# PiggyCh/RL_arm_under_sparse_reward

Hardware: AMD Instinct MI355X
Metric: HER-relabelled transitions sampled+updated /sec, batch 256, 1/2/4/8 MI355X (higher is better)
Workload: dtype f32; 1 GPU; push task (obs 27, goal 3, action 4, T 100), buffer 500000 transitions (5000 episodes) per GPU, batch 256 per GPU, replay_k 4, HIP HER sampler + FP32-MFMA DDPG update, 40 updates + store/normalizer/polyak per cycle; global_batch=256, episodes_per_gpu=5000, parallelism=dp1, cycle_mode=hipGraph, sampler_rng=MT19937 numpy-legacy stream on device (bit-exact indices)

## Files before the change

include/rlarm_hip_debug.h:

```cpp
#ifndef RLARM_HIP_DEBUG_H
#define RLARM_HIP_DEBUG_H

#include "rlarm_hip.h"

#ifdef __cplusplus
extern "C" {
#endif

int hp_ctx_launch_floor(hp_ctx *ctx, int n, int graph, double *us_per_kernel);
int hp_ctx_event_pair_us(hp_ctx *ctx, int reps, double *us);
int hp_ctx_clock_mhz(hp_ctx *ctx, double *mhz);

int hp_buffer_sample_device_us(hp_buffer *buf, hp_rng *rng, int64_t batch, double future_p, double sq_threshold,
                               int32_t reps, double *draw_us, double *gather_us);

int hp_buffer_sample_dev_us(hp_buffer *buf, hp_rng *rng, hp_norm *o_norm, hp_norm *g_norm, int64_t batch, double future_p,
                            double sq_threshold, double clip_obs, int32_t reps, int32_t f32_rows, double *draw_us, double *gather_us);

int hp_buffer_sample_dev_fast_us(hp_buffer *buf, hp_norm *o_norm, hp_norm *g_norm, int64_t batch, double future_p, double sq_threshold,
                                 double clip_obs, int32_t reps, int32_t f32_rows, double *us);

int hp_mt_jump_poly(uint64_t n_words, uint64_t *limbs312);
int hp_rng_parallel_info(hp_rng *rng, int64_t *min_batch, int64_t *n_parallel, int64_t *n_fallback);
int hp_rng_debug_set_window(hp_rng *rng, int64_t words);
int hp_rng_debug_table_ms(hp_rng *rng, double *ms);

int hp_agent_set_adam(hp_agent *ag, int32_t net, const float *m_host, const float *v_host, int64_t n, int64_t step);

int hp_agent_debug_chain(hp_agent *ag, int32_t kind, int32_t n, double *us_per_launch);
int hp_agent_update_kernels(hp_agent *ag, hp_buffer *buf, hp_norm *o_norm, hp_norm *g_norm, hp_rng *rng, double future_p,
                            double sq_threshold, int32_t n_updates, int32_t caller_exchanges, char *out, int32_t out_len);
int hp_agent_debug_timeline(hp_agent *ag, uint64_t *out192);

#define HP_STATE_DIRTY_CHUNK 2048
int hp_state_debug_dirty_scan(hp_buffer *buf, const uint32_t *stamps_host, int64_t current_size, uint32_t since, int64_t max_dirty,
                              int64_t *slots_out, int64_t *n_dirty, int32_t *overflow);

int hp_rollout_debug_set_launch_cap(hp_rollout *ro, int64_t timesteps);

int hp_ctx_calibrate(hp_ctx *ctx, double *out4);

#ifdef __cplusplus
}
#endif
#endif
```

rl_arm_under_sparse_reward_amd/_lib.py:

```python
from __future__ import annotations

import ctypes as C
import os
import threading

import numpy as np

_PKG = os.path.dirname(os.path.abspath(__file__))
LIB_PATH = os.path.join(_PKG, "librlarm_hip.so")

c_void_pp = C.POINTER(C.c_void_p)
f64p = C.POINTER(C.c_double)
f32p = C.POINTER(C.c_float)
i64p = C.POINTER(C.c_int64)
u32p = C.POINTER(C.c_uint32)
u8p = C.POINTER(C.c_uint8)


class HpError(RuntimeError):
    pass


class SampleOut(C.Structure):
    _fields_ = [("obs", f64p), ("ag", f64p), ("g", f64p), ("actions", f64p), ("obs_next", f64p), ("ag_next", f64p),
                ("r", f32p), ("e", i64p), ("t", i64p), ("future_t", i64p), ("her", u8p), ("r64", f64p)]


class SampleDevOut(C.Structure):
    _fields_ = [("x", C.c_void_p), ("x_next", C.c_void_p), ("actions", C.c_void_p), ("r", C.c_void_p),
                ("e", C.c_void_p), ("t", C.c_void_p), ("future_t", C.c_void_p), ("her", C.c_void_p)]


class AgentCfg(C.Structure):
    _fields_ = [("obs_dim", C.c_int32), ("goal_dim", C.c_int32), ("act_dim", C.c_int32), ("hidden", C.c_int32),
                ("batch", C.c_int32), ("grad_world_size", C.c_int32),
                ("max_action", C.c_double), ("gamma", C.c_double), ("action_l2", C.c_double),
                ("lr_actor", C.c_double), ("lr_critic", C.c_double), ("polyak", C.c_double),
                ("clip_obs", C.c_double), ("clip_range", C.c_double),
                ("adam_beta1", C.c_double), ("adam_beta2", C.c_double), ("adam_eps", C.c_double)]


class StateSection(C.Structure):
    _fields_ = [("name", C.c_char * 32), ("dtype", C.c_int32), ("elem_bytes", C.c_int32), ("count", C.c_int64),
                ("offset", C.c_int64)]


class EnvDesc(C.Structure):
    _fields_ = [("kind", C.c_int32), ("reserved", C.c_int32), ("params", C.c_double * 8), ("state_dev", C.c_void_p * 4)]


class DemoScriptDesc(C.Structure):
    _fields_ = [("phase_end", C.c_int32 * 5), ("reserved", C.c_int32), ("lift", C.c_double * 4), ("waypoint", C.c_double * 3),
                ("behind", C.c_double), ("stop_radius", C.c_double)]


ENV_POINT_MASS = 1
ENV_PUSH_BLOCK = 2
ROLLOUT_MAX_LAUNCH_TIMESTEPS = 4096


class StateDims(C.Structure):
    _fields_ = [("obs_dim", C.c_int32), ("goal_dim", C.c_int32), ("act_dim", C.c_int32), ("hidden", C.c_int32),
                ("T", C.c_int32), ("reserved", C.c_int32), ("capacity", C.c_int64), ("current_size", C.c_int64)]


STATE_SECTIONS = 32
STATE_DELTA_SECTIONS = 34
STATE_DIRTY_CHUNK = 2048
ABI_VERSION = 4
PARALLEL_DRAW_MIN_BATCH = 65536

DEBUG_SYMBOLS = {"hp_ctx_launch_floor", "hp_ctx_event_pair_us", "hp_ctx_clock_mhz", "hp_ctx_calibrate", "hp_buffer_sample_device_us",
                 "hp_buffer_sample_dev_us", "hp_buffer_sample_dev_fast_us",
                 "hp_mt_jump_poly", "hp_rng_parallel_info", "hp_rng_debug_set_window", "hp_rng_debug_table_ms",
                 "hp_state_debug_dirty_scan", "hp_rollout_debug_set_launch_cap",
                 "hp_agent_set_adam", "hp_agent_debug_chain", "hp_agent_debug_timeline", "hp_agent_update_kernels"}

PROTOTYPES = {
    "hp_abi_version": (C.c_int, []),
    "hp_last_error": (C.c_char_p, []),
    "hp_ctx_create": (C.c_int, [C.c_int, c_void_pp]),
    "hp_ctx_set_stream": (C.c_int, [C.c_void_p, C.c_void_p]),
    "hp_ctx_get_stream": (C.c_int, [C.c_void_p, c_void_pp]),
    "hp_ctx_borrow_stream": (C.c_int, [C.c_void_p, C.c_void_p]),
    "hp_ctx_return_stream": (C.c_int, [C.c_void_p]),
    "hp_ctx_synchronize": (C.c_int, [C.c_void_p]),
    "hp_ctx_device_name": (C.c_int, [C.c_void_p, C.c_char_p, C.c_size_t]),
    "hp_ctx_pci_bus_id": (C.c_int, [C.c_void_p, C.c_char_p, C.c_size_t]),
    "hp_ctx_launch_floor": (C.c_int, [C.c_void_p, C.c_int, C.c_int, f64p]),
    "hp_ctx_event_pair_us": (C.c_int, [C.c_void_p, C.c_int, f64p]),
    "hp_ctx_clock_mhz": (C.c_int, [C.c_void_p, f64p]),
    "hp_ctx_calibrate": (C.c_int, [C.c_void_p, f64p]),
    "hp_ctx_destroy": (None, [C.c_void_p]),
    "hp_rng_create": (C.c_int, [C.c_void_p, c_void_pp]),
    "hp_rng_seed": (C.c_int, [C.c_void_p, C.c_uint32]),
    "hp_rng_set_state": (C.c_int, [C.c_void_p, u32p, C.c_int32]),
    "hp_rng_get_state": (C.c_int, [C.c_void_p, u32p, C.POINTER(C.c_int32)]),
    "hp_rng_randint": (C.c_int, [C.c_void_p, C.c_int64, C.c_int64, C.c_int64, i64p]),
    "hp_rng_uniform": (C.c_int, [C.c_void_p, C.c_int64, f64p]),
    "hp_rng_standard_normal": (C.c_int, [C.c_void_p, C.c_int64, f64p]),
    "hp_rng_binomial1": (C.c_int, [C.c_void_p, C.c_double, C.c_double, C.c_int64, i64p]),
    "hp_rng_get_gauss": (C.c_int, [C.c_void_p, C.POINTER(C.c_int32), f64p]),
    "hp_rng_set_gauss": (C.c_int, [C.c_void_p, C.c_int32, C.c_double]),
    "hp_rng_advance": (C.c_int, [C.c_void_p, C.c_uint64]),
    "hp_rng_set_parallel": (C.c_int, [C.c_void_p, C.c_int64]),
    "hp_rng_parallel_info": (C.c_int, [C.c_void_p, i64p, i64p, i64p]),
    "hp_rng_debug_set_window": (C.c_int, [C.c_void_p, C.c_int64]),
    "hp_rng_debug_table_ms": (C.c_int, [C.c_void_p, f64p]),
    "hp_mt_jump_poly": (C.c_int, [C.c_uint64, C.POINTER(C.c_uint64)]),
    "hp_rng_destroy": (None, [C.c_void_p]),
    "hp_buffer_create": (C.c_int, [C.c_void_p, C.c_int64, C.c_int32, C.c_int32, C.c_int32, C.c_int32, c_void_pp]),
    "hp_buffer_store": (C.c_int, [C.c_void_p, C.c_void_p, f64p, f64p, f64p, f64p, C.c_int64]),
    "hp_buffer_stage": (C.c_int, [C.c_void_p, f64p, f64p, f64p, f64p, C.c_int64]),
    "hp_host_register": (C.c_int, [C.c_void_p, C.c_void_p, C.c_size_t]),
    "hp_host_unregister": (C.c_int, [C.c_void_p, C.c_void_p]),
    "hp_buffer_store_pinned": (C.c_int, [C.c_void_p, C.c_void_p, C.c_void_p, C.c_int64, C.POINTER(C.c_uint64)]),
    "hp_buffer_store_dev": (C.c_int, [C.c_void_p, C.c_void_p, C.c_void_p, C.c_int64]),
    "hp_buffer_store_done": (C.c_int, [C.c_void_p, C.c_uint64, C.c_int32, C.POINTER(C.c_int32)]),
    "hp_buffer_info": (C.c_int, [C.c_void_p, i64p, i64p, i64p, C.POINTER(C.c_int32)]),
    "hp_buffer_last_slots": (C.c_int, [C.c_void_p, i64p, C.c_int64]),
    "hp_buffer_read": (C.c_int, [C.c_void_p, C.c_int32, C.c_int64, C.c_int64, f64p]),
    "hp_buffer_sample": (C.c_int, [C.c_void_p, C.c_void_p, C.c_int64, C.c_double, C.c_double, C.POINTER(SampleOut)]),
    "hp_buffer_sample_device_us": (C.c_int, [C.c_void_p, C.c_void_p, C.c_int64, C.c_double, C.c_double, C.c_int32, f64p,
                                             f64p]),
    "hp_buffer_sample_dev": (C.c_int, [C.c_void_p, C.c_void_p, C.c_void_p, C.c_void_p, C.c_int64, C.c_double, C.c_double,
                                       C.c_double, C.POINTER(SampleDevOut)]),
    "hp_buffer_sample_dev_us": (C.c_int, [C.c_void_p, C.c_void_p, C.c_void_p, C.c_void_p, C.c_int64, C.c_double, C.c_double,
                                          C.c_double, C.c_int32, C.c_int32, f64p, f64p]),
    "hp_buffer_enable_f32_rows": (C.c_int, [C.c_void_p]),
    "hp_buffer_sample_dev_f32": (C.c_int, [C.c_void_p, C.c_void_p, C.c_void_p, C.c_void_p, C.c_int64, C.c_double, C.c_double,
                                           C.c_double, C.POINTER(SampleDevOut)]),
    "hp_buffer_sample_dev_fast": (C.c_int, [C.c_void_p, C.c_void_p, C.c_void_p, C.c_int64, C.c_double, C.c_double, C.c_double,
                                            C.c_uint64, C.c_uint64, C.c_int32, C.POINTER(SampleDevOut)]),
    "hp_buffer_sample_dev_fast_us": (C.c_int, [C.c_void_p, C.c_void_p, C.c_void_p, C.c_int64, C.c_double, C.c_double, C.c_double,
                                               C.c_int32, C.c_int32, f64p]),
    "hp_buffer_destroy": (None, [C.c_void_p]),
    "hp_compute_reward_dev": (C.c_int, [C.c_void_p, C.c_void_p, C.c_void_p, C.c_int64, C.c_int32, C.c_double, C.c_int32,
                                        C.c_void_p, C.c_void_p]),
    "hp_is_success_dev": (C.c_int, [C.c_void_p, C.c_void_p, C.c_void_p, C.c_int64, C.c_int32, C.c_double, C.c_void_p]),
    "hp_compute_reward": (C.c_int, [C.c_void_p, f64p, f64p, C.c_int64, C.c_int32, C.c_double, C.c_int32, f32p, f64p]),
    "hp_is_success": (C.c_int, [C.c_void_p, f64p, f64p, C.c_int64, C.c_int32, C.c_double, f32p]),
    "hp_norm_create": (C.c_int, [C.c_void_p, C.c_int32, C.c_double, C.c_double, C.c_int32, c_void_pp]),
    "hp_norm_update": (C.c_int, [C.c_void_p, f64p, C.c_int64]),
    "hp_norm_recompute_begin": (C.c_int, [C.c_void_p, c_void_pp, i64p]),
    "hp_norm_recompute_end": (C.c_int, [C.c_void_p]),
    "hp_norm_recompute": (C.c_int, [C.c_void_p]),
    "hp_norm_get": (C.c_int, [C.c_void_p, f32p, f64p, f32p, f32p, f32p, f32p, f32p, f32p]),
    "hp_norm_set_stats": (C.c_int, [C.c_void_p, f32p, f64p]),
    "hp_norm_normalize": (C.c_int, [C.c_void_p, f64p, C.c_int64, C.c_double, f64p]),
    "hp_norm_update_from_staged": (C.c_int, [C.c_void_p, C.c_void_p, C.c_void_p, C.c_void_p, C.c_double, C.c_double]),
    "hp_norm_destroy": (None, [C.c_void_p]),
    "hp_agent_create": (C.c_int, [C.c_void_p, C.POINTER(AgentCfg), c_void_pp]),
    "hp_agent_param_count": (C.c_int64, [C.c_void_p, C.c_int32]),
    "hp_agent_set_params": (C.c_int, [C.c_void_p, C.c_int32, f32p, C.c_int64]),
    "hp_agent_get_params": (C.c_int, [C.c_void_p, C.c_int32, f32p, C.c_int64]),
    "hp_agent_get_grads": (C.c_int, [C.c_void_p, C.c_int32, f32p, C.c_int64]),
    "hp_agent_get_adam": (C.c_int, [C.c_void_p, C.c_int32, f32p, f32p, C.c_int64, i64p]),
    "hp_agent_set_adam": (C.c_int, [C.c_void_p, C.c_int32, f32p, f32p, C.c_int64, C.c_int64]),
    "hp_agent_update_minibatch": (C.c_int, [C.c_void_p, f32p, f32p, f32p, f32p, f32p]),
    "hp_agent_sample_and_update": (C.c_int, [C.c_void_p, C.c_void_p, C.c_void_p, C.c_void_p, C.c_void_p, C.c_double,
                                             C.c_double, C.c_int32]),
    "hp_agent_get_losses": (C.c_int, [C.c_void_p, f32p, C.c_int32]),
    "hp_agent_soft_update": (C.c_int, [C.c_void_p]),
    "hp_agent_actor_forward": (C.c_int, [C.c_void_p, C.c_int32, f32p, C.c_int64, f32p]),
    "hp_agent_critic_forward": (C.c_int, [C.c_void_p, C.c_int32, f32p, f32p, C.c_int64, f32p]),
    "hp_agent_act": (C.c_int, [C.c_void_p, C.c_void_p, C.c_void_p, C.c_int32, f64p, f64p, C.c_int64, C.c_double, f32p]),
    "hp_agent_act_dev": (C.c_int, [C.c_void_p, C.c_void_p, C.c_void_p, C.c_int32, C.c_void_p, C.c_void_p, C.c_int64, C.c_double,
                                   C.c_void_p]),
    "hp_rollout_create": (C.c_int, [C.c_void_p, C.c_void_p, C.c_int64, c_void_pp]),
    "hp_rollout_begin": (C.c_int, [C.c_void_p, C.c_int64, C.c_int64]),
    "hp_rollout_set_action_max": (C.c_int, [C.c_void_p, C.c_double]),
    "hp_rollout_step": (C.c_int, [C.c_void_p, C.c_void_p, C.c_void_p, C.c_void_p, C.c_void_p, C.c_int32, C.c_void_p, C.c_void_p,
                                  C.c_void_p, C.c_int32, C.c_double, C.c_double, C.c_double, C.c_double, C.c_void_p]),
    "hp_rollout_finish": (C.c_int, [C.c_void_p, C.c_void_p, C.c_void_p]),
    "hp_rollout_block": (C.c_int, [C.c_void_p, c_void_pp, i64p, i64p, i64p]),
    "hp_rollout_read": (C.c_int, [C.c_void_p, C.c_int32, f64p]),
    "hp_rollout_destroy": (None, [C.c_void_p]),
    "hp_streams_create": (C.c_int, [C.c_void_p, C.c_int64, c_void_pp]),
    "hp_streams_seed": (C.c_int, [C.c_void_p, u32p, C.c_int64, C.c_uint32]),
    "hp_streams_get_state": (C.c_int, [C.c_void_p, C.c_int64, u32p, C.POINTER(C.c_int32), C.POINTER(C.c_int32), f64p]),
    "hp_streams_set_state": (C.c_int, [C.c_void_p, C.c_int64, u32p, C.c_int32, C.c_int32, C.c_double]),
    "hp_streams_get_all": (C.c_int, [C.c_void_p, u32p, C.POINTER(C.c_int32), C.POINTER(C.c_int32), f64p]),
    "hp_streams_set_all": (C.c_int, [C.c_void_p, u32p, C.POINTER(C.c_int32), C.POINTER(C.c_int32), f64p]),
    "hp_streams_destroy": (None, [C.c_void_p]),
    "hp_rollout_step_streams": (C.c_int, [C.c_void_p, C.c_void_p, C.c_void_p, C.c_void_p, C.c_void_p, C.c_int32, C.c_void_p,
                                          C.c_void_p, C.c_void_p, C.c_int32, C.c_double, C.c_double, C.c_double, C.c_double,
                                          C.c_void_p]),
    "hp_rollout_episodes": (C.c_int, [C.c_void_p, C.c_void_p, C.c_void_p, C.c_void_p, C.c_void_p, C.POINTER(EnvDesc), C.c_int32,
                                      C.c_double, C.c_double, C.c_double, C.c_double, C.c_void_p]),
    "hp_env_reset": (C.c_int, [C.c_void_p, C.POINTER(EnvDesc), C.c_void_p, C.c_int64]),
    "hp_rollout_waves": (C.c_int, [C.c_void_p, C.c_void_p, C.c_void_p, C.c_void_p, C.c_void_p, C.c_void_p, C.POINTER(EnvDesc),
                                   C.c_int64, C.c_int32, C.c_double, C.c_double, C.c_double, C.c_double, C.c_void_p,
                                   C.POINTER(C.c_int32)]),
    "hp_rollout_debug_set_launch_cap": (C.c_int, [C.c_void_p, C.c_int64]),
    "hp_demo_episodes": (C.c_int, [C.c_void_p, C.POINTER(EnvDesc), C.c_void_p, C.POINTER(DemoScriptDesc), C.c_int64, C.c_int64,
                                   C.c_int64, C.c_int32, C.c_void_p, C.c_void_p, C.c_void_p, C.POINTER(C.c_int32)]),
    "hp_demo_compact": (C.c_int, [C.c_void_p, C.c_void_p, C.c_void_p, C.c_void_p, C.c_int64, C.c_void_p, C.c_void_p, C.c_int64,
                                  C.c_int64, C.c_void_p]),
    "hp_agent_policy_snapshot": (C.c_int, [C.c_void_p, C.c_void_p, C.c_void_p]),
    "hp_agent_act_snapshot": (C.c_int, [C.c_void_p, f64p, f64p, C.c_int64, C.c_double, f32p]),
    "hp_agent_forward_backward": (C.c_int, [C.c_void_p, C.c_void_p, C.c_void_p, C.c_void_p, C.c_void_p, C.c_double,
                                            C.c_double]),
    "hp_agent_grad_buffer": (C.c_int, [C.c_void_p, c_void_pp, i64p]),
    "hp_agent_param_buffer": (C.c_int, [C.c_void_p, c_void_pp, i64p]),
    "hp_agent_apply": (C.c_int, [C.c_void_p]),
    "hp_agent_sync_targets": (C.c_int, [C.c_void_p]),
    "hp_comm_unique_id": (C.c_int, [u8p]),
    "hp_comm_create": (C.c_int, [C.c_void_p, u8p, C.c_int32, C.c_int32, c_void_pp]),
    "hp_comm_info": (C.c_int, [C.c_void_p, C.POINTER(C.c_int32), C.POINTER(C.c_int32)]),
    "hp_comm_allreduce_sum_f32": (C.c_int, [C.c_void_p, C.c_void_p, C.c_int64]),
    "hp_comm_allreduce_mean_f32": (C.c_int, [C.c_void_p, C.c_void_p, C.c_int64]),
    "hp_comm_broadcast_f32": (C.c_int, [C.c_void_p, C.c_void_p, C.c_int64, C.c_int32]),
    "hp_comm_destroy": (None, [C.c_void_p]),
    "hp_agent_set_comm": (C.c_int, [C.c_void_p, C.c_void_p]),
    "hp_peer_create": (C.c_int, [C.c_void_p, C.c_int32, C.c_int32, C.c_int64, c_void_pp, u8p]),
    "hp_peer_connect": (C.c_int, [C.c_void_p, u8p]),
    "hp_peer_allreduce_f32": (C.c_int, [C.c_void_p, C.c_void_p, C.c_int64, C.c_int32]),
    "hp_peer_selfcheck": (C.c_int, [C.c_void_p, C.POINTER(C.c_uint32)]),
    "hp_peer_status": (C.c_int, [C.c_void_p, C.POINTER(C.c_uint32)]),
    "hp_peer_phases": (C.c_int, [C.c_void_p, C.POINTER(C.c_int32)]),
    "hp_peer_set_gate": (C.c_int, [C.c_void_p, C.c_int32]),
    "hp_peer_destroy": (None, [C.c_void_p]),
    "hp_agent_set_peer": (C.c_int, [C.c_void_p, C.c_void_p]),
    "hp_agent_cycle_mode": (C.c_int, [C.c_void_p, C.POINTER(C.c_int32)]),
    "hp_agent_set_grad_reduce": (C.c_int, [C.c_void_p, C.c_int32]),
    "hp_agent_train_cycle": (C.c_int, [C.c_void_p, C.c_void_p, C.c_void_p, C.c_void_p, C.c_void_p, f64p, f64p, f64p,
                                       f64p, C.c_int64, C.c_double, C.c_double, C.c_int32]),
    "hp_agent_train_cycle_pinned": (C.c_int, [C.c_void_p, C.c_void_p, C.c_void_p, C.c_void_p, C.c_void_p, C.c_void_p, C.c_int64,
                                              C.c_double, C.c_double, C.c_int32, C.POINTER(C.c_uint64)]),
    "hp_agent_train_cycle_dev": (C.c_int, [C.c_void_p, C.c_void_p, C.c_void_p, C.c_void_p, C.c_void_p, C.c_void_p, C.c_int64,
                                           C.c_double, C.c_double, C.c_int32]),
    "hp_agent_debug_chain": (C.c_int, [C.c_void_p, C.c_int32, C.c_int32, f64p]),
    "hp_agent_debug_timeline": (C.c_int, [C.c_void_p, C.POINTER(C.c_uint64)]),
    "hp_agent_update_kernels": (C.c_int, [C.c_void_p, C.c_void_p, C.c_void_p, C.c_void_p, C.c_void_p, C.c_double, C.c_double,
                                          C.c_int32, C.c_int32, C.c_char_p, C.c_int32]),
    "hp_agent_engine": (C.c_int, [C.c_void_p, C.POINTER(C.c_int32), C.POINTER(C.c_int32), C.POINTER(C.c_int32)]),
    "hp_agent_status": (C.c_int, [C.c_void_p, u32p]),
    "hp_agent_update_form": (C.c_int, [C.c_void_p, C.c_int32, C.POINTER(C.c_int32)]),
    "hp_agent_profile": (C.c_int, [C.c_void_p, C.c_int32]),
    "hp_agent_profile_read": (C.c_int, [C.c_void_p, f64p, C.c_int32]),
    "hp_agent_destroy": (None, [C.c_void_p]),
    "hp_state_layout": (C.c_int, [C.c_void_p, C.c_void_p, C.c_void_p, C.c_void_p, C.c_int64, C.POINTER(StateSection),
                                  C.POINTER(C.c_int32), C.POINTER(C.c_size_t)]),
    "hp_state_capture": (C.c_int, [C.c_void_p, C.c_void_p, C.c_void_p, C.c_void_p, C.c_void_p, C.POINTER(C.c_uint64),
                                   C.POINTER(C.c_size_t)]),
    "hp_state_fetch": (C.c_int, [C.c_void_p, C.c_uint64, C.c_int32, C.c_void_p, C.c_size_t, C.POINTER(C.c_uint64),
                                 C.POINTER(C.c_int32)]),
    "hp_state_restore": (C.c_int, [C.c_void_p, C.c_void_p, C.c_void_p, C.c_void_p, C.c_void_p, C.POINTER(StateDims), C.c_void_p,
                                   C.c_size_t, C.POINTER(C.c_uint64)]),
    "hp_state_layout_delta": (C.c_int, [C.c_void_p, C.c_void_p, C.c_void_p, C.c_void_p, C.c_int64, C.POINTER(StateSection),
                                        C.POINTER(C.c_int32), C.POINTER(C.c_size_t)]),
    "hp_state_capture_delta": (C.c_int, [C.c_void_p, C.c_void_p, C.c_void_p, C.c_void_p, C.c_void_p, C.c_uint32, C.c_int64,
                                         C.POINTER(C.c_uint64), C.POINTER(C.c_size_t)]),
    "hp_state_epochs": (C.c_int, [C.c_void_p, C.c_void_p, u32p, u32p, u32p]),
    "hp_state_debug_dirty_scan": (C.c_int, [C.c_void_p, u32p, C.c_int64, C.c_uint32, C.c_int64, i64p, i64p,
                                            C.POINTER(C.c_int32)]),
    "hp_state_checksum_dev": (C.c_int, [C.c_void_p, C.c_void_p, C.c_size_t, C.c_int32, C.POINTER(C.c_uint64)]),
}

_lib = None
_lock = threading.Lock()

pending_lock = threading.RLock()
_pending = []
_NO_FLUSH = {"hp_last_error", "hp_abi_version"}


def register_pending(obj):
    with pending_lock:
        if not any(o is obj for o in _pending):
            _pending.append(obj)


def unregister_pending(obj):
    with pending_lock:
        _pending[:] = [o for o in _pending if o is not obj]


def flush_pending():
    if not _pending:
        return
    with pending_lock:
        todo, _pending[:] = list(_pending), []
        for i, o in enumerate(todo):
            try:
                o._flush_updates()
            except BaseException:
                for rest in todo[i + 1:]:
                    register_pending(rest)
                raise


class _Library:

    def __init__(self, cdll):
        object.__setattr__(self, "_cdll", cdll)

    def __getattr__(self, name):
        fn = getattr(object.__getattribute__(self, "_cdll"), name)
        if name in _NO_FLUSH or not name.startswith("hp_"):
            return fn

        def call(*args):
            if _pending:
                flush_pending()
            return fn(*args)

        call.__name__ = name
        object.__setattr__(self, name, call)
        return call


def load(path: str | None = None):
    global _lib
    with _lock:
        if _lib is not None:
            return _lib
        p = path or os.environ.get("RLARM_LIB") or LIB_PATH
        if not os.path.exists(p):
            raise HpError(
                f"{p} is missing: build it with `python -c 'import __graft_entry__ as g; g.build()'` "
                "(hipcc --offload-arch=gfx950).  This package has no CPU fallback.")
        lib = C.CDLL(p)
        missing = []
        for name, (res, args) in PROTOTYPES.items():
            try:
                fn = getattr(lib, name)
            except AttributeError:
                missing.append(name)
                continue
            fn.restype = res
            fn.argtypes = args
        if missing:
            raise HpError("librlarm_hip.so does not export: " + ", ".join(missing) + " -- rebuild it")
        if lib.hp_abi_version() != ABI_VERSION:
            raise HpError(f"librlarm_hip.so has ABI version {lib.hp_abi_version()}, this package binds version {ABI_VERSION} "
                          "(include/rlarm_hip.h: HP_ABI_VERSION) -- rebuild it")
        _lib = _Library(lib)
        return _lib


def last_error(lib=None):
    return ((lib or load()).hp_last_error() or b"").decode("utf-8", "replace")


def check(status: int):
    if status == 0:
        return
    msg = (load().hp_last_error() or b"").decode("utf-8", "replace")
    if status in (-1, -2):
        raise ValueError(msg)
    raise HpError(f"[hp_status {status}] {msg}")


def ptr(a: np.ndarray, ctype):
    return a.ctypes.data_as(C.POINTER(ctype)) if a is not None else None


def as_f64(a):
    return np.ascontiguousarray(a, dtype=np.float64)


def as_f32(a):
    return np.ascontiguousarray(a, dtype=np.float32)


class Context:

    _default = None

    def __init__(self, device_id: int | None = None):
        lib = load()
        if device_id is None:
            device_id = int(os.environ.get("LOCAL_RANK", "0"))
        h = C.c_void_p()
        check(lib.hp_ctx_create(int(device_id), C.byref(h)))
        self.lib, self.h, self.device_id = lib, h, int(device_id)

    @classmethod
    def default(cls):
        if cls._default is None:
            cls._default = cls()
        return cls._default

    def set_stream(self, stream_ptr):
        check(self.lib.hp_ctx_set_stream(self.h, C.c_void_p(stream_ptr or 0)))
        self._bound_stream = stream_ptr or 0

    def use_torch_stream(self):
        import torch

        torch.cuda.set_device(self.device_id)
        self.set_stream(torch.cuda.current_stream(self.device_id).cuda_stream or 1)

    def torch_bridge(self):
        import contextlib

        import torch

        @contextlib.contextmanager
        def bridge():
            cur = C.c_void_p(torch.cuda.current_stream(self.device_id).cuda_stream or None)
            check(self.lib.hp_ctx_borrow_stream(self.h, cur))
            try:
                yield
            finally:
                self.lib.hp_ctx_return_stream(self.h)
        return bridge()

    def synchronize(self):
        check(self.lib.hp_ctx_synchronize(self.h))

    @property
    def name(self):
        buf = C.create_string_buffer(160)
        check(self.lib.hp_ctx_device_name(self.h, buf, 160))
        return buf.value.decode()


class DevicePointer:

    def __init__(self, address: int, n: int, typestr="<f4"):
        self.__cuda_array_interface__ = {"shape": (int(n),), "typestr": typestr, "data": (int(address), False),
                                         "version": 2}
```

rl_arm_under_sparse_reward_amd/csrc/agent.h:

```cpp
#pragma once
#include "internal.h"

#include <algorithm>
#include <cstdlib>

typedef float f32x4 __attribute__((ext_vector_type(4)));
typedef float f32x16 __attribute__((ext_vector_type(16)));

#define S8_AHEAD_WGS 4
#define S32_ROWS 32
#define DW_PART (64 * 64 + 64)

struct NetLayout {
    int K1;
    int w1, b1, w2, b2, w3, b3, w4, b4, total;
};

enum { EPI_NONE = 0, EPI_BIAS_RELU = 1, EPI_BIAS = 2, EPI_BIAS_TANH = 3, EPI_MASK = 4 };

struct GemmProb {
    const float *A, *B;
    float *C;
    const float *bias;
    const float *mask;
    float *bias_grad;
    float *C2;
    int a_si, a_sk;
    int b_sj, b_sk;
    int ldc, ldmask, ldc2;
    int M, N, K;
    int n_store;
    int epi;
    int tile0, tiles_n;
    int ks, part0;
    float max_action;
    int frag_layer;
};

#define MAX_PROBS 8
#define GL_PART (32 * 32 + 32)
#define GL_MAX_SPLIT_TILES 64
#define GL_MAX_KS 8
struct GemmGroup {
    int n;
    int xcd;
    int uni;
    int bias0;
    int loss_wg;
    float *part;
    unsigned long long *ticket;
    GemmProb p[MAX_PROBS];
};

struct Pass {
    float *h1, *h2, *h3;
};

struct AgentDevState {
    long long step;
    long long n_logged;
    float neg_step_actor, neg_step_critic, bc2_sqrt;
    unsigned open_timeouts;
};

struct AdamCfg {
    double lr_actor, lr_critic, beta1, beta2, eps;
};

__device__ __forceinline__ void adam_prepare(AgentDevState *st, const AdamCfg c) {
    const double step = (double)st->step;
    const double bc1 = 1.0 - pow(c.beta1, step);
    const double bc2 = 1.0 - pow(c.beta2, step);
    st->neg_step_actor = (float)(-(c.lr_actor / bc1));
    st->neg_step_critic = (float)(-(c.lr_critic / bc1));
    st->bc2_sqrt = (float)sqrt(bc2);
}

#define SPLIT_CTR_STRIDE 64
#define SPLIT_COUNTERS 8
#define SPLIT_CTR_NONE 15u
#define SPLIT_SET_WORDS (SPLIT_COUNTERS * 8 * SPLIT_CTR_STRIDE)
#define SPLIT_FAULT (2 * SPLIT_SET_WORDS)
#define SPLIT_SYNC_WORDS (SPLIT_FAULT + 4)

__device__ __forceinline__ void handoff_fault(unsigned *fault, unsigned *fault_host, unsigned which) {
    const unsigned word = 1u | (1u << (3u + which));
    __hip_atomic_fetch_or(fault, word, __ATOMIC_RELAXED, __HIP_MEMORY_SCOPE_AGENT);
    if (fault_host) __hip_atomic_fetch_or(fault_host, word, __ATOMIC_RELAXED, __HIP_MEMORY_SCOPE_SYSTEM);
}

__device__ __forceinline__ bool handoff_wait(const unsigned *ctr, unsigned need, unsigned long long ticks, unsigned *fault,
                                             unsigned *fault_host, unsigned which, int *flag) {
    if (threadIdx.x == 0) {
        int ok = 1;
        const unsigned long long t0 = wall_clock64();
        for (;;) {
            const unsigned seen = __hip_atomic_load(ctr, __ATOMIC_RELAXED, __HIP_MEMORY_SCOPE_AGENT);
            if (seen >= need) break;
            if (seen == 0u) __builtin_amdgcn_s_sleep(64);
            else __builtin_amdgcn_s_sleep(6);
            if (wall_clock64() - t0 > ticks) {
                handoff_fault(fault, fault_host, which);
                ok = 0;
                break;
            }
        }
        *flag = ok;
    }
    __syncthreads();
    const bool ok = *flag != 0;
    __syncthreads();
    return ok;
}
#define LOSS_LOG 4096

#include "slab_common.h"
#include "peer.h"

struct SeqKey {
    enum Kind { CYCLE, UPDATES } kind;
    hp_buffer *b;
    hp_norm *on, *gn;
    hp_rng *rng;
    int n;
    int64_t n_new;
    double future_p, sq_threshold;
    bool open;
    uint64_t gen;
    bool operator==(const SeqKey &o) const {
        return kind == o.kind && b == o.b && on == o.on && gn == o.gn && rng == o.rng && n == o.n && n_new == o.n_new &&
               future_p == o.future_p && sq_threshold == o.sq_threshold && open == o.open && gen == o.gen;
    }
};
struct GraphCache {
    struct Entry {
        SeqKey key;
        GraphExec exec;
    };
    std::vector<Entry> entries;
    hipGraphExec_t find(const SeqKey &k) const {
        for (const Entry &e : entries)
            if (e.key == k) return e.exec.h;
        return nullptr;
    }
    bool has(SeqKey::Kind kind) const {
        return std::any_of(entries.begin(), entries.end(), [&](const Entry &e) { return e.key.kind == kind; });
    }
    hipGraphExec_t put(const SeqKey &k, GraphExec &&x) {
        const auto same_kind = [&](const Entry &e) { return e.key.kind == k.kind; };
        if (std::count_if(entries.begin(), entries.end(), same_kind) >= (k.kind == SeqKey::CYCLE ? 1 : 8))
            entries.erase(std::find_if(entries.begin(), entries.end(), same_kind));
        entries.push_back({k, std::move(x)});
        return entries.back().exec.h;
    }
    void clear() { entries.clear(); }
};

enum { PROF_SAMPLE = 0, PROF_GEMM_FWD = 1, PROF_GEMM_BWD = 2, PROF_LOSS = 3, PROF_ADAM = 4, PROF_PLAN = 5, PROF_DW = 6, PROF_N = 7 };

struct hp_agent {
    hp_ctx *ctx = nullptr;
    hp_agent_cfg cfg;
    int H = 256, B = 0, Mp = 0;
    int xdim = 0, act_off = 0, ldx = 0;
    NetLayout la, lc;
    int n_arena = 0;
    float *params = nullptr, *targets = nullptr, *grads = nullptr, *adam_m = nullptr, *adam_v = nullptr;
    float *XA = nullptr, *XP = nullptr, *XT = nullptr, *R = nullptr, *TP = nullptr;
    float *XA2 = nullptr, *XP2 = nullptr, *XT2 = nullptr, *R2 = nullptr;
    Pass AT, CT, CA, AP, CP;
    float *QT = nullptr, *QA = nullptr, *QP = nullptr, *dQA = nullptr, *dQP = nullptr;
    float *QT2 = nullptr;
    float *dA3 = nullptr, *dA2 = nullptr, *dA1 = nullptr;
    float *dP3 = nullptr, *dP2 = nullptr, *dP1 = nullptr, *dXP = nullptr;
    float *dZ = nullptr, *dK3 = nullptr, *dK2 = nullptr, *dK1 = nullptr;
    float *loss_log = nullptr;
    AgentDevState *d_state = nullptr;
    float *fragF = nullptr, *fragD = nullptr, *fragFT = nullptr, *part = nullptr;
    unsigned long long *timeline = nullptr;
    bool slab = true;
    bool slab8 = true;
    bool slab32 = false;
    int s8_rows = 4;
    bool fuse_adam_ok = true;
    bool dw64 = false;
    int dw_S = 3;
    DevBuf dw_part, dw_ticket;
    int chain_wt = -1;
    bool keep_grads_dbg = false;
    bool upd_graph_ok = true;
    bool gather_ahead = true;
    DevBuf plan, norm_plan;
    int plan_batches = 0;
    DevBuf fwd_ws;
    struct PolicySnap {
        float *params = nullptr, *fragF = nullptr;
        NormDev *on = nullptr, *gn = nullptr;
        double clip_o = 0, clip_g = 0;
        int od = 0, gd = 0;
        hipEvent_t ready = nullptr;
    } snap[2];
    int snap_cur = -1, snap_pending = -1;
    struct StateArena *state = nullptr;
    hipStream_t act_stream = nullptr;
    hipEvent_t act_done = nullptr;
    bool act_recorded = false;
    DevBuf act_ws;
    PinnedBuf pin;
    std::vector<void *> owned;
    hp_comm *comm = nullptr;
    hp_peer *peer = nullptr;
    bool grad_mean = false;
    bool comm_warm = false;
    bool graph_refused = false;
    GraphCache graphs;
    unsigned *open_sync = nullptr;
    int loss_wg = 1;
    int dw_ksplit = 0;
    float *gl_part = nullptr;
    unsigned long long *gl_ticket = nullptr;
    int split_mode = -1;
    unsigned *k1_sync = nullptr;
    unsigned *fault_host = nullptr;
    unsigned *fault_host_dev = nullptr;
    bool cycle_open = true;
    bool prof = false;
    hipEvent_t ev0 = nullptr, ev1 = nullptr;
    double prof_ms[PROF_N] = {0};
    long long prof_cnt[PROF_N] = {0};
    long long host_steps = 0;
};


static inline AdamCfg adam_cfg(const hp_agent *a) {
    return AdamCfg{a->cfg.lr_actor, a->cfg.lr_critic, a->cfg.adam_beta1, a->cfg.adam_beta2, a->cfg.adam_eps};
}

static inline NetLayout make_layout(int K1, int H) {
    NetLayout l;
    l.K1 = K1;
    int o = 0;
    l.w1 = o; o += H * K1;
    l.b1 = o; o += H;
    l.w2 = o; o += H * H;
    l.b2 = o; o += H;
    l.w3 = o; o += H * H;
    l.b3 = o; o += H;
    l.w4 = o; o += 16 * H;
    l.b4 = o; o += 16;
    l.total = o;
    return l;
}

static inline int roundup(int v, int m) { return (v + m - 1) / m * m; }

struct Launch {
    GemmGroup g;
    int tiles = 0;
    Launch() {
        g.n = 0;
        g.xcd = 0;
        g.uni = 0;
        g.bias0 = 0;
        g.loss_wg = 0;
        g.part = nullptr;
        g.ticket = nullptr;
    }
    int split_tiles = 0;
    unsigned long long head(int half) const {
        unsigned long long w = 0ull;
        for (int i = 0; i < 4; ++i) {
            const int pi = 4 * half + i;
            w |= (unsigned long long)(pi < g.n ? (g.p[pi].tile0 & 0xffff) : 0xffff) << (16 * i);
        }
        return w;
    }
    int separate_bias() {
        int nb = 0;
        for (int i = 0; i < g.n; ++i)
            if (g.p[i].bias_grad) nb += (g.p[i].M + 31) / 32;
        g.bias0 = tiles;
        return nb;
    }
    void split_last(int ks) {
        GemmProb &p = g.p[g.n - 1];
        const int nt = tiles - p.tile0;
        p.ks = ks;
        p.part0 = split_tiles;
        split_tiles += nt;
        tiles += (ks - 1) * nt;
    }
    void place_on_xcds() {
        if (g.n < 4) return;
        for (int i = 0; i < 4; ++i)
            if (g.p[i].tiles_n != 8 || g.p[i].M != 256 || g.p[i].tile0 != 64 * i) return;
        g.xcd = 1;
    }
    GemmProb &add(int M, int N, int K) {
        GemmProb &p = g.p[g.n++];
        memset(&p, 0, sizeof(p));
        p.M = M; p.N = N; p.K = K;
        p.n_store = N;
        p.ks = 1;
        p.tiles_n = (N + 31) / 32;
        p.tile0 = tiles;
        tiles += ((M + 31) / 32) * p.tiles_n;
        return p;
    }
};

struct ProfScope {
    hp_agent *a;
    int which;
    ProfScope(hp_agent *ag, int w) : a(ag), which(w) {
        if (a->prof) (void)hipEventRecord(a->ev0, a->ctx->stream);
    }
    ~ProfScope() {
        if (a->prof) {
            (void)hipEventRecord(a->ev1, a->ctx->stream);
            (void)hipEventSynchronize(a->ev1);
            float ms = 0.f;
            (void)hipEventElapsedTime(&ms, a->ev0, a->ev1);
            a->prof_ms[which] += ms;
            a->prof_cnt[which] += 1;
        }
    }
};

static inline void add_fwd(Launch &L, const float *X, int ldx, int K, const float *W, const float *bias, float *Y, int ldy,
                    int M, int N, int epi) {
    GemmProb &p = L.add(M, N, K);
    p.A = X; p.a_si = ldx; p.a_sk = 1;
    p.B = W; p.b_sj = K; p.b_sk = 1;
    p.C = Y; p.ldc = ldy;
    p.bias = bias;
    p.epi = epi;
}

static inline void add_dx(Launch &L, const float *dY, int ldy, int Nout, const float *W, int Kin, float *dX, int lddx, int M,
                   const float *gate, int ldgate) {
    GemmProb &p = L.add(M, Kin, Nout);
    p.A = dY; p.a_si = ldy; p.a_sk = 1;
    p.B = W; p.b_sj = 1; p.b_sk = Kin;
    p.C = dX; p.ldc = lddx;
    p.mask = gate; p.ldmask = ldgate;
    p.epi = gate ? EPI_MASK : EPI_NONE;
}

static inline void add_dw(Launch &L, const float *dY, int ldy, int Nout, const float *X, int ldx, int Kin, float *dW,
                   float *db, int Mrows, int layer = 0) {
    GemmProb &p = L.add(Nout, Kin, Mrows);
    p.frag_layer = layer;
    p.A = dY; p.a_si = 1; p.a_sk = ldy;
    p.B = X; p.b_sj = 1; p.b_sk = ldx;
    p.C = dW; p.ldc = Kin;
    p.bias_grad = db;
    p.epi = EPI_NONE;
}

enum { SPLIT_TILES_ADAM = 0,
       SPLIT_TILES_PEER = 1,
       SPLIT_TILES_GRADS = 2 };
#define SPLIT_MIN_UPDATES 12

struct SeqPlan {
    enum { RIDE_NONE,
           RIDE_CHAIN,
           RIDE_DW,
           RIDE_FRONT
    } ride = RIDE_NONE;
    int lead = 1;
    bool ahead = false;
    bool s32_serial = false;
    bool split = false;
    int tiles_mode = SPLIT_TILES_GRADS;
    enum { OPT_NONE,
           OPT_TILES,
           OPT_PEER_TILES,
           OPT_KERNEL,
           OPT_PEER_KERNEL,
           OPT_ALLREDUCE
    } opt = OPT_NONE;
    bool fold = false;
};

struct GatherCtx {
    hp_buffer *b;
    hp_norm *on, *gn;
    const PlanRec *plan;
    double sq;
    const SeqPlan *seq = nullptr;
    int u = 0;
    hp_rng *rng = nullptr;
    PlanRec *next_plan = nullptr;
    double future_p = 0.0;
    int xset = 0;
    bool pregathered = false;
    const PlanRec *ahead_plan = nullptr;
    float *grads_out = nullptr;
    bool polyak_after = false;
    int qset = 0;
    const PlanRec *t_plan = nullptr;
};

static inline int chain_wgs(const hp_agent *a) { return 2 * (a->Mp / a->s8_rows); }

int launch_group(hp_agent *a, const Launch &L, int which);
int enqueue_gather(hp_agent *a, hp_buffer *b, hp_norm *on, hp_norm *gn, const PlanRec *plan, double sq, int xset = 0,
                   hipStream_t stream = nullptr);
int enqueue_relayout(hp_agent *a, bool targets);
Launch build_dw_group(const hp_agent *a, const float *sXA, const float *sXP, float *grads = nullptr);
int enqueue_forward_backward(hp_agent *a, const GatherCtx *gc = nullptr, bool fuse_adam = false, bool *fused = nullptr);
int enqueue_forward_backward_slab(hp_agent *a, const GatherCtx *gc, bool fuse_adam, int only = 0);
bool split_fits(const hp_agent *a);
bool split_fits_rows(const hp_agent *a, int rows);
int enqueue_split_prologue(hp_agent *a, const GatherCtx *gc);
int agent_check_fault(const hp_agent *a, const char *who);
static inline unsigned *split_set(const hp_agent *a, int u) { return a->k1_sync + (u & 1) * SPLIT_SET_WORDS; }
int enqueue_adam(hp_agent *a, const GatherCtx *gc = nullptr, unsigned *reset_sync = nullptr);
int enqueue_polyak(hp_agent *a);
bool cycle_open_fits(const hp_agent *a, int64_t n_new);
int cycle_open_launch(hp_agent *a, hp_buffer *b, hp_norm *on, hp_norm *gn, hp_rng *rng, PlanRec *norm_plan, int n_first,
                      double future_p, bool recompute);
int enqueue_peer_adam(hp_agent *a, const GatherCtx *gc, unsigned *reset_sync);
void state_arena_destroy(hp_agent *a);
int enqueue_forward_backward_layers(hp_agent *a);
int layers_enqueue_adam(hp_agent *a);
int layers_enqueue_polyak(hp_agent *a);
```

rl_arm_under_sparse_reward_amd/csrc/agent.hip:

```cpp
#include "agent.h"

#include <functional>

static int run_seq(hp_agent *a, const SeqKey &k);

int agent_check_fault(const hp_agent *a, const char *who) {
    const unsigned w = a->fault_host ? *(volatile const unsigned *)a->fault_host : 0u;
    if (w == 0u) return HP_OK;
    hp_set_error("%s: an in-launch hand-off gave up earlier (%s%s%s; word 0x%x): the launches since skipped work and the "
                 "learner's state is not valid -- recreate the agent", who, (w & 0x10u) ? "critic chains -> weight-gradient tiles; " : "",
                 (w & 0x20u) ? "actor chains -> critic optimizer step; " : "", (w & 0x40u) ? "cycle-opening launch; " : "", w);
    return HP_ERR_STATE;
}

static int ensure_plan(hp_agent *a, int n_batches, int norm_rows = 0) {
    if (n_batches > a->plan_batches) {
        a->graphs.clear();
        HP_TRY(a->plan.ensure((size_t)n_batches * a->B * sizeof(PlanRec)));
        a->plan_batches = n_batches;
    }
    if ((size_t)norm_rows * sizeof(PlanRec) > a->norm_plan.bytes) {
        a->graphs.clear();
        HP_TRY(a->norm_plan.ensure((size_t)norm_rows * sizeof(PlanRec)));
    }
    return HP_OK;
}

static int check_handles(hp_agent *a, hp_buffer *b, hp_norm *on, hp_norm *gn, hp_rng *rng, const char *who) {
    HP_REQUIRE(a && b && on && gn && rng, HP_ERR_INVALID, "%s: null handle", who);
    HP_REQUIRE(b->obs_dim == a->cfg.obs_dim && b->goal_dim == a->cfg.goal_dim && b->act_dim == a->cfg.act_dim,
               HP_ERR_INVALID, "%s: buffer dimensions do not match the agent", who);
    HP_REQUIRE(on->size == a->cfg.obs_dim && gn->size == a->cfg.goal_dim, HP_ERR_INVALID,
               "%s: normalizer sizes do not match the agent", who);
    return HP_OK;
}

struct CycleOpts {
    PlanRec *norm_plan;
    bool open;
    bool recompute;
    std::function<int()> between;
    bool polyak_folded = false;
};
static bool peer_tiles_ok(const hp_agent *a) {
    return a->peer && a->peer->tiles && a->peer->phases == 1 && !a->peer->gate && a->slab && !a->dw64 && a->fuse_adam_ok &&
           build_dw_group(a, a->XA, a->XP).tiles <= HP_PEER_TILES;
}

static SeqPlan seq_plan(const hp_agent *a, int n_updates, bool with_adam) {
    SeqPlan p;
    const bool ride = a->slab && with_adam;
    const bool full = a->slab8 && chain_wgs(a) + 1 + S8_AHEAD_WGS > a->ctx->cu_count;
    const bool s32_ride = ride && a->slab32 && !a->prof;
    const bool dw_ride = s32_ride || (ride && a->slab8 && full);
    p.s32_serial = a->slab32 && !s32_ride;
    p.ahead = ride && ((a->slab8 && (a->gather_ahead || dw_ride)) || s32_ride);
    p.lead = p.ahead ? 2 : 1;
    p.ride = !ride ? SeqPlan::RIDE_NONE : dw_ride ? SeqPlan::RIDE_DW
           : (p.s32_serial && 2 * (a->Mp / S32_ROWS) >= a->ctx->cu_count) ? SeqPlan::RIDE_FRONT : SeqPlan::RIDE_CHAIN;
    const bool peer_tiles = with_adam && peer_tiles_ok(a);
    const bool fuse = with_adam && !a->comm && (!a->peer || peer_tiles) && a->slab && a->fuse_adam_ok;
    p.opt = !with_adam ? SeqPlan::OPT_NONE : peer_tiles ? SeqPlan::OPT_PEER_TILES : a->peer ? SeqPlan::OPT_PEER_KERNEL
          : fuse ? SeqPlan::OPT_TILES : a->comm ? SeqPlan::OPT_ALLREDUCE : SeqPlan::OPT_KERNEL;
    p.split = p.ahead && p.ride == SeqPlan::RIDE_CHAIN && a->slab8 && split_fits(a) &&
              (a->split_mode >= 0 ? a->split_mode == 1 : n_updates >= SPLIT_MIN_UPDATES);
    p.tiles_mode = p.opt == SeqPlan::OPT_PEER_TILES ? SPLIT_TILES_PEER : p.opt == SeqPlan::OPT_TILES ? SPLIT_TILES_ADAM : SPLIT_TILES_GRADS;
    return p;
}

static int enqueue_updates(hp_agent *a, hp_buffer *b, hp_norm *on, hp_norm *gn, hp_rng *rng, double future_p, double sq,
                           int n_updates, bool with_adam, CycleOpts *cyc = nullptr) {
    SeqPlan P = seq_plan(a, n_updates, with_adam);
    P.fold = cyc && with_adam && a->slab;
    HP_REQUIRE(P.opt != SeqPlan::OPT_PEER_TILES || !a->comm, HP_ERR_STATE,
               "tile-wise exchange: the engine did not take the fused optimizer path (a communicator is attached too)");
    PlanRec *plans = a->plan.as<PlanRec>();
    HP_KLOG("#open");
    {
        ProfScope ps(a, PROF_PLAN);
        const int first = P.ride != SeqPlan::RIDE_NONE ? std::min(n_updates, P.lead) : n_updates;
        if (cyc && cyc->open)
            HP_TRY(cycle_open_launch(a, b, on, gn, rng, cyc->norm_plan, first, future_p, cyc->recompute));
        else if (cyc)
            HP_TRY(rng_launch_plan2(rng, b->staged_n, b->T, b->T, cyc->norm_plan, b->d_meta, a->B, first, future_p, plans));
        else
            HP_TRY(rng_launch_plan(rng, b->d_meta, 0, b->T, a->B, first, future_p, plans));
    }
    if (cyc && cyc->between) HP_TRY(cyc->between());
    if (cyc) cyc->polyak_folded = P.fold;
    if (P.split) {
        HP_KLOG("#prologue");
        GatherCtx g0{b, on, gn, plans, sq, &P};
        HP_TRY(enqueue_split_prologue(a, &g0));
    }
    for (int u = 0; u < n_updates; ++u) {
        HP_KLOG("#update");
        GatherCtx gc{b, on, gn, plans + (size_t)u * a->B, sq, &P, u};
        gc.qset = u & 1;
        gc.t_plan = (P.split && u + 1 < n_updates) ? plans + (size_t)(u + 1) * a->B : nullptr;
        if (P.ride != SeqPlan::RIDE_NONE && u + P.lead < n_updates) {
            PlanRec *next = plans + (size_t)(u + P.lead) * a->B;
            if (P.ride == SeqPlan::RIDE_FRONT) HP_TRY(rng_launch_plan(rng, b->d_meta, 0, b->T, a->B, 1, future_p, next));
            else {
                gc.rng = rng;
                gc.next_plan = next;
                gc.future_p = future_p;
            }
        }
        if (a->slab32 && (P.s32_serial || u == 0))
            HP_TRY(enqueue_gather(a, b, on, gn, gc.plan, sq, P.ahead ? (u & 1) : 0));
        if (P.ahead) {
            gc.xset = u & 1;
            gc.pregathered = u > 0;
            if (u + 1 < n_updates) gc.ahead_plan = plans + (size_t)(u + 1) * a->B;
        }
        gc.polyak_after = P.fold && u == n_updates - 1;
        if (P.opt == SeqPlan::OPT_PEER_KERNEL) gc.grads_out = peer_grad_buffer(a->peer, u + 1);
        HP_TRY(enqueue_forward_backward(a, &gc, P.opt == SeqPlan::OPT_TILES || P.opt == SeqPlan::OPT_PEER_TILES));
        unsigned *reset = P.split && P.tiles_mode == SPLIT_TILES_GRADS ? split_set(a, u) : nullptr;
        if (P.opt == SeqPlan::OPT_PEER_KERNEL) {
            HP_TRY(enqueue_peer_adam(a, &gc, reset));
        } else if (P.opt == SeqPlan::OPT_ALLREDUCE) {
            HP_TRY(a->grad_mean ? comm_allreduce_mean_f32(a->comm, a->grads, (size_t)a->n_arena)
                                : comm_allreduce_sum_f32(a->comm, a->grads, (size_t)a->n_arena));
            HP_TRY(enqueue_adam(a, &gc, reset));
        } else if (P.opt == SeqPlan::OPT_KERNEL) {
            HP_TRY(enqueue_adam(a, &gc, reset));
        }
    }
    HP_KLOG("#close");
    if (with_adam && a->peer) HP_TRY(peer_enqueue_seq_end(a->peer, n_updates));
    return HP_OK;
}

static void pack_net(const hp_agent *a, bool critic, const float *flat, float *arena_seg) {
    const NetLayout &l = critic ? a->lc : a->la;
    const int H = a->H, xdim = a->xdim, act = a->cfg.act_dim;
    const int in1 = critic ? xdim + act : xdim;
    const int out4 = critic ? 1 : act;
    memset(arena_seg, 0, sizeof(float) * l.total);
    const float *src = flat;
    for (int r = 0; r < H; ++r)
        for (int c = 0; c < in1; ++c) arena_seg[l.w1 + r * l.K1 + (c < xdim ? c : a->act_off + (c - xdim))] = *src++;
    memcpy(arena_seg + l.b1, src, H * 4); src += H;
    memcpy(arena_seg + l.w2, src, H * H * 4); src += H * H;
    memcpy(arena_seg + l.b2, src, H * 4); src += H;
    memcpy(arena_seg + l.w3, src, H * H * 4); src += H * H;
    memcpy(arena_seg + l.b3, src, H * 4); src += H;
    memcpy(arena_seg + l.w4, src, out4 * H * 4); src += out4 * H;
    memcpy(arena_seg + l.b4, src, out4 * 4);
}

static void unpack_net(const hp_agent *a, bool critic, const float *arena_seg, float *flat) {
    const NetLayout &l = critic ? a->lc : a->la;
    const int H = a->H, xdim = a->xdim, act = a->cfg.act_dim;
    const int in1 = critic ? xdim + act : xdim;
    const int out4 = critic ? 1 : act;
    float *dst = flat;
    for (int r = 0; r < H; ++r)
        for (int c = 0; c < in1; ++c) *dst++ = arena_seg[l.w1 + r * l.K1 + (c < xdim ? c : a->act_off + (c - xdim))];
    memcpy(dst, arena_seg + l.b1, H * 4); dst += H;
    memcpy(dst, arena_seg + l.w2, H * H * 4); dst += H * H;
    memcpy(dst, arena_seg + l.b2, H * 4); dst += H;
    memcpy(dst, arena_seg + l.w3, H * H * 4); dst += H * H;
    memcpy(dst, arena_seg + l.b3, H * 4); dst += H;
    memcpy(dst, arena_seg + l.w4, out4 * H * 4); dst += out4 * H;
    memcpy(dst, arena_seg + l.b4, out4 * 4);
}

static int64_t flat_count(const hp_agent *a, bool critic) {
    const int H = a->H, act = a->cfg.act_dim;
    const int in1 = critic ? a->xdim + act : a->xdim;
    const int out4 = critic ? 1 : act;
    return (int64_t)H * in1 + H + 2ll * (H * H + H) + (int64_t)out4 * H + out4;
}

static int arena_read(hp_agent *a, const float *d_arena, bool critic, float *flat_host, int64_t n) {
    HP_REQUIRE(n == flat_count(a, critic), HP_ERR_INVALID, "flat vector has %lld elements, expected %lld", (long long)n,
               (long long)flat_count(a, critic));
    const NetLayout &l = critic ? a->lc : a->la;
    std::vector<float> seg(l.total);
    HP_CHECK_HIP(hipMemcpyAsync(seg.data(), d_arena + (critic ? a->la.total : 0), sizeof(float) * l.total,
                                hipMemcpyDeviceToHost, a->ctx->stream));
    HP_CHECK_HIP(hipStreamSynchronize(a->ctx->stream));
    unpack_net(a, critic, seg.data(), flat_host);
    return HP_OK;
}

template <class T> static int dev_alloc(hp_agent *a, T **p, size_t count) {
    void *q = nullptr;
    HP_CHECK_HIP(hipMalloc(&q, count * sizeof(T)));
    HP_CHECK_HIP(hipMemsetAsync(q, 0, count * sizeof(T), a->ctx->stream));
    a->owned.push_back(q);
    *p = static_cast<T *>(q);
    return HP_OK;
}

extern "C" {

int hp_agent_create(hp_ctx *ctx, const hp_agent_cfg *cfg, hp_agent **out) {
    HP_REQUIRE(ctx && cfg && out, HP_ERR_INVALID, "hp_agent_create: null argument");
    HP_REQUIRE(cfg->hidden > 0 && cfg->hidden % 32 == 0, HP_ERR_INVALID, "hp_agent_create: hidden must be a multiple of 32");
    HP_REQUIRE(cfg->batch > 0, HP_ERR_INVALID, "hp_agent_create: batch must be positive");
    HP_REQUIRE(cfg->obs_dim > 0 && cfg->goal_dim > 0 && cfg->act_dim > 0 && cfg->act_dim <= 16, HP_ERR_INVALID,
               "hp_agent_create: need obs_dim, goal_dim > 0 and 0 < act_dim <= 16");
    HP_REQUIRE(cfg->max_action > 0, HP_ERR_INVALID, "hp_agent_create: max_action must be positive");
    hp_agent *a = new hp_agent();
    a->ctx = ctx;
    a->cfg = *cfg;
    a->H = cfg->hidden;
    a->B = cfg->batch;
    a->Mp = roundup(cfg->batch, 32);
    a->xdim = cfg->obs_dim + cfg->goal_dim;
    a->act_off = roundup(a->xdim, 16);
    a->ldx = roundup(a->act_off + cfg->act_dim, 16);
    a->la = make_layout(a->act_off, a->H);
    a->lc = make_layout(a->ldx, a->H);
    a->n_arena = a->la.total + a->lc.total;
    const size_t Mp = a->Mp, H = a->H, ldx = a->ldx;
    int st = HP_OK;
    auto A = [&](float **p, size_t n) { if (st == HP_OK) st = dev_alloc(a, p, n); };
    A(&a->params, a->n_arena); A(&a->targets, a->n_arena); A(&a->grads, a->n_arena);
    A(&a->adam_m, a->n_arena); A(&a->adam_v, a->n_arena);
    A(&a->XA, Mp * ldx); A(&a->XP, Mp * ldx); A(&a->XT, Mp * ldx); A(&a->R, Mp); A(&a->TP, 2 * Mp * 16);
    A(&a->XA2, Mp * ldx); A(&a->XP2, Mp * ldx); A(&a->XT2, Mp * ldx); A(&a->R2, Mp);
    for (Pass *ps : {&a->AT, &a->CT, &a->CA, &a->AP, &a->CP}) { A(&ps->h1, Mp * H); A(&ps->h2, Mp * H); A(&ps->h3, Mp * H); }
    A(&a->QT, Mp * 16); A(&a->QT2, Mp * 16); A(&a->QA, Mp * 16); A(&a->QP, Mp * 16); A(&a->dQA, Mp * 16); A(&a->dQP, Mp * 16);
    A(&a->dA3, Mp * H); A(&a->dA2, Mp * H); A(&a->dA1, Mp * H);
    A(&a->dP3, Mp * H); A(&a->dP2, Mp * H); A(&a->dP1, Mp * H); A(&a->dXP, Mp * ldx);
    A(&a->dZ, Mp * 16); A(&a->dK3, Mp * H); A(&a->dK2, Mp * H); A(&a->dK1, Mp * H);
    A(&a->loss_log, LOSS_LOG * 2);
    A(&a->fragF, a->n_arena); A(&a->fragD, a->n_arena); A(&a->fragFT, a->n_arena); A(&a->part, 3 * (Mp / 4));
    {
        const char *e_all = getenv("RLARM_ENGINE");
        char e_name[16] = "";
        for (const char *t = e_all; t && *t;) {
            const size_t n = strcspn(t, ",");
            if (n == 8 && strncmp(t, "chain_wt", n) == 0) a->chain_wt = 1;
            else if (n == 11 && strncmp(t, "chain_plain", n) == 0) a->chain_wt = 0;
            else if (n < sizeof(e_name)) { memcpy(e_name, t, n); e_name[n] = 0; }
            t += n + (t[n] == ',' ? 1 : 0);
        }
        const char *e = e_name[0] ? e_name : nullptr;
        const bool slab_shape = a->H == 256 && a->ldx <= 48 && cfg->act_dim <= 4;
        a->slab = !(e && strcmp(e, "layers") == 0) && slab_shape;
        const int cus_e = a->ctx->cu_count > 0 ? a->ctx->cu_count : 256;
        const bool thin_fits = 2 * (a->Mp / 16) <= cus_e;
        a->slab8 = a->slab && (e && (strcmp(e, "slab8") == 0 || strcmp(e, "slab32") == 0) ? strcmp(e, "slab8") == 0 : thin_fits);
        a->slab32 = a->slab && !a->slab8;
        const int cus = a->ctx->cu_count > 0 ? a->ctx->cu_count : 256;
        auto tri = [](const char *name) { const char *e = getenv(name); return e ? (e[0] != '0' ? 1 : 0) : -1; };
        a->s8_rows = 2 * (a->Mp / 4) <= cus ? 4 : (2 * (a->Mp / 8) <= cus ? 8 : 16);
        if (const char *sr = getenv("RLARM_SLAB_ROWS")) {
            if (strcmp(sr, "4") == 0) a->s8_rows = 4;
            if (strcmp(sr, "8") == 0) a->s8_rows = 8;
            if (strcmp(sr, "16") == 0) a->s8_rows = 16;
        }
        const char *fa = getenv("RLARM_FUSE_ADAM");
        a->fuse_adam_ok = !(fa && fa[0] == '0');
        a->upd_graph_ok = tri("RLARM_UPDATE_GRAPH") != 0;
        a->keep_grads_dbg = tri("RLARM_KEEP_GRADS") == 1;
        a->cycle_open = tri("RLARM_CYCLE_OPEN") != 0;
        a->split_mode = tri("RLARM_SPLIT");
        a->dw64 = a->slab && (tri("RLARM_DW64") >= 0 ? tri("RLARM_DW64") == 1 : a->Mp >= 1536);
        if (const char *ds = getenv("RLARM_DW64"))
            if (ds[0] == 's' && atoi(ds + 1) > 0 && atoi(ds + 1) <= 16) a->dw_S = atoi(ds + 1);
        a->gather_ahead = chain_wgs(a) + 1 + S8_AHEAD_WGS <= cus;
    }
    if (st == HP_OK) st = dev_alloc(a, &a->d_state, 1);
    if (st == HP_OK) st = dev_alloc(a, &a->open_sync, 4);
    if (st == HP_OK) st = dev_alloc(a, &a->k1_sync, SPLIT_SYNC_WORDS);
    if (st == HP_OK) {
        void *hp = nullptr, *dp = nullptr;
        if (hipHostMalloc(&hp, 64, hipHostMallocMapped) != hipSuccess || hipHostGetDevicePointer(&dp, hp, 0) != hipSuccess) {
            hp_set_error("hp_agent_create: pinned fault word: %s", hipGetErrorString(hipGetLastError()));
            st = HP_ERR_HIP;
        } else {
            memset(hp, 0, 64);
            a->fault_host = static_cast<unsigned *>(hp);
            a->fault_host_dev = static_cast<unsigned *>(dp);
        }
    }
    if (st == HP_OK && a->slab) {
        const char *e = getenv("RLARM_DW_KSPLIT");
        a->dw_ksplit = e ? atoi(e) : (a->Mp >= 768 ? 4 : 1);
        if (a->dw_ksplit < 1 || a->dw_ksplit > GL_MAX_KS) a->dw_ksplit = 1;
        const int H = a->H;
        const int narrow = 2 * ((H + 31) / 32) + ((H + 31) / 32) * (((a->lc.K1 + 31) / 32) + ((a->la.K1 + 31) / 32));
        if (narrow <= GL_MAX_SPLIT_TILES) {
            st = dev_alloc(a, &a->gl_part, (size_t)GL_MAX_SPLIT_TILES * GL_MAX_KS * GL_PART);
            if (st == HP_OK) st = dev_alloc(a, &a->gl_ticket, GL_MAX_SPLIT_TILES);
        }
    }
    if (st == HP_OK) st = dev_alloc(a, &a->timeline, 192);
    if (st == HP_OK && a->dw64) {
        Launch L = build_dw_group(a, a->XA, a->XP);
        size_t tiles = 0;
        for (int i = 0; i < L.g.n; ++i) tiles += (size_t)((L.g.p[i].M + 63) / 64) * ((L.g.p[i].N + 63) / 64);
        if (a->dw_part.ensure(tiles * a->dw_S * DW_PART * sizeof(float)) != HP_OK || a->dw_ticket.ensure(tiles * sizeof(unsigned long long)) != HP_OK ||
            hipMemsetAsync(a->dw_ticket.p, 0, tiles * sizeof(unsigned long long), a->ctx->stream) != hipSuccess)
            st = HP_ERR_HIP;
    }
    if (st == HP_OK && hipEventCreate(&a->ev0) != hipSuccess) st = HP_ERR_HIP;
    if (st == HP_OK && hipEventCreate(&a->ev1) != hipSuccess) st = HP_ERR_HIP;
    if (st == HP_OK) st = ensure_plan(a, 1);
    if (st != HP_OK) {
        hp_agent_destroy(a);
        return st;
    }
    *out = a;
    return HP_OK;
}

int64_t hp_agent_param_count(hp_agent *a, int32_t net) {
    if (!a) return -1;
    return flat_count(a, net == HP_NET_CRITIC || net == HP_NET_CRITIC_TARGET);
}

int hp_agent_set_params(hp_agent *a, int32_t net, const float *flat_host, int64_t n) {
    HP_REQUIRE(a && flat_host, HP_ERR_INVALID, "hp_agent_set_params: null argument");
    HP_SERIALISE(a);
    HP_REQUIRE(net >= 0 && net <= 3, HP_ERR_INVALID, "hp_agent_set_params: net=%d not in 0..3", net);
    const bool critic = (net == HP_NET_CRITIC || net == HP_NET_CRITIC_TARGET);
    const bool target = net >= 2;
    HP_REQUIRE(n == flat_count(a, critic), HP_ERR_INVALID, "hp_agent_set_params: got %lld values, expected %lld",
               (long long)n, (long long)flat_count(a, critic));
    const NetLayout &l = critic ? a->lc : a->la;
    std::vector<float> seg(l.total);
    pack_net(a, critic, flat_host, seg.data());
    float *dst = (target ? a->targets : a->params) + (critic ? a->la.total : 0);
    HP_CHECK_HIP(hipMemcpyAsync(dst, seg.data(), sizeof(float) * l.total, hipMemcpyHostToDevice, a->ctx->stream));
    HP_TRY(enqueue_relayout(a, target));
    HP_CHECK_HIP(hipStreamSynchronize(a->ctx->stream));
    return HP_OK;
}

int hp_agent_get_params(hp_agent *a, int32_t net, float *flat_host, int64_t n) {
    HP_REQUIRE(a && flat_host, HP_ERR_INVALID, "hp_agent_get_params: null argument");
    HP_SERIALISE(a);
    HP_REQUIRE(net >= 0 && net <= 3, HP_ERR_INVALID, "hp_agent_get_params: net=%d not in 0..3", net);
    return arena_read(a, net >= 2 ? a->targets : a->params, net == HP_NET_CRITIC || net == HP_NET_CRITIC_TARGET,
                      flat_host, n);
}

int hp_agent_get_grads(hp_agent *a, int32_t net, float *flat_host, int64_t n) {
    HP_REQUIRE(a && flat_host, HP_ERR_INVALID, "hp_agent_get_grads: null argument");
    HP_SERIALISE(a);
    HP_REQUIRE(net == HP_NET_ACTOR || net == HP_NET_CRITIC, HP_ERR_INVALID, "hp_agent_get_grads: net must be actor or critic");
    return arena_read(a, a->grads, net == HP_NET_CRITIC, flat_host, n);
}

int hp_agent_get_adam(hp_agent *a, int32_t net, float *m_host, float *v_host, int64_t n, int64_t *step) {
    HP_REQUIRE(a, HP_ERR_INVALID, "hp_agent_get_adam: null handle");
    HP_SERIALISE(a);
    HP_REQUIRE(net == HP_NET_ACTOR || net == HP_NET_CRITIC, HP_ERR_INVALID, "hp_agent_get_adam: net must be actor or critic");
    if (m_host) HP_TRY(arena_read(a, a->adam_m, net == HP_NET_CRITIC, m_host, n));
    if (v_host) HP_TRY(arena_read(a, a->adam_v, net == HP_NET_CRITIC, v_host, n));
    if (step) {
        AgentDevState h;
        HP_CHECK_HIP(hipMemcpyAsync(&h, a->d_state, sizeof(h), hipMemcpyDeviceToHost, a->ctx->stream));
        HP_CHECK_HIP(hipStreamSynchronize(a->ctx->stream));
        *step = h.step;
    }
    return HP_OK;
}

int hp_agent_set_adam(hp_agent *a, int32_t net, const float *m_host, const float *v_host, int64_t n, int64_t step) {
    HP_REQUIRE(a, HP_ERR_INVALID, "hp_agent_set_adam: null handle");
    HP_SERIALISE(a);
    HP_REQUIRE(net == HP_NET_ACTOR || net == HP_NET_CRITIC, HP_ERR_INVALID, "hp_agent_set_adam: net must be actor or critic");
    HP_REQUIRE(step >= 0, HP_ERR_INVALID, "hp_agent_set_adam: step must be >= 0");
    const bool critic = net == HP_NET_CRITIC;
    HP_REQUIRE(n == flat_count(a, critic), HP_ERR_INVALID, "hp_agent_set_adam: got %lld values, expected %lld", (long long)n,
               (long long)flat_count(a, critic));
    const NetLayout &l = critic ? a->lc : a->la;
    std::vector<float> seg(l.total);
    for (int which = 0; which < 2; ++which) {
        const float *src = which ? v_host : m_host;
        if (!src) continue;
        pack_net(a, critic, src, seg.data());
        float *dst = (which ? a->adam_v : a->adam_m) + (critic ? a->la.total : 0);
        HP_CHECK_HIP(hipMemcpyAsync(dst, seg.data(), sizeof(float) * l.total, hipMemcpyHostToDevice, a->ctx->stream));
        HP_CHECK_HIP(hipStreamSynchronize(a->ctx->stream));
    }
    const long long st = step;
    HP_CHECK_HIP(hipMemcpyAsync(&a->d_state->step, &st, sizeof(st), hipMemcpyHostToDevice, a->ctx->stream));
    HP_CHECK_HIP(hipStreamSynchronize(a->ctx->stream));
    return HP_OK;
}

int hp_agent_sync_targets(hp_agent *a) {
    HP_REQUIRE(a, HP_ERR_INVALID, "hp_agent_sync_targets: null handle");
    HP_SERIALISE(a);
    HP_CHECK_HIP(hipMemcpyAsync(a->targets, a->params, sizeof(float) * a->n_arena, hipMemcpyDeviceToDevice, a->ctx->stream));
    HP_TRY(enqueue_relayout(a, false));
    return enqueue_relayout(a, true);
}

int hp_agent_update_minibatch(hp_agent *a, const float *x, const float *x_next, const float *actions, const float *r,
                              float *losses_host) {
    HP_REQUIRE(a && x && x_next && actions && r, HP_ERR_INVALID, "hp_agent_update_minibatch: null argument");
    HP_SERIALISE(a);
    const int B = a->B, Mp = a->Mp, ldx = a->ldx, xd = a->xdim, ad = a->cfg.act_dim;
    std::vector<float> hxa((size_t)Mp * ldx, 0.f), hxp((size_t)Mp * ldx, 0.f), hxt((size_t)Mp * ldx, 0.f), hr(Mp, 0.f);
    const float maxa = (float)a->cfg.max_action;
    for (int i = 0; i < B; ++i) {
        for (int c = 0; c < xd; ++c) {
            hxa[(size_t)i * ldx + c] = x[(size_t)i * xd + c];
            hxp[(size_t)i * ldx + c] = x[(size_t)i * xd + c];
            hxt[(size_t)i * ldx + c] = x_next[(size_t)i * xd + c];
        }
        for (int c = 0; c < ad; ++c) hxa[(size_t)i * ldx + a->act_off + c] = actions[(size_t)i * ad + c] / maxa;
        hr[i] = r[i];
    }
    hipStream_t s = a->ctx->stream;
    HP_CHECK_HIP(hipMemcpyAsync(a->XA, hxa.data(), hxa.size() * 4, hipMemcpyHostToDevice, s));
    HP_CHECK_HIP(hipMemcpyAsync(a->XP, hxp.data(), hxp.size() * 4, hipMemcpyHostToDevice, s));
    HP_CHECK_HIP(hipMemcpyAsync(a->XT, hxt.data(), hxt.size() * 4, hipMemcpyHostToDevice, s));
    HP_CHECK_HIP(hipMemcpyAsync(a->R, hr.data(), hr.size() * 4, hipMemcpyHostToDevice, s));
    HP_CHECK_HIP(hipStreamSynchronize(s));
    bool fused = false;
    HP_TRY(enqueue_forward_backward(a, nullptr, true, &fused));
    if (!fused) HP_TRY(enqueue_adam(a));
    a->host_steps += 1;
    if (losses_host) HP_TRY(hp_agent_get_losses(a, losses_host, 1));
    else HP_CHECK_HIP(hipStreamSynchronize(s));
    return HP_OK;
}

int hp_agent_sample_and_update(hp_agent *a, hp_buffer *b, hp_norm *on, hp_norm *gn, hp_rng *rng, double future_p,
                               double sq_threshold, int32_t n_updates) {
    HP_TRY(check_handles(a, b, on, gn, rng, "hp_agent_sample_and_update"));
    HP_SERIALISE(a);
    HP_REQUIRE(n_updates > 0, HP_ERR_INVALID, "hp_agent_sample_and_update: n_updates must be positive");
    HP_TRY(peer_check_alive(a->peer, "hp_agent_sample_and_update"));
    HP_TRY(agent_check_fault(a, "hp_agent_sample_and_update"));
    HP_REQUIRE(b->current_size > 0, HP_ERR_EMPTY, "high <= 0");
    return run_seq(a, {SeqKey::UPDATES, b, on, gn, rng, n_updates, 0, future_p, sq_threshold, false, b->gen});
}

int hp_agent_forward_backward(hp_agent *a, hp_buffer *b, hp_norm *on, hp_norm *gn, hp_rng *rng, double future_p,
                              double sq_threshold) {
    HP_TRY(check_handles(a, b, on, gn, rng, "hp_agent_forward_backward"));
    HP_SERIALISE(a);
    HP_REQUIRE(b->current_size > 0, HP_ERR_EMPTY, "high <= 0");
    HP_TRY(ensure_plan(a, 1));
    return enqueue_updates(a, b, on, gn, rng, future_p, sq_threshold, 1, false);
}

int hp_agent_grad_buffer(hp_agent *a, void **dev_grads, int64_t *n_floats) {
    HP_REQUIRE(a && dev_grads && n_floats, HP_ERR_INVALID, "hp_agent_grad_buffer: null argument");
    HP_SERIALISE(a);
    *dev_grads = a->grads;
    *n_floats = a->n_arena;
    return HP_OK;
}

int hp_agent_param_buffer(hp_agent *a, void **dev_params, int64_t *n_floats) {
    HP_REQUIRE(a && dev_params && n_floats, HP_ERR_INVALID, "hp_agent_param_buffer: null argument");
    HP_SERIALISE(a);
    *dev_params = a->params;
    *n_floats = a->n_arena;
    return HP_OK;
}

int hp_agent_apply(hp_agent *a) {
    HP_REQUIRE(a, HP_ERR_INVALID, "hp_agent_apply: null handle");
    HP_SERIALISE(a);
    HP_TRY(enqueue_adam(a));
    a->host_steps += 1;
    return HP_OK;
}

int hp_agent_get_losses(hp_agent *a, float *out_host, int32_t n_last) {
    HP_REQUIRE(a && out_host, HP_ERR_INVALID, "hp_agent_get_losses: null argument");
    HP_SERIALISE(a);
    HP_REQUIRE(n_last > 0 && n_last <= LOSS_LOG, HP_ERR_INVALID, "hp_agent_get_losses: n_last must be in [1, %d]", LOSS_LOG);
    hipStream_t s = a->ctx->stream;
    AgentDevState h;
    std::vector<float> log(LOSS_LOG * 2);
    HP_CHECK_HIP(hipMemcpyAsync(&h, a->d_state, sizeof(h), hipMemcpyDeviceToHost, s));
    HP_CHECK_HIP(hipMemcpyAsync(log.data(), a->loss_log, log.size() * 4, hipMemcpyDeviceToHost, s));
    HP_CHECK_HIP(hipStreamSynchronize(s));
    HP_TRY(agent_check_fault(a, "hp_agent_get_losses"));
    HP_REQUIRE(h.open_timeouts == 0u, HP_ERR_STATE, "hp_agent_get_losses: %u hand-off polls of the cycle-opening launch gave up "
               "(k_cycle_open): the cycles since are not valid", h.open_timeouts);
    HP_REQUIRE(h.n_logged >= n_last, HP_ERR_STATE, "hp_agent_get_losses: only %lld updates logged", h.n_logged);
    for (int i = 0; i < n_last; ++i) {
        const long long k = h.n_logged - n_last + i;
        out_host[2 * i] = log[(k % LOSS_LOG) * 2];
        out_host[2 * i + 1] = log[(k % LOSS_LOG) * 2 + 1];
    }
    return HP_OK;
}

int hp_agent_status(hp_agent *a, uint32_t *fault) {
    HP_REQUIRE(a && fault, HP_ERR_INVALID, "hp_agent_status: null argument");
    *fault = a->fault_host ? *(volatile const unsigned *)a->fault_host : 0u;
    return HP_OK;
}

int hp_agent_soft_update(hp_agent *a) {
    HP_REQUIRE(a, HP_ERR_INVALID, "hp_agent_soft_update: null handle");
    HP_SERIALISE(a);
    return enqueue_polyak(a);
}

}

static int enqueue_cycle_tail(hp_agent *a, hp_buffer *b, hp_norm *on, hp_norm *gn, hp_rng *rng, double future_p,
                              double sq, int n_batches, PlanRec *norm_plan, bool open) {
    CycleOpts cyc;
    cyc.norm_plan = norm_plan;
    cyc.open = open;
    cyc.recompute = !a->comm && !a->peer;
    cyc.between = [=]() -> int {
        if (!open) HP_TRY(norm_launch_update_from_plan(on, gn, b, norm_plan, b->T, a->cfg.clip_obs, !a->comm && !a->peer));
        if (!a->comm && !a->peer) {
        } else if (a->peer) {
            HP_TRY(norm_launch_begin(on));
            HP_TRY(norm_launch_begin(gn));
            HP_TRY(peer_allreduce_small(a->peer, on->d->sync, (size_t)(2 * on->size + 1), true));
            HP_TRY(peer_allreduce_small(a->peer, gn->d->sync, (size_t)(2 * gn->size + 1), true));
            HP_TRY(norm_launch_end(on));
            HP_TRY(norm_launch_end(gn));
        } else {
            HP_TRY(norm_launch_begin(on));
            HP_TRY(norm_launch_begin(gn));
            HP_TRY(comm_allreduce_mean_f32(a->comm, on->d->sync, (size_t)(2 * on->size + 1)));
            HP_TRY(comm_allreduce_mean_f32(a->comm, gn->d->sync, (size_t)(2 * gn->size + 1)));
            HP_TRY(norm_launch_end(on));
            HP_TRY(norm_launch_end(gn));
        }
        return HP_OK;
    };
    HP_TRY(enqueue_updates(a, b, on, gn, rng, future_p, sq, n_batches, true, &cyc));
    if (!cyc.polyak_folded) HP_TRY(enqueue_polyak(a));
    return HP_OK;
}

static int comm_warm_up(hp_agent *a, hp_norm *on, hp_norm *gn) {
    if (!a->comm || a->comm_warm) return HP_OK;
    a->comm_warm = true;
    HP_TRY(comm_allreduce_sum_f32(a->comm, a->grads, (size_t)a->n_arena));
    HP_TRY(comm_allreduce_sum_f32(a->comm, on->d->sync, (size_t)(2 * on->size + 1)));
    return comm_allreduce_sum_f32(a->comm, gn->d->sync, (size_t)(2 * gn->size + 1));
}

static int enqueue_seq(hp_agent *a, const SeqKey &k) {
    if (k.kind == SeqKey::UPDATES) return enqueue_updates(a, k.b, k.on, k.gn, k.rng, k.future_p, k.sq_threshold, k.n, true);
    return enqueue_cycle_tail(a, k.b, k.on, k.gn, k.rng, k.future_p, k.sq_threshold, k.n, a->norm_plan.as<PlanRec>(), k.open);
}

static int run_seq(hp_agent *a, const SeqKey &k) {
    hipStream_t s = a->ctx->stream;
    const bool eager = a->prof || s == hipStreamLegacy || a->graph_refused || (k.kind == SeqKey::UPDATES && !a->upd_graph_ok);
    hipGraphExec_t exec = eager ? nullptr : a->graphs.find(k);
    if (!exec) {
        HP_TRY(ensure_plan(a, k.n, k.kind == SeqKey::CYCLE ? k.b->T : 0));
        if (!eager) {
            HP_TRY(comm_warm_up(a, k.on, k.gn));
            HP_CHECK_HIP(hipStreamSynchronize(s));
            Captured c = capture_graph(s, [&] { return enqueue_seq(a, k); });
            if (c.exec.h) exec = a->graphs.put(k, std::move(c.exec));
            else if (!a->comm) return c.status();
            else a->graph_refused = true;
        }
    }
    if (exec) HP_CHECK_HIP(hipGraphLaunch(exec, s));
    else HP_TRY(enqueue_seq(a, k));
    a->host_steps += k.n;
    return HP_OK;
}

extern "C" {

int hp_agent_set_grad_reduce(hp_agent *a, int32_t mean) {
    HP_REQUIRE(a, HP_ERR_INVALID, "hp_agent_set_grad_reduce: null handle");
    HP_SERIALISE(a);
    if (a->grad_mean != (mean != 0)) a->graphs.clear();
    a->grad_mean = mean != 0;
    return HP_OK;
}

int hp_agent_cycle_mode(hp_agent *a, int32_t *mode) {
    HP_REQUIRE(a && mode, HP_ERR_INVALID, "hp_agent_cycle_mode: null argument");
    HP_SERIALISE(a);
    *mode = a->graph_refused ? 2 : (a->graphs.has(SeqKey::CYCLE) ? 1 : 0);
    return HP_OK;
}

int hp_agent_set_peer(hp_agent *a, hp_peer *peer) {
    HP_REQUIRE(a, HP_ERR_INVALID, "hp_agent_set_peer: null handle");
    HP_SERIALISE(a);
    HP_REQUIRE(!peer || peer->ctx == a->ctx, HP_ERR_INVALID, "hp_agent_set_peer: exchange belongs to another context");
    HP_REQUIRE(!peer || (peer->connected && peer->n_grad == (size_t)a->n_arena), HP_ERR_INVALID,
               "hp_agent_set_peer: exchange not connected, or its gradient length differs from the agent's (%d floats)", a->n_arena);
    HP_REQUIRE(!peer || a->slab, HP_ERR_INVALID, "hp_agent_set_peer: needs a slab engine (the optimizer kernel with fragment copies)");
    a->graphs.clear();
    a->peer = peer;
    return HP_OK;
}

int hp_agent_set_comm(hp_agent *a, hp_comm *comm) {
    HP_REQUIRE(a, HP_ERR_INVALID, "hp_agent_set_comm: null handle");
    HP_SERIALISE(a);
    HP_REQUIRE(!comm || comm->ctx == a->ctx, HP_ERR_INVALID, "hp_agent_set_comm: communicator belongs to another context");
    a->graphs.clear();
    a->graph_refused = false;
    a->comm_warm = false;
    a->comm = comm;
    return HP_OK;
}

static int train_cycle_checks(hp_agent *a, hp_buffer *b, int64_t n_new, int32_t n_batches, const char *who) {
    HP_REQUIRE(n_new > 0 && n_batches > 0, HP_ERR_INVALID, "%s: n_new and n_batches must be positive", who);
    HP_REQUIRE(!(b->current_size == 0 && n_new > b->size), HP_ERR_INVALID, "high <= 0");
    HP_REQUIRE(!a->prof, HP_ERR_STATE, "%s: profiling mode uses the eager path (hp_agent_profile(0) first)", who);
    HP_TRY(agent_check_fault(a, who));
    return peer_check_alive(a->peer, who);
}

int hp_agent_train_cycle(hp_agent *a, hp_buffer *b, hp_norm *on, hp_norm *gn, hp_rng *rng, const double *obs,
                         const double *ag_host, const double *g, const double *actions, int64_t n_new,
                         double future_p, double sq_threshold, int32_t n_batches) {
    HP_TRY(check_handles(a, b, on, gn, rng, "hp_agent_train_cycle"));
    HP_SERIALISE(a);
    HP_REQUIRE(obs && ag_host && g && actions, HP_ERR_INVALID, "hp_agent_train_cycle: null episode array");
    HP_TRY(train_cycle_checks(a, b, n_new, n_batches, "hp_agent_train_cycle"));
    const bool open = a->cycle_open && cycle_open_fits(a, n_new);
    if (open) HP_TRY(buffer_stage_for_cycle(b, obs, ag_host, g, actions, n_new));
    else HP_TRY(buffer_stage_and_store(b, rng, obs, ag_host, g, actions, n_new));
    return run_seq(a, {SeqKey::CYCLE, b, on, gn, rng, n_batches, n_new, future_p, sq_threshold, open, b->gen});
}

int hp_agent_train_cycle_pinned(hp_agent *a, hp_buffer *b, hp_norm *on, hp_norm *gn, hp_rng *rng, const double *block,
                                int64_t n_new, double future_p, double sq_threshold, int32_t n_batches, uint64_t *ticket) {
    HP_TRY(check_handles(a, b, on, gn, rng, "hp_agent_train_cycle_pinned"));
    HP_SERIALISE(a);
    HP_REQUIRE(block, HP_ERR_INVALID, "hp_agent_train_cycle_pinned: null block");
    HP_TRY(train_cycle_checks(a, b, n_new, n_batches, "hp_agent_train_cycle_pinned"));
    const bool open = a->cycle_open && cycle_open_fits(a, n_new);
    HP_TRY(buffer_stage_pinned(b, rng, block, n_new, ticket, !open));
    return run_seq(a, {SeqKey::CYCLE, b, on, gn, rng, n_batches, n_new, future_p, sq_threshold, open, b->gen});
}

int hp_agent_train_cycle_dev(hp_agent *a, hp_buffer *b, hp_norm *on, hp_norm *gn, hp_rng *rng, const double *block_dev,
                             int64_t n_new, double future_p, double sq_threshold, int32_t n_batches) {
    HP_TRY(check_handles(a, b, on, gn, rng, "hp_agent_train_cycle_dev"));
    HP_SERIALISE(a);
    HP_REQUIRE(block_dev, HP_ERR_INVALID, "hp_agent_train_cycle_dev: null block");
    HP_TRY(train_cycle_checks(a, b, n_new, n_batches, "hp_agent_train_cycle_dev"));
    const bool open = a->cycle_open && cycle_open_fits(a, n_new);
    HP_TRY(buffer_stage_dev(b, rng, block_dev, n_new, !open));
    return run_seq(a, {SeqKey::CYCLE, b, on, gn, rng, n_batches, n_new, future_p, sq_threshold, open, b->gen});
}

int hp_agent_update_form(hp_agent *a, int32_t n_updates, int32_t *form) {
    HP_REQUIRE(a && form, HP_ERR_INVALID, "hp_agent_update_form: null argument");
    *form = seq_plan(a, n_updates, true).split ? 1 : 0;
    return HP_OK;
}

int hp_agent_update_kernels(hp_agent *a, hp_buffer *b, hp_norm *on, hp_norm *gn, hp_rng *rng, double future_p, double sq_threshold,
                            int32_t n_updates, int32_t caller_exchanges, char *out, int32_t out_len) {
    HP_TRY(check_handles(a, b, on, gn, rng, "hp_agent_update_kernels"));
    HP_SERIALISE(a);
    HP_REQUIRE(out && out_len > 0 && n_updates > 0, HP_ERR_INVALID, "hp_agent_update_kernels: bad argument");
    HP_REQUIRE(!a->prof, HP_ERR_STATE, "hp_agent_update_kernels: not in profiling mode (its launches are bracketed by events)");
    hipStream_t bound = a->ctx->stream, s = (bound == hipStreamLegacy || bound == hipStreamPerThread) ? a->ctx->own_stream : bound;
    HP_TRY(ensure_plan(a, n_updates));
    HP_CHECK_HIP(hipStreamSynchronize(bound));
    struct Rebind {
        hp_ctx *c; hipStream_t keep;
        ~Rebind() { c->stream = keep; }
    } rebind{a->ctx, bound};
    a->ctx->stream = s;
    std::vector<std::string> log;
    hp_klog = &log;
    const Captured c = capture_graph(s, [&] {
        if (!caller_exchanges) return enqueue_updates(a, b, on, gn, rng, future_p, sq_threshold, n_updates, true);
        HP_TRY(enqueue_updates(a, b, on, gn, rng, future_p, sq_threshold, 1, false));
        HP_KLOG("host:all_reduce");
        return enqueue_adam(a);
    }, false);
    hp_klog = nullptr;
    HP_TRY(c.status());
    std::string j;
    for (size_t i = 0; i < log.size(); ++i) j += (i ? "," : "") + log[i];
    HP_REQUIRE((int)j.size() + 1 <= out_len, HP_ERR_INVALID, "hp_agent_update_kernels: %zu bytes needed", j.size() + 1);
    memcpy(out, j.c_str(), j.size() + 1);
    return HP_OK;
}

int hp_agent_engine(hp_agent *a, int32_t *engine, int32_t *slab_rows, int32_t *dw_split) {
    HP_REQUIRE(a, HP_ERR_INVALID, "hp_agent_engine: null handle");
    if (engine) *engine = !a->slab ? 0 : (a->slab8 ? 8 : 32);
    if (slab_rows) *slab_rows = !a->slab ? 0 : (a->slab8 ? a->s8_rows : S32_ROWS);
    if (dw_split) *dw_split = a->dw64 ? a->dw_S : 0;
    return HP_OK;
}

int hp_agent_profile(hp_agent *a, int32_t enable) {
    HP_REQUIRE(a, HP_ERR_INVALID, "hp_agent_profile: null handle");
    HP_SERIALISE(a);
    a->prof = enable != 0;
    for (int i = 0; i < PROF_N; ++i) {
        a->prof_ms[i] = 0;
        a->prof_cnt[i] = 0;
    }
    return HP_OK;
}

int hp_agent_profile_read(hp_agent *a, double *ms_out, int32_t n) {
    HP_REQUIRE(a && ms_out, HP_ERR_INVALID, "hp_agent_profile_read: null argument");
    HP_SERIALISE(a);
    for (int i = 0; i < PROF_N && 2 * i + 1 < n; ++i) {
        ms_out[2 * i] = a->prof_ms[i];
        ms_out[2 * i + 1] = (double)a->prof_cnt[i];
    }
    return HP_OK;
}

void hp_agent_destroy(hp_agent *a) {
    if (!a) return;
    a->graphs.clear();
    (void)hipStreamSynchronize(a->ctx->stream);
    state_arena_destroy(a);
    for (void *p : a->owned) (void)hipFree(p);
    if (a->act_stream) {
        (void)hipStreamSynchronize(a->act_stream);
        for (auto &ps : a->snap) {
            if (ps.params) (void)hipFree(ps.params);
            if (ps.fragF) (void)hipFree(ps.fragF);
            if (ps.on) (void)hipFree(ps.on);
            if (ps.gn) (void)hipFree(ps.gn);
            if (ps.ready) (void)hipEventDestroy(ps.ready);
        }
        (void)hipEventDestroy(a->act_done);
        (void)hipStreamDestroy(a->act_stream);
    }
    a->act_ws.release();
    a->plan.release();
    a->dw_part.release();
    a->dw_ticket.release();
    a->norm_plan.release();
    a->fwd_ws.release();
    a->pin.release();
    if (a->ev0) (void)hipEventDestroy(a->ev0);
    if (a->ev1) (void)hipEventDestroy(a->ev1);
    if (a->fault_host) (void)hipHostFree(a->fault_host);
    delete a;
}

}
```

rl_arm_under_sparse_reward_amd/csrc/buffer.hip:

```cpp
#include "store_device.h"

#include <cmath>

__global__ __launch_bounds__(256) void k_gather_dict(const double *__restrict__ obs, const double *__restrict__ ag,
                                                     const double *__restrict__ g, const double *__restrict__ act,
                                                     const PlanRec *__restrict__ plan, long long batch, int T,
                                                     int obs_dim, int goal_dim, int act_dim, double sq_threshold,
                                                     double *o_obs, double *o_ag, double *o_g, double *o_act,
                                                     double *o_obs_next, double *o_ag_next, float *o_r,
                                                     double *o_r64) {
    const int lane = threadIdx.x & 63;
    const long long i = (long long)blockIdx.x * (blockDim.x >> 6) + (threadIdx.x >> 6);
    if (i >= batch) return;
    const PlanRec rec = plan[i];
    const long long e = rec.e;
    const int t = rec.t;
    const double *obs_row = obs + (e * (T + 1) + t) * obs_dim;
    const double *ag_row = ag + (e * (T + 1) + t) * goal_dim;
    const double *g_src = rec.her ? ag + (e * (T + 1) + rec.fut) * goal_dim
                                  : g + (e * T + t) * goal_dim;
    const double *act_row = act + (e * T + t) * act_dim;
    for (int c = lane; c < obs_dim; c += 64) {
        o_obs[i * obs_dim + c] = obs_row[c];
        o_obs_next[i * obs_dim + c] = obs_row[obs_dim + c];
    }
    for (int c = lane; c < goal_dim; c += 64) {
        o_ag[i * goal_dim + c] = ag_row[c];
        o_ag_next[i * goal_dim + c] = ag_row[goal_dim + c];
        o_g[i * goal_dim + c] = g_src[c];
    }
    for (int c = lane; c < act_dim; c += 64) o_act[i * act_dim + c] = act_row[c];
    if (lane == 0) {
        double s = 0.0;
        for (int c = 0; c < goal_dim; ++c) {
            double d = __dsub_rn(ag_row[goal_dim + c], g_src[c]);
            double sq = __dmul_rn(d, d);
            s = (c == 0) ? sq : __dadd_rn(s, sq);
        }
        o_r[i] = hp_reward(s, sq_threshold);
        if (o_r64) o_r64[i] = hp_reward64(s, sq_threshold);
    }
}

struct FusedSampleArgs {
    const double *obs, *ag, *g, *act;
    const PlanRec *plan;
    const NormDev *onz, *gnz;
    long long batch;
    int T, od, gd, ad;
    double sq_threshold, clip_obs, clip_o, clip_g;
    float *x, *xn, *a, *r;
    long long *o_e, *o_t, *o_fut;
    unsigned char *o_her;
    unsigned long long fast_seed, fast_call;
    int fast_n_eps;
    double fast_future_p;
};

__device__ __forceinline__ void fs_philox4x32_10(unsigned c0, unsigned c1, unsigned c2, unsigned c3, unsigned k0, unsigned k1,
                                                 unsigned (&out)[4]) {
#pragma unroll
    for (int r = 0; r < 10; ++r) {
        const unsigned long long p0 = 0xD2511F53ull * c0, p1 = 0xCD9E8D57ull * c2;
        const unsigned n0 = (unsigned)(p1 >> 32) ^ c1 ^ k0, n2 = (unsigned)(p0 >> 32) ^ c3 ^ k1;
        c1 = (unsigned)p1;
        c3 = (unsigned)p0;
        c0 = n0;
        c2 = n2;
        k0 += 0x9E3779B9u;
        k1 += 0xBB67AE85u;
    }
    out[0] = c0; out[1] = c1; out[2] = c2; out[3] = c3;
}
__device__ __forceinline__ PlanRec fs_fast_rec(const FusedSampleArgs &A, long long m) {
    unsigned r[4];
    fs_philox4x32_10((unsigned)m, (unsigned)((unsigned long long)m >> 32), (unsigned)A.fast_call, (unsigned)(A.fast_call >> 32),
                     (unsigned)A.fast_seed, (unsigned)(A.fast_seed >> 32), r);
    PlanRec rec;
    rec.e = (int)(((unsigned long long)r[0] * (unsigned)A.fast_n_eps) >> 32);
    rec.t = (int)(((unsigned long long)r[1] * (unsigned)A.T) >> 32);
    rec.her = ((double)r[2] * 0x1p-32 < A.fast_future_p) ? 1 : 0;
    rec.fut = rec.t + 1 + (int)(((unsigned long long)r[3] * (unsigned)(A.T - rec.t)) >> 32);
    return rec;
}
template <int FLIGHT>
__device__ __forceinline__ void fs_fast_recs(const FusedSampleArgs &A, long long base, int lane, int h, PlanRec (&rec)[FLIGHT]) {
    const long long mj = base + (lane & (2 * FLIGHT - 1));
    const PlanRec mine = fs_fast_rec(A, mj < A.batch ? mj : A.batch - 1);
#pragma unroll
    for (int k = 0; k < FLIGHT; ++k) {
        const int src = 2 * k + h;
        rec[k].e = __shfl(mine.e, src);
        rec[k].t = __shfl(mine.t, src);
        rec[k].fut = __shfl(mine.fut, src);
        rec[k].her = __shfl(mine.her, src);
    }
}

template <int FLIGHT>
__global__ __launch_bounds__(256) void k_gather_fused(const FusedSampleArgs A) {
    const int lane = threadIdx.x & 63;
    const long long wave = (long long)blockIdx.x * (blockDim.x >> 6) + (threadIdx.x >> 6);
    const long long n_waves = (long long)gridDim.x * (blockDim.x >> 6);
    const int od = A.od, gd = A.gd, ad = A.ad, ldx = od + gd, Q = 2 * od + 2 * gd + ad;
    auto kind_of = [&](int q) { return q < od ? 0 : q < 2 * od ? 1 : q < 2 * od + gd ? 2 : q < 2 * od + 2 * gd ? 3 : q < Q ? 4 : 5; };
    auto col_of = [&](int q, int kind) { return kind == 0 ? q : kind == 1 ? q - od : kind == 2 ? q - 2 * od : kind == 3 ? q - 2 * od - gd : q - 2 * od - 2 * gd; };
    const int rc = lane < gd ? lane : gd - 1;
    for (long long base = wave * FLIGHT; base < A.batch; base += n_waves * FLIGHT) {
        PlanRec rec[FLIGHT];
#pragma unroll
        for (int k = 0; k < FLIGHT; ++k) rec[k] = A.plan[base + k < A.batch ? base + k : A.batch - 1];
        const double *obs0[FLIGHT], *g_src[FLIGHT];
        double ra[FLIGHT], rg[FLIGHT];
#pragma unroll
        for (int k = 0; k < FLIGHT; ++k) {
            const long long e = rec[k].e;
            const int t = rec[k].t;
            obs0[k] = A.obs + (e * (A.T + 1) + t) * od;
            g_src[k] = rec[k].her ? A.ag + (e * (A.T + 1) + rec[k].fut) * gd : A.g + (e * A.T + t) * gd;
            ra[k] = A.ag[(e * (A.T + 1) + t + 1) * gd + rc];
            rg[k] = g_src[k][rc];
        }
        for (int q0 = 0; q0 < Q; q0 += 64) {
            const int q = q0 + lane, kind = kind_of(q), j = col_of(q, kind);
            float mu = 0.f;
            double sd = 1.0, clip = 0.0;
            if (kind <= 1) { mu = A.onz->mean[j]; sd = A.onz->std[j]; clip = A.clip_o; }
            if (kind == 3) { mu = A.gnz->mean[j]; sd = A.gnz->std[j]; clip = A.clip_g; }
            double v[FLIGHT];
#pragma unroll
            for (int k = 0; k < FLIGHT; ++k) {
                const long long e = rec[k].e;
                const int t = rec[k].t;
                const double *p = kind <= 1 ? obs0[k] + q : kind == 2 ? A.ag + (e * (A.T + 1) + t + 1) * gd + j
                                : kind == 3 ? g_src[k] + j : kind == 4 ? A.act + (e * A.T + t) * ad + j : obs0[k];
                v[k] = *p;
            }
#pragma unroll
            for (int k = 0; k < FLIGHT; ++k) {
                const long long m = base + k;
                if (m >= A.batch) continue;
                if (kind <= 1 || kind == 3) {
                    double c = fmin(fmax(v[k], -A.clip_obs), A.clip_obs);
                    c = __ddiv_rn(__dsub_rn(c, (double)mu), sd);
                    const float x = (float)fmin(fmax(c, -clip), clip);
                    if (kind == 0) { if (A.x) A.x[m * ldx + j] = x; }
                    else if (kind == 1) { if (A.xn) A.xn[m * ldx + j] = x; }
                    else {
                        if (A.x) A.x[m * ldx + od + j] = x;
                        if (A.xn) A.xn[m * ldx + od + j] = x;
                    }
                } else if (kind == 4) {
                    if (A.a) A.a[m * ad + j] = (float)v[k];
                }
            }
        }
#pragma unroll
        for (int k = 0; k < FLIGHT; ++k) {
            const long long m = base + k;
            const double d = __dsub_rn(ra[k], rg[k]);
            const double sq = __dmul_rn(d, d);
            double s = 0.0;
            for (int c = 0; c < gd; ++c) {
                const double sc = __shfl(sq, c);
                s = (c == 0) ? sc : __dadd_rn(s, sc);
            }
            if (m < A.batch && lane == 0) {
                if (A.r) A.r[m] = hp_reward(s, A.sq_threshold);
                if (A.o_e) A.o_e[m] = rec[k].e;
                if (A.o_t) A.o_t[m] = rec[k].t;
                if (A.o_fut) A.o_fut[m] = rec[k].fut;
                if (A.o_her) A.o_her[m] = (unsigned char)rec[k].her;
            }
        }
    }
}

#ifndef FS2_FLIGHT
#define FS2_FLIGHT 4
#endif
typedef double fs_d2 __attribute__((ext_vector_type(2), aligned(8)));
template <int FLIGHT, bool FAST = false>
__global__ __launch_bounds__(256) void k_gather_fused2(const FusedSampleArgs A) {
    const int lane = threadIdx.x & 63, l = lane & 31, h = lane >> 5;
    const long long wave = (long long)blockIdx.x * (blockDim.x >> 6) + (threadIdx.x >> 6);
    const long long n_waves = (long long)gridDim.x * (blockDim.x >> 6);
    const int od = A.od, gd = A.gd, ad = A.ad, ldx = od + gd;
    const int ug = (gd + 1) >> 1, ua = (ad + 1) >> 1;
    const int unit = l < od ? 0 : l < od + ug ? 1 : l < od + ug + ua ? 2 : 3;
    const int j = unit == 0 ? l : unit == 1 ? l - od : l - od - ug;
    const int len = unit == 0 ? 2 * od : unit == 1 ? gd : ad;
    const bool tail = unit != 3 && 2 * j + 1 >= len;
    const int e0 = unit == 3 ? 0 : (tail ? len - 2 : 2 * j);
    float *p0[2], *p1[2];
    int stride0[2], off[2];
    float mu[2] = {0.f, 0.f};
    double sd[2] = {1.0, 1.0}, clip[2] = {INFINITY, INFINITY}, cobs[2] = {INFINITY, INFINITY};
#pragma unroll
    for (int s = 0; s < 2; ++s) {
        const int el = e0 + s;
        const bool ok = unit != 3 && !(tail && s == 0);
        p0[s] = p1[s] = nullptr;
        stride0[s] = ldx;
        off[s] = 0;
        if (ok && unit == 0) {
            const int col = el < od ? el : el - od;
            p0[s] = el < od ? A.x : A.xn;
            off[s] = col;
            mu[s] = A.onz->mean[col]; sd[s] = A.onz->std[col]; clip[s] = A.clip_o; cobs[s] = A.clip_obs;
        } else if (ok && unit == 1) {
            p0[s] = A.x;
            p1[s] = A.xn;
            off[s] = od + el;
            mu[s] = A.gnz->mean[el]; sd[s] = A.gnz->std[el]; clip[s] = A.clip_g; cobs[s] = A.clip_obs;
        } else if (ok) {
            p0[s] = A.a;
            stride0[s] = ad;
            off[s] = el;
        }
    }
    const int rc = l < gd ? l : gd - 1;
    const bool rc_tail = (gd & 1) && rc == gd - 1;
    const int g_lane = (h << 5) + od + (rc_tail ? ug - 1 : (rc >> 1)), g_slot = rc_tail ? 1 : (rc & 1);
    for (long long base = wave * (2 * FLIGHT); base < A.batch; base += n_waves * (2 * FLIGHT)) {
        PlanRec rec[FLIGHT];
        if constexpr (FAST) {
            fs_fast_recs<FLIGHT>(A, base, lane, h, rec);
        } else {
#pragma unroll
            for (int k = 0; k < FLIGHT; ++k) {
                const long long m = base + 2 * k + h;
                rec[k] = A.plan[m < A.batch ? m : A.batch - 1];
            }
        }
        fs_d2 v[FLIGHT];
        double ra[FLIGHT];
#pragma unroll
        for (int k = 0; k < FLIGHT; ++k) {
            const long long e = rec[k].e;
            const int t = rec[k].t;
            const double *obs0 = A.obs + (e * (A.T + 1) + t) * od;
            const double *g_src = rec[k].her ? A.ag + (e * (A.T + 1) + rec[k].fut) * gd : A.g + (e * A.T + t) * gd;
            const double *p = unit == 0 ? obs0 + e0 : unit == 1 ? g_src + e0 : unit == 2 ? A.act + (e * A.T + t) * ad + e0 : obs0;
            v[k] = *reinterpret_cast<const fs_d2 *>(p);
            ra[k] = A.ag[(e * (A.T + 1) + t + 1) * gd + rc];
        }
#pragma unroll
        for (int k = 0; k < FLIGHT; ++k) {
            const long long m = base + 2 * k + h;
            const bool live = m < A.batch;
#pragma unroll
            for (int s = 0; s < 2; ++s) {
                const double val = s ? v[k].y : v[k].x;
                double c = fmin(fmax(val, -cobs[s]), cobs[s]);
                c = __ddiv_rn(__dsub_rn(c, (double)mu[s]), sd[s]);
                const float x = (float)fmin(fmax(c, -clip[s]), clip[s]);
                if (live && p0[s]) p0[s][m * stride0[s] + off[s]] = x;
                if (live && p1[s]) p1[s][m * ldx + off[s]] = x;
            }
            const double gx = __shfl(v[k].x, g_lane), gy = __shfl(v[k].y, g_lane);
            const double d = __dsub_rn(ra[k], g_slot ? gy : gx);
            const double sq = __dmul_rn(d, d);
            double sum = 0.0;
            for (int c = 0; c < gd; ++c) {
                const double sc = __shfl(sq, (h << 5) + c);
                sum = (c == 0) ? sc : __dadd_rn(sum, sc);
            }
            if (live && l == 0) {
                if (A.r) A.r[m] = hp_reward(sum, A.sq_threshold);
                if (A.o_e) A.o_e[m] = rec[k].e;
                if (A.o_t) A.o_t[m] = rec[k].t;
                if (A.o_fut) A.o_fut[m] = rec[k].fut;
                if (A.o_her) A.o_her[m] = (unsigned char)rec[k].her;
            }
        }
    }
}

__global__ __launch_bounds__(256) void k_pack_rows(const long long *__restrict__ slots, long long n, long long first,
                                                   const double *__restrict__ obs, const double *__restrict__ ag,
                                                   const double *__restrict__ g, const double *__restrict__ act, float *p_row,
                                                   double *p_goal, int T, int od, int gd, int ad, int row_w, int goal_w) {
    const long long i = blockIdx.x / ((T + 8) / 8);
    const int t0 = (int)(blockIdx.x % ((T + 8) / 8)) * 8;
    const long long e = slots ? slots[i] : first + i;
    for (int idx = threadIdx.x; idx < 8 * row_w; idx += blockDim.x) {
        const int t = t0 + idx / row_w, c = idx % row_w;
        if (t > T) continue;
        float v = 0.f;
        if (c < od) v = (float)obs[(e * (T + 1) + t) * od + c];
        else if (c < od + ad && t < T) v = (float)act[(e * T + t) * ad + (c - od)];
        p_row[(e * (T + 1) + t) * row_w + c] = v;
    }
    for (int idx = threadIdx.x; idx < 8 * goal_w; idx += blockDim.x) {
        const int t = t0 + idx / goal_w, c = idx % goal_w;
        if (t > T) continue;
        double v = 0.0;
        if (c < gd) v = ag[(e * (T + 1) + t) * gd + c];
        else if (c < 2 * gd && t < T) v = g[(e * T + t) * gd + (c - gd)];
        p_goal[(e * (T + 1) + t) * goal_w + c] = v;
    }
}

struct PackedSampleArgs {
    const float *p_row;
    const double *p_goal;
    int row_w, goal_w;
    FusedSampleArgs f;
};
template <int FLIGHT, bool FAST = false>
__global__ __launch_bounds__(256) void k_gather_packed(const PackedSampleArgs P) {
    const FusedSampleArgs &A = P.f;
    const int lane = threadIdx.x & 63, l = lane & 31, h = lane >> 5;
    const long long wave = (long long)blockIdx.x * (blockDim.x >> 6) + (threadIdx.x >> 6);
    const long long n_waves = (long long)gridDim.x * (blockDim.x >> 6);
    const int od = A.od, gd = A.gd, ad = A.ad, ldx = od + gd, rw = P.row_w, gw = P.goal_w;
    const int load = l < 15 ? 0 : (l == 15 || l == 31) ? 1 : (l == 16 || l == 17) ? 2 : 3;
    const int gj = l == 31 ? 1 : 0;
    float *p0[2], *p1[2];
    int stride0[2], off[2];
    bool goal[2] = {false, false};
    float mu[2] = {0.f, 0.f};
    double sd[2] = {1.0, 1.0}, clip[2] = {INFINITY, INFINITY}, cobs[2] = {INFINITY, INFINITY};
#pragma unroll
    for (int s = 0; s < 2; ++s) {
        p0[s] = p1[s] = nullptr;
        stride0[s] = ldx;
        off[s] = 0;
        if (load == 1) {
            const int c = 2 * gj + s;
            if (c < gd) {
                goal[s] = true;
                p0[s] = A.x; p1[s] = A.xn;
                off[s] = od + c; mu[s] = A.gnz->mean[c]; sd[s] = A.gnz->std[c]; clip[s] = A.clip_g; cobs[s] = A.clip_obs;
            }
        } else if (l != 15 && l != 31) {
            const int col = 4 * (l & 15) + 2 * (l >> 4) + s;
            const int oc = col < rw ? col : col - rw;
            if (oc < od) {
                p0[s] = col < rw ? A.x : A.xn;
                off[s] = oc; mu[s] = A.onz->mean[oc]; sd[s] = A.onz->std[oc]; clip[s] = A.clip_o; cobs[s] = A.clip_obs;
            } else if (col < rw && oc < od + ad) {
                p0[s] = A.a;
                stride0[s] = ad;
                off[s] = oc - od;
            }
        }
    }
    const int rc = l < gd ? l : gd - 1;
    const int a_lane = (h << 5) + 16 + (rc >> 1), g_lane = (h << 5) + (rc < 2 ? 15 : 31), r_slot = rc & 1;
    const int from = (h << 5) + (l & 15);
    typedef float f4_t __attribute__((ext_vector_type(4)));
    typedef double d2_t __attribute__((ext_vector_type(2)));
    typedef float f4_a8 __attribute__((ext_vector_type(4), aligned(8)));
    union Ld { f4_t f; d2_t d; };
    for (long long base = wave * (2 * FLIGHT); base < A.batch; base += n_waves * (2 * FLIGHT)) {
        PlanRec rec[FLIGHT];
        if constexpr (FAST) {
            fs_fast_recs<FLIGHT>(A, base, lane, h, rec);
        } else {
#pragma unroll
            for (int k = 0; k < FLIGHT; ++k) {
                const long long m = base + 2 * k + h;
                rec[k] = A.plan[m < A.batch ? m : A.batch - 1];
            }
        }
        Ld v[FLIGHT];
#pragma unroll
        for (int k = 0; k < FLIGHT; ++k) {
            const long long e = rec[k].e;
            const int t = rec[k].t;
            const float *row = P.p_row + (e * (A.T + 1) + t) * rw;
            const double *goal_t = P.p_goal + (e * (A.T + 1) + t) * gw;
            const double *gsrc = rec[k].her ? P.p_goal + (e * (A.T + 1) + rec[k].fut) * gw : goal_t + gd;
            const void *p = load == 0 ? (const void *)(row + 4 * l) : load == 1 ? (const void *)(gsrc + 2 * gj)
                          : load == 2 ? (const void *)(goal_t + gw + 2 * (l - 16)) : (const void *)row;
            v[k].f = *reinterpret_cast<const f4_a8 *>(p);
        }
#pragma unroll
        for (int k = 0; k < FLIGHT; ++k) {
            const long long m = base + 2 * k + h;
            const bool live = m < A.batch;
            const float z = __shfl(v[k].f[2], from), w = __shfl(v[k].f[3], from);
            const float lo = l < 16 ? v[k].f[0] : z, hi = l < 16 ? v[k].f[1] : w;
#pragma unroll
            for (int s = 0; s < 2; ++s) {
                const float raw = s ? hi : lo;
                double x = goal[s] ? v[k].d[s] : (double)raw;
                x = fmin(fmax(x, -cobs[s]), cobs[s]);
                x = __ddiv_rn(__dsub_rn(x, (double)mu[s]), sd[s]);
                const float o = (float)fmin(fmax(x, -clip[s]), clip[s]);
                if (live && p0[s]) p0[s][m * stride0[s] + off[s]] = o;
                if (live && p1[s]) p1[s][m * ldx + off[s]] = o;
            }
            const double ax = __shfl(v[k].d[0], a_lane), ay = __shfl(v[k].d[1], a_lane);
            const double gx = __shfl(v[k].d[0], g_lane), gy = __shfl(v[k].d[1], g_lane);
            const double d = __dsub_rn(r_slot ? ay : ax, r_slot ? gy : gx);
            const double sq = __dmul_rn(d, d);
            double sum = 0.0;
            for (int c = 0; c < gd; ++c) {
                const double sc = __shfl(sq, (h << 5) + c);
                sum = (c == 0) ? sc : __dadd_rn(sum, sc);
            }
            if (live && l == 0) {
                if (A.r) A.r[m] = hp_reward(sum, A.sq_threshold);
                if (A.o_e) A.o_e[m] = rec[k].e;
                if (A.o_t) A.o_t[m] = rec[k].t;
                if (A.o_fut) A.o_fut[m] = rec[k].fut;
                if (A.o_her) A.o_her[m] = (unsigned char)rec[k].her;
            }
        }
    }
}

__global__ __launch_bounds__(256) void k_goal_reward(const double *__restrict__ ag, const double *__restrict__ g,
                                                     long long n, int goal_dim, double thr_sq, int mode, float *out32,
                                                     double *out64) {
    const long long i = (long long)blockIdx.x * blockDim.x + threadIdx.x;
    if (i >= n) return;
    double s = 0.0;
    for (int c = 0; c < goal_dim; ++c) {
        const double d = __dsub_rn(ag[i * goal_dim + c], g[i * goal_dim + c]);
        const double sq = __dmul_rn(d, d);
        s = (c == 0) ? sq : __dadd_rn(s, sq);
    }
    if (mode == 0) out32[i] = (s >= thr_sq) ? -1.0f : -0.0f;
    else if (mode == 1) out64[i] = -__dsqrt_rn(s);
    else out32[i] = (s < thr_sq) ? 1.0f : 0.0f;
}

#define STORE_PARTS 8
__global__ __launch_bounds__(256) void k_store_scatter(const long long *__restrict__ slots, long long n_new,
                                                       const double *s_obs, const double *s_ag, const double *s_g,
                                                       const double *s_act, double *obs, double *ag, double *g,
                                                       double *act, long long ep_obs, long long ep_ag,
                                                       long long ep_g, long long ep_act, uint32_t *slot_epoch,
                                                       const uint32_t *epoch) {
    store_scatter_share([&](long long j) { return slots[j]; }, blockIdx.x / STORE_PARTS, blockIdx.x % STORE_PARTS, STORE_PARTS,
                        n_new, s_obs, s_ag, s_g, s_act, obs, ag, g, act, ep_obs, ep_ag, ep_g, ep_act, slot_epoch, epoch);
}

int buffer_launch_gather_dict(hp_buffer *b, const PlanRec *d_plan, int64_t batch, double sq_threshold, double *d_out,
                              float *d_r, double *d_r64) {
    const int od = b->obs_dim, gd = b->goal_dim, ad = b->act_dim;
    double *o_obs = d_out;
    double *o_ag = o_obs + batch * od;
    double *o_g = o_ag + batch * gd;
    double *o_act = o_g + batch * gd;
    double *o_obs_next = o_act + batch * ad;
    double *o_ag_next = o_obs_next + batch * od;
    const int waves_per_block = 4;
    dim3 grid((unsigned)((batch + waves_per_block - 1) / waves_per_block));
    hipLaunchKernelGGL(k_gather_dict, grid, dim3(256), 0, b->ctx->stream, b->d_obs, b->d_ag, b->d_g, b->d_act, d_plan,
                       (long long)batch, (int)b->T, od, gd, ad, sq_threshold, o_obs, o_ag, o_g, o_act, o_obs_next,
                       o_ag_next, d_r, d_r64);
    HP_CHECK_HIP(hipGetLastError());
    return HP_OK;
}

static int launch_pack(hp_buffer *b, const long long *slots, int64_t first, int64_t n) {
    if (!b->p_row || n <= 0) return HP_OK;
    const unsigned per_ep = (unsigned)((b->T + 8) / 8);
    HP_KLOG("k_pack_rows");
    hipLaunchKernelGGL(k_pack_rows, dim3((unsigned)n * per_ep), dim3(256), 0, b->ctx->stream, slots, (long long)n, (long long)first,
                       b->d_obs, b->d_ag, b->d_g, b->d_act, b->p_row, b->p_goal, (int)b->T, (int)b->obs_dim, (int)b->goal_dim,
                       (int)b->act_dim, (int)b->row_w, (int)b->goal_w);
    HP_CHECK_HIP(hipGetLastError());
    return HP_OK;
}
int buffer_launch_pack(hp_buffer *b, int64_t n_new) { return launch_pack(b, b->st_slots.as<long long>(), 0, n_new); }
int buffer_launch_pack_range(hp_buffer *b, int64_t first, int64_t n) { return launch_pack(b, nullptr, first, n); }

static int stage_ensure(hp_buffer *b, DevBuf &d, size_t need) {
    if (need > d.bytes) ++b->gen;
    return d.ensure(need);
}

static int buffer_stage(hp_buffer *b, const double *obs, const double *ag, const double *g, const double *actions,
                        int64_t n_new) {
    hipStream_t s = b->ctx->stream;
    const size_t n0 = n_new * b->ep_obs() * 8, n1 = n_new * b->ep_ag() * 8, n2 = n_new * b->ep_g() * 8,
                 n3 = n_new * b->ep_act() * 8;
    HP_TRY(stage_ensure(b, b->st_obs, n0 + n1 + n2 + n3));
    char *dst = b->st_obs.as<char>();
    b->st_ag = reinterpret_cast<double *>(dst + n0);
    b->st_g = reinterpret_cast<double *>(dst + n0 + n1);
    b->st_act = reinterpret_cast<double *>(dst + n0 + n1 + n2);
    HP_TRY(b->pin.ensure(n0 + n1 + n2 + n3));
    char *h = static_cast<char *>(b->pin.p);
    memcpy(h, obs, n0);
    memcpy(h + n0, ag, n1);
    memcpy(h + n0 + n1, g, n2);
    memcpy(h + n0 + n1 + n2, actions, n3);
    HP_CHECK_HIP(hipMemcpyAsync(dst, h, n0 + n1 + n2 + n3, hipMemcpyHostToDevice, s));
    HP_TRY(b->pin.mark(s));
    b->staged_n = n_new;
    return HP_OK;
}

int buffer_stage_and_store(hp_buffer *b, hp_rng *rng, const double *obs, const double *ag, const double *g,
                           const double *actions, int64_t n_new) {
    hipStream_t s = b->ctx->stream;
    HP_TRY(stage_ensure(b, b->st_slots, n_new * 8));
    HP_TRY(buffer_stage(b, obs, ag, g, actions, n_new));
    HP_TRY(rng_launch_slots(rng, b, n_new, b->st_slots.as<int64_t>()));
    hipLaunchKernelGGL(k_store_scatter, dim3((unsigned)(n_new * STORE_PARTS)), dim3(256), 0, s, b->st_slots.as<long long>(),
                       (long long)n_new, b->st_obs.as<double>(), b->st_ag, b->st_g,
                       b->st_act, b->d_obs, b->d_ag, b->d_g, b->d_act, (long long)b->ep_obs(),
                       (long long)b->ep_ag(), (long long)b->ep_g(), (long long)b->ep_act(), b->d_slot_epoch, b->d_epoch);
    HP_CHECK_HIP(hipGetLastError());
    HP_TRY(buffer_launch_pack(b, n_new));
    b->current_size = (b->current_size + n_new < b->size) ? b->current_size + n_new : b->size;
    b->n_transitions_stored += (int64_t)b->T * n_new;
    return HP_OK;
}

int buffer_stage_pinned(hp_buffer *b, hp_rng *rng, const double *block, int64_t n_new, uint64_t *ticket, bool store_now) {
    hipStream_t s = b->ctx->stream;
    const size_t n0 = n_new * b->ep_obs() * 8, n1 = n_new * b->ep_ag() * 8, n2 = n_new * b->ep_g() * 8,
                 n3 = n_new * b->ep_act() * 8;
    HP_TRY(stage_ensure(b, b->st_slots, n_new * 8));
    HP_TRY(stage_ensure(b, b->st_obs, n0 + n1 + n2 + n3));
    char *dst = b->st_obs.as<char>();
    b->st_ag = reinterpret_cast<double *>(dst + n0);
    b->st_g = reinterpret_cast<double *>(dst + n0 + n1);
    b->st_act = reinterpret_cast<double *>(dst + n0 + n1 + n2);
    HP_CHECK_HIP(hipMemcpyAsync(dst, block, n0 + n1 + n2 + n3, hipMemcpyHostToDevice, s));
    const uint64_t t = ++b->pin_tickets;
    hipEvent_t &ev = b->pin_events[t % hp_buffer::PIN_RING];
    if (!ev) HP_CHECK_HIP(hipEventCreateWithFlags(&ev, hipEventDisableTiming));
    else HP_CHECK_HIP(hipEventSynchronize(ev));
    HP_CHECK_HIP(hipEventRecord(ev, s));
    if (ticket) *ticket = t;
    b->staged_n = n_new;
    if (store_now) {
        HP_TRY(rng_launch_slots(rng, b, n_new, b->st_slots.as<int64_t>()));
        hipLaunchKernelGGL(k_store_scatter, dim3((unsigned)(n_new * STORE_PARTS)), dim3(256), 0, s, b->st_slots.as<long long>(),
                           (long long)n_new, b->st_obs.as<double>(), b->st_ag, b->st_g, b->st_act, b->d_obs, b->d_ag, b->d_g,
                           b->d_act, (long long)b->ep_obs(), (long long)b->ep_ag(), (long long)b->ep_g(), (long long)b->ep_act(), b->d_slot_epoch, b->d_epoch);
        HP_CHECK_HIP(hipGetLastError());
        HP_TRY(buffer_launch_pack(b, n_new));
    }
    b->current_size = (b->current_size + n_new < b->size) ? b->current_size + n_new : b->size;
    b->n_transitions_stored += (int64_t)b->T * n_new;
    return HP_OK;
}

int buffer_stage_dev(hp_buffer *b, hp_rng *rng, const double *block_dev, int64_t n_new, bool store_now) {
    hipStream_t s = b->ctx->stream;
    const size_t n0 = n_new * b->ep_obs() * 8, n1 = n_new * b->ep_ag() * 8, n2 = n_new * b->ep_g() * 8,
                 n3 = n_new * b->ep_act() * 8;
    HP_TRY(stage_ensure(b, b->st_slots, n_new * 8));
    HP_TRY(stage_ensure(b, b->st_obs, n0 + n1 + n2 + n3));
    char *dst = b->st_obs.as<char>();
    b->st_ag = reinterpret_cast<double *>(dst + n0);
    b->st_g = reinterpret_cast<double *>(dst + n0 + n1);
    b->st_act = reinterpret_cast<double *>(dst + n0 + n1 + n2);
    HP_CHECK_HIP(hipMemcpyAsync(dst, block_dev, n0 + n1 + n2 + n3, hipMemcpyDeviceToDevice, s));
    b->staged_n = n_new;
    if (store_now) {
        HP_TRY(rng_launch_slots(rng, b, n_new, b->st_slots.as<int64_t>()));
        hipLaunchKernelGGL(k_store_scatter, dim3((unsigned)(n_new * STORE_PARTS)), dim3(256), 0, s, b->st_slots.as<long long>(),
                           (long long)n_new, b->st_obs.as<double>(), b->st_ag, b->st_g, b->st_act, b->d_obs, b->d_ag, b->d_g,
                           b->d_act, (long long)b->ep_obs(), (long long)b->ep_ag(), (long long)b->ep_g(), (long long)b->ep_act(), b->d_slot_epoch, b->d_epoch);
        HP_CHECK_HIP(hipGetLastError());
        HP_TRY(buffer_launch_pack(b, n_new));
    }
    b->current_size = (b->current_size + n_new < b->size) ? b->current_size + n_new : b->size;
    b->n_transitions_stored += (int64_t)b->T * n_new;
    return HP_OK;
}

int buffer_stage_for_cycle(hp_buffer *b, const double *obs, const double *ag, const double *g, const double *actions,
                           int64_t n_new) {
    HP_TRY(stage_ensure(b, b->st_slots, n_new * 8));
    HP_TRY(buffer_stage(b, obs, ag, g, actions, n_new));
    b->current_size = (b->current_size + n_new < b->size) ? b->current_size + n_new : b->size;
    b->n_transitions_stored += (int64_t)b->T * n_new;
    return HP_OK;
}

extern "C" {

int hp_buffer_create(hp_ctx *ctx, int64_t size_episodes, int32_t T, int32_t obs_dim, int32_t goal_dim,
                     int32_t act_dim, hp_buffer **out) {
    HP_REQUIRE(ctx && out, HP_ERR_INVALID, "hp_buffer_create: null argument");
    HP_REQUIRE(size_episodes > 0 && size_episodes < (1ll << 31), HP_ERR_INVALID,
               "hp_buffer_create: size_episodes=%lld must be in [1, 2^31)", (long long)size_episodes);
    HP_REQUIRE(T > 0 && obs_dim > 0 && goal_dim > 0 && act_dim > 0, HP_ERR_INVALID,
               "hp_buffer_create: dimensions must be positive");
    hp_buffer *b = new hp_buffer();
    b->ctx = ctx;
    b->size = size_episodes;
    b->T = T;
    b->obs_dim = obs_dim;
    b->goal_dim = goal_dim;
    b->act_dim = act_dim;
    hipError_t e = hipSuccess;
    if (e == hipSuccess) e = hipMalloc((void **)&b->d_obs, size_episodes * b->ep_obs() * 8);
    if (e == hipSuccess) e = hipMalloc((void **)&b->d_ag, size_episodes * b->ep_ag() * 8);
    if (e == hipSuccess) e = hipMalloc((void **)&b->d_g, size_episodes * b->ep_g() * 8);
    if (e == hipSuccess) e = hipMalloc((void **)&b->d_act, size_episodes * b->ep_act() * 8);
    if (e == hipSuccess) e = hipMalloc((void **)&b->d_meta, sizeof(BufMeta));
    if (e == hipSuccess) e = hipMemsetAsync(b->d_meta, 0, sizeof(BufMeta), ctx->stream);
    if (e == hipSuccess) e = hipMalloc((void **)&b->d_slot_epoch, size_episodes * sizeof(uint32_t));
    if (e == hipSuccess) e = hipMemsetAsync(b->d_slot_epoch, 0, size_episodes * sizeof(uint32_t), ctx->stream);
    if (e == hipSuccess) e = hipMalloc((void **)&b->d_epoch, sizeof(uint32_t));
    if (e == hipSuccess) e = hipMemsetD32Async((hipDeviceptr_t)b->d_epoch, (int)b->epoch, 1, ctx->stream);
    if (e != hipSuccess) {
        hp_set_error("hp_buffer_create: device allocation failed: %s", hipGetErrorString(e));
        hp_buffer_destroy(b);
        return HP_ERR_HIP;
    }
    *out = b;
    return HP_OK;
}

int hp_buffer_store(hp_buffer *b, hp_rng *rng, const double *obs, const double *ag, const double *g,
                    const double *actions, int64_t n_new) {
    HP_REQUIRE(b && rng && obs && ag && g && actions, HP_ERR_INVALID, "hp_buffer_store: null argument");
    HP_SERIALISE(b);
    HP_REQUIRE(n_new > 0, HP_ERR_INVALID, "hp_buffer_store: n_new must be positive");
    HP_REQUIRE(!(b->current_size == 0 && n_new > b->size), HP_ERR_INVALID, "high <= 0");
    return buffer_stage_and_store(b, rng, obs, ag, g, actions, n_new);
}

int hp_host_register(hp_ctx *ctx, void *host, size_t bytes) {
    HP_REQUIRE(ctx && host && bytes > 0, HP_ERR_INVALID, "hp_host_register: bad argument");
    CtxGuard guard(ctx);
    HP_CHECK_HIP(hipHostRegister(host, bytes, hipHostRegisterDefault));
    return HP_OK;
}

int hp_host_unregister(hp_ctx *ctx, void *host) {
    HP_REQUIRE(ctx && host, HP_ERR_INVALID, "hp_host_unregister: bad argument");
    CtxGuard guard(ctx);
    HP_CHECK_HIP(hipHostUnregister(host));
    return HP_OK;
}

int hp_buffer_store_pinned(hp_buffer *b, hp_rng *rng, const double *block, int64_t n_new, uint64_t *ticket) {
    HP_REQUIRE(b && rng && block, HP_ERR_INVALID, "hp_buffer_store_pinned: null argument");
    HP_SERIALISE(b);
    HP_REQUIRE(n_new > 0, HP_ERR_INVALID, "hp_buffer_store_pinned: n_new must be positive");
    HP_REQUIRE(!(b->current_size == 0 && n_new > b->size), HP_ERR_INVALID, "high <= 0");
    return buffer_stage_pinned(b, rng, block, n_new, ticket, true);
}

int hp_buffer_store_dev(hp_buffer *b, hp_rng *rng, const double *block_dev, int64_t n_new) {
    HP_REQUIRE(b && rng && block_dev, HP_ERR_INVALID, "hp_buffer_store_dev: null argument");
    HP_SERIALISE(b);
    HP_REQUIRE(n_new > 0, HP_ERR_INVALID, "hp_buffer_store_dev: n_new must be positive");
    HP_REQUIRE(!(b->current_size == 0 && n_new > b->size), HP_ERR_INVALID, "high <= 0");
    return buffer_stage_dev(b, rng, block_dev, n_new, true);
}

int hp_buffer_store_done(hp_buffer *b, uint64_t ticket, int32_t wait, int32_t *done) {
    HP_REQUIRE(b && done, HP_ERR_INVALID, "hp_buffer_store_done: null argument");
    hipEvent_t ev = nullptr;
    {
        HP_SERIALISE(b);
        HP_REQUIRE(ticket >= 1 && ticket <= b->pin_tickets, HP_ERR_INVALID, "hp_buffer_store_done: unknown ticket");
        if (ticket + hp_buffer::PIN_RING <= b->pin_tickets) {
            *done = 1;
            return HP_OK;
        }
        ev = b->pin_events[ticket % hp_buffer::PIN_RING];
    }
    hipError_t e = hipSuccess;
    if (wait) HP_CHECK_HIP(hipEventSynchronize(ev));
    else e = hipEventQuery(ev);
    if (e != hipSuccess && e != hipErrorNotReady) HP_CHECK_HIP(e);
    (void)hipGetLastError();
    *done = (e == hipSuccess) ? 1 : 0;
    if (!*done) {
        HP_SERIALISE(b);
        if (ticket + hp_buffer::PIN_RING <= b->pin_tickets) *done = 1;
    }
    return HP_OK;
}

int hp_buffer_stage(hp_buffer *b, const double *obs, const double *ag, const double *g, const double *actions,
                    int64_t n_new) {
    HP_REQUIRE(b && obs && ag && g && actions, HP_ERR_INVALID, "hp_buffer_stage: null argument");
    HP_SERIALISE(b);
    HP_REQUIRE(n_new > 0, HP_ERR_INVALID, "high <= 0");
    return buffer_stage(b, obs, ag, g, actions, n_new);
}

int hp_buffer_info(hp_buffer *b, int64_t *size, int64_t *current_size, int64_t *n_transitions_stored, int32_t *T) {
    HP_REQUIRE(b, HP_ERR_INVALID, "hp_buffer_info: null handle");
    HP_SERIALISE(b);
    if (size) *size = b->size;
    if (current_size) *current_size = b->current_size;
    if (n_transitions_stored) *n_transitions_stored = b->n_transitions_stored;
    if (T) *T = b->T;
    return HP_OK;
}

int hp_buffer_last_slots(hp_buffer *b, int64_t *host_out, int64_t n) {
    HP_REQUIRE(b && host_out, HP_ERR_INVALID, "hp_buffer_last_slots: null argument");
    HP_SERIALISE(b);
    HP_REQUIRE(n >= 0 && n <= b->staged_n, HP_ERR_INVALID, "hp_buffer_last_slots: n=%lld exceeds last store (%lld)",
               (long long)n, (long long)b->staged_n);
    HP_CHECK_HIP(hipMemcpyAsync(host_out, b->st_slots.p, n * 8, hipMemcpyDeviceToHost, b->ctx->stream));
    HP_CHECK_HIP(hipStreamSynchronize(b->ctx->stream));
    return HP_OK;
}

int hp_buffer_read(hp_buffer *b, int32_t which, int64_t first, int64_t n, double *host_out) {
    HP_REQUIRE(b && host_out, HP_ERR_INVALID, "hp_buffer_read: null argument");
    HP_SERIALISE(b);
    HP_REQUIRE(first >= 0 && n >= 0 && first + n <= b->size, HP_ERR_INVALID, "hp_buffer_read: range out of bounds");
    const double *src;
    size_t ep;
    switch (which) {
        case 0: src = b->d_obs; ep = b->ep_obs(); break;
        case 1: src = b->d_ag; ep = b->ep_ag(); break;
        case 2: src = b->d_g; ep = b->ep_g(); break;
        case 3: src = b->d_act; ep = b->ep_act(); break;
        default: hp_set_error("hp_buffer_read: which=%d not in 0..3", which); return HP_ERR_INVALID;
    }
    if (n == 0) return HP_OK;
    HP_CHECK_HIP(hipMemcpyAsync(host_out, src + first * ep, n * ep * 8, hipMemcpyDeviceToHost, b->ctx->stream));
    HP_CHECK_HIP(hipStreamSynchronize(b->ctx->stream));
    return HP_OK;
}

int hp_buffer_sample_device_us(hp_buffer *b, hp_rng *rng, int64_t batch, double future_p, double sq_threshold,
                               int32_t reps, double *draw_us, double *gather_us) {
    HP_REQUIRE(b && rng && draw_us && gather_us && batch > 0 && reps > 0, HP_ERR_INVALID, "hp_buffer_sample_device_us: bad argument");
    HP_SERIALISE(b);
    HP_REQUIRE(b->current_size > 0, HP_ERR_EMPTY, "high <= 0");
    hipStream_t s = b->ctx->stream;
    const size_t row = (size_t)(2 * b->obs_dim + 3 * b->goal_dim + b->act_dim);
    HP_TRY(b->plan.ensure(batch * sizeof(PlanRec)));
    HP_TRY(b->out.ensure(batch * row * 8 + batch * 4));
    PlanRec *d_plan = b->plan.as<PlanRec>();
    double *d_out = b->out.as<double>();
    float *d_r = reinterpret_cast<float *>(d_out + batch * row);
    struct Events {
        hipEvent_t e[3] = {nullptr, nullptr, nullptr};
        ~Events() { for (hipEvent_t x : e) if (x) (void)hipEventDestroy(x); }
    } ev;
    for (int i = 0; i < 3; ++i) HP_CHECK_HIP(hipEventCreate(&ev.e[i]));
    HP_TRY(rng_launch_plan(rng, b->d_meta, 0, b->T, batch, 1, future_p, d_plan));
    HP_TRY(buffer_launch_gather_dict(b, d_plan, batch, sq_threshold, d_out, d_r, nullptr));
    HP_CHECK_HIP(hipEventRecord(ev.e[0], s));
    for (int i = 0; i < reps; ++i) HP_TRY(rng_launch_plan(rng, b->d_meta, 0, b->T, batch, 1, future_p, d_plan));
    HP_CHECK_HIP(hipEventRecord(ev.e[1], s));
    for (int i = 0; i < reps; ++i) HP_TRY(buffer_launch_gather_dict(b, d_plan, batch, sq_threshold, d_out, d_r, nullptr));
    HP_CHECK_HIP(hipEventRecord(ev.e[2], s));
    HP_CHECK_HIP(hipEventSynchronize(ev.e[2]));
    float ms01 = 0.f, ms12 = 0.f;
    HP_CHECK_HIP(hipEventElapsedTime(&ms01, ev.e[0], ev.e[1]));
    HP_CHECK_HIP(hipEventElapsedTime(&ms12, ev.e[1], ev.e[2]));
    *draw_us = 1e3 * ms01 / reps;
    *gather_us = 1e3 * ms12 / reps;
    return HP_OK;
}

int hp_buffer_sample(hp_buffer *b, hp_rng *rng, int64_t batch, double future_p, double sq_threshold,
                     const hp_sample_out *o) {
    HP_REQUIRE(b && rng && o, HP_ERR_INVALID, "hp_buffer_sample: null argument");
    HP_SERIALISE(b);
    HP_REQUIRE(batch > 0, HP_ERR_INVALID, "hp_buffer_sample: batch must be positive");
    HP_REQUIRE(b->current_size > 0, HP_ERR_EMPTY, "high <= 0");
    hipStream_t s = b->ctx->stream;
    const int od = b->obs_dim, gd = b->goal_dim, ad = b->act_dim;
    const size_t row = (size_t)(2 * od + 3 * gd + ad);
    HP_TRY(b->plan.ensure(batch * sizeof(PlanRec)));
    HP_TRY(b->out.ensure(batch * row * 8 + batch * 8 + batch * 4));
    PlanRec *d_plan = b->plan.as<PlanRec>();
    double *d_out = b->out.as<double>();
    double *d_r64 = d_out + batch * row;
    float *d_r = reinterpret_cast<float *>(d_r64 + batch);
    HP_TRY(rng_launch_plan_sample(rng, b->d_meta, b->T, batch, future_p, d_plan));
    HP_TRY(buffer_launch_gather_dict(b, d_plan, batch, sq_threshold, d_out, d_r, o->r64 ? d_r64 : nullptr));
    double *p = d_out;
    auto pull = [&](double *dst, size_t n) -> hipError_t {
        hipError_t e = dst ? hipMemcpyAsync(dst, p, n * 8, hipMemcpyDeviceToHost, s) : hipSuccess;
        p += n;
        return e;
    };
    HP_CHECK_HIP(pull(o->obs, batch * od));
    HP_CHECK_HIP(pull(o->ag, batch * gd));
    HP_CHECK_HIP(pull(o->g, batch * gd));
    HP_CHECK_HIP(pull(o->actions, batch * ad));
    HP_CHECK_HIP(pull(o->obs_next, batch * od));
    HP_CHECK_HIP(pull(o->ag_next, batch * gd));
    if (o->r) HP_CHECK_HIP(hipMemcpyAsync(o->r, d_r, batch * 4, hipMemcpyDeviceToHost, s));
    if (o->r64) HP_CHECK_HIP(hipMemcpyAsync(o->r64, d_r64, batch * 8, hipMemcpyDeviceToHost, s));
    std::vector<PlanRec> hplan;
    if (o->e || o->t || o->future_t || o->her) {
        hplan.resize(batch);
        HP_CHECK_HIP(hipMemcpyAsync(hplan.data(), d_plan, batch * sizeof(PlanRec), hipMemcpyDeviceToHost, s));
    }
    HP_CHECK_HIP(hipStreamSynchronize(s));
    for (size_t i = 0; i < hplan.size(); ++i) {
        if (o->e) o->e[i] = hplan[i].e;
        if (o->t) o->t[i] = hplan[i].t;
        if (o->future_t) o->future_t[i] = hplan[i].fut;
        if (o->her) o->her[i] = (uint8_t)hplan[i].her;
    }
    return HP_OK;
}

struct FastDraw {
    uint64_t seed, call;
    double future_p;
};
static int buffer_launch_gather_fused(hp_buffer *b, const PlanRec *d_plan, hp_norm *on, hp_norm *gn, int64_t batch,
                                      double sq_threshold, double clip_obs, const hp_sample_dev_out *o, const FastDraw *fast = nullptr) {
    FusedSampleArgs A;
    A.fast_seed = fast ? fast->seed : 0ull; A.fast_call = fast ? fast->call : 0ull;
    A.fast_n_eps = (int)b->current_size; A.fast_future_p = fast ? fast->future_p : 0.0;
    A.obs = b->d_obs; A.ag = b->d_ag; A.g = b->d_g; A.act = b->d_act;
    A.plan = d_plan;
    A.onz = on->d; A.gnz = gn->d;
    A.batch = batch;
    A.T = b->T; A.od = b->obs_dim; A.gd = b->goal_dim; A.ad = b->act_dim;
    A.sq_threshold = sq_threshold;
    A.clip_obs = clip_obs;
    A.clip_o = on->clip; A.clip_g = gn->clip;
    A.x = o->x; A.xn = o->x_next; A.a = o->actions; A.r = o->r;
    A.o_e = reinterpret_cast<long long *>(o->e); A.o_t = reinterpret_cast<long long *>(o->t);
    A.o_fut = reinterpret_cast<long long *>(o->future_t);
    A.o_her = o->her;
    const int64_t cap = (int64_t)b->ctx->cu_count * 32;
    const int ug = (b->goal_dim + 1) / 2, ua = (b->act_dim + 1) / 2;
    if (b->obs_dim + ug + ua <= 32 && b->goal_dim >= 2 && b->act_dim >= 2) {
        HP_KLOG("k_gather_fused2");
        if (batch >= 16384) {
            const int64_t waves = (batch + 2 * FS2_FLIGHT - 1) / (2 * FS2_FLIGHT), wgs = (waves + 3) / 4;
            const dim3 grid((unsigned)(wgs < cap ? wgs : cap));
            if (fast) hipLaunchKernelGGL((k_gather_fused2<FS2_FLIGHT, true>), grid, dim3(256), 0, b->ctx->stream, A);
            else hipLaunchKernelGGL((k_gather_fused2<FS2_FLIGHT, false>), grid, dim3(256), 0, b->ctx->stream, A);
        } else {
            const int64_t waves = (batch + 1) / 2, wgs = (waves + 3) / 4;
            const dim3 grid((unsigned)(wgs < cap ? wgs : cap));
            if (fast) hipLaunchKernelGGL((k_gather_fused2<1, true>), grid, dim3(256), 0, b->ctx->stream, A);
            else hipLaunchKernelGGL((k_gather_fused2<1, false>), grid, dim3(256), 0, b->ctx->stream, A);
        }
        HP_CHECK_HIP(hipGetLastError());
        return HP_OK;
    }
    HP_REQUIRE(!fast, HP_ERR_INVALID, "hp_buffer_sample_dev_fast: needs obs_dim + ceil(goal_dim / 2) + ceil(act_dim / 2) <= 32 and goal_dim, act_dim >= 2");
    const int flight = batch >= 16384 ? 4 : 1;
    const int64_t waves = (batch + flight - 1) / flight, wgs = (waves + 3) / 4;
    HP_KLOG("k_gather_fused");
    if (flight == 4) hipLaunchKernelGGL(k_gather_fused<4>, dim3((unsigned)(wgs < cap ? wgs : cap)), dim3(256), 0, b->ctx->stream, A);
    else hipLaunchKernelGGL(k_gather_fused<1>, dim3((unsigned)(wgs < cap ? wgs : cap)), dim3(256), 0, b->ctx->stream, A);
    HP_CHECK_HIP(hipGetLastError());
    return HP_OK;
}

static int buffer_launch_gather_packed(hp_buffer *b, const PlanRec *d_plan, hp_norm *on, hp_norm *gn, int64_t batch,
                                       double sq_threshold, double clip_obs, const hp_sample_dev_out *o, const FastDraw *fast = nullptr) {
    PackedSampleArgs P;
    P.p_row = b->p_row; P.p_goal = b->p_goal; P.row_w = b->row_w; P.goal_w = b->goal_w;
    FusedSampleArgs &A = P.f;
    A.fast_seed = fast ? fast->seed : 0ull; A.fast_call = fast ? fast->call : 0ull;
    A.fast_n_eps = (int)b->current_size; A.fast_future_p = fast ? fast->future_p : 0.0;
    A.obs = b->d_obs; A.ag = b->d_ag; A.g = b->d_g; A.act = b->d_act;
    A.plan = d_plan;
    A.onz = on->d; A.gnz = gn->d;
    A.batch = batch;
    A.T = b->T; A.od = b->obs_dim; A.gd = b->goal_dim; A.ad = b->act_dim;
    A.sq_threshold = sq_threshold;
    A.clip_obs = clip_obs;
    A.clip_o = on->clip; A.clip_g = gn->clip;
    A.x = o->x; A.xn = o->x_next; A.a = o->actions; A.r = o->r;
    A.o_e = reinterpret_cast<long long *>(o->e); A.o_t = reinterpret_cast<long long *>(o->t);
    A.o_fut = reinterpret_cast<long long *>(o->future_t);
    A.o_her = o->her;
    const int64_t cap = (int64_t)b->ctx->cu_count * 32;
    HP_KLOG("k_gather_packed");
    if (batch >= 16384) {
        const int64_t waves = (batch + 2 * FS2_FLIGHT - 1) / (2 * FS2_FLIGHT), wgs = (waves + 3) / 4;
        const dim3 grid((unsigned)(wgs < cap ? wgs : cap));
        if (fast) hipLaunchKernelGGL((k_gather_packed<FS2_FLIGHT, true>), grid, dim3(256), 0, b->ctx->stream, P);
        else hipLaunchKernelGGL((k_gather_packed<FS2_FLIGHT, false>), grid, dim3(256), 0, b->ctx->stream, P);
    } else {
        const int64_t waves = (batch + 1) / 2, wgs = (waves + 3) / 4;
        const dim3 grid((unsigned)(wgs < cap ? wgs : cap));
        if (fast) hipLaunchKernelGGL((k_gather_packed<1, true>), grid, dim3(256), 0, b->ctx->stream, P);
        else hipLaunchKernelGGL((k_gather_packed<1, false>), grid, dim3(256), 0, b->ctx->stream, P);
    }
    HP_CHECK_HIP(hipGetLastError());
    return HP_OK;
}

static int sample_dev_check(hp_buffer *b, hp_rng *rng, hp_norm *on, hp_norm *gn, int64_t batch, double clip_obs,
                            const hp_sample_dev_out *o, const char *who) {
    HP_REQUIRE(b && rng && on && gn && o, HP_ERR_INVALID, "%s: null argument", who);
    HP_REQUIRE(on->ctx == b->ctx && gn->ctx == b->ctx && rng->ctx == b->ctx, HP_ERR_INVALID, "%s: handles of different contexts", who);
    HP_REQUIRE(on->size == b->obs_dim && gn->size == b->goal_dim, HP_ERR_INVALID,
               "%s: normalizer sizes (%d, %d) do not match the buffer's observation / goal widths (%d, %d)", who, on->size, gn->size,
               b->obs_dim, b->goal_dim);
    HP_REQUIRE(batch > 0, HP_ERR_INVALID, "%s: batch must be positive", who);
    HP_REQUIRE(clip_obs > 0, HP_ERR_INVALID, "%s: clip_obs must be positive (arguments.py:87; pass a huge value for none)", who);
    HP_REQUIRE(b->goal_dim <= 64, HP_ERR_INVALID, "%s: goal_dim > 64", who);
    return HP_OK;
}

extern "C" int hp_buffer_sample_dev(hp_buffer *b, hp_rng *rng, hp_norm *on, hp_norm *gn, int64_t batch, double future_p,
                                    double sq_threshold, double clip_obs, const hp_sample_dev_out *o) {
    HP_TRY(sample_dev_check(b, rng, on, gn, batch, clip_obs, o, "hp_buffer_sample_dev"));
    HP_SERIALISE(b);
    HP_REQUIRE(b->current_size > 0, HP_ERR_EMPTY, "high <= 0");
    if ((size_t)batch * sizeof(PlanRec) > b->plan.bytes) HP_CHECK_HIP(hipStreamSynchronize(b->ctx->stream));
    HP_TRY(b->plan.ensure(batch * sizeof(PlanRec)));
    PlanRec *d_plan = b->plan.as<PlanRec>();
    HP_TRY(rng_launch_plan_sample(rng, b->d_meta, b->T, batch, future_p, d_plan));
    return buffer_launch_gather_fused(b, d_plan, on, gn, batch, sq_threshold, clip_obs, o);
}

extern "C" int hp_buffer_enable_f32_rows(hp_buffer *b) {
    HP_REQUIRE(b, HP_ERR_INVALID, "hp_buffer_enable_f32_rows: null handle");
    HP_SERIALISE(b);
    if (b->p_row) return HP_OK;
    const int row_w = (b->obs_dim + b->act_dim + 31) / 32 * 32, goal_w = (2 * b->goal_dim + 7) / 8 * 8;
    HP_REQUIRE(row_w == 32 && b->obs_dim <= 28 && b->goal_dim <= 4, HP_ERR_INVALID,
               "hp_buffer_enable_f32_rows: needs obs_dim <= 28, obs_dim + act_dim <= 32 (one 128-byte line of float32 per timestep) and "
               "goal_dim <= 4; got %d, %d, %d", b->obs_dim, b->act_dim, b->goal_dim);
    const size_t rows = (size_t)b->size * (b->T + 1);
    HP_CHECK_HIP(hipMalloc((void **)&b->p_row, rows * row_w * sizeof(float)));
    if (hipMalloc((void **)&b->p_goal, rows * goal_w * sizeof(double)) != hipSuccess) {
        (void)hipFree(b->p_row);
        b->p_row = nullptr;
        hp_set_error("hp_buffer_enable_f32_rows: cannot allocate the goal rows");
        return HP_ERR_HIP;
    }
    b->row_w = row_w;
    b->goal_w = goal_w;
    ++b->gen;
    return launch_pack(b, nullptr, 0, b->size);
}

extern "C" int hp_buffer_sample_dev_f32(hp_buffer *b, hp_rng *rng, hp_norm *on, hp_norm *gn, int64_t batch, double future_p,
                                        double sq_threshold, double clip_obs, const hp_sample_dev_out *o) {
    HP_TRY(sample_dev_check(b, rng, on, gn, batch, clip_obs, o, "hp_buffer_sample_dev_f32"));
    HP_SERIALISE(b);
    HP_REQUIRE(b->p_row, HP_ERR_STATE, "hp_buffer_sample_dev_f32: hp_buffer_enable_f32_rows first");
    HP_REQUIRE(b->current_size > 0, HP_ERR_EMPTY, "high <= 0");
    if ((size_t)batch * sizeof(PlanRec) > b->plan.bytes) HP_CHECK_HIP(hipStreamSynchronize(b->ctx->stream));
    HP_TRY(b->plan.ensure(batch * sizeof(PlanRec)));
    PlanRec *d_plan = b->plan.as<PlanRec>();
    HP_TRY(rng_launch_plan_sample(rng, b->d_meta, b->T, batch, future_p, d_plan));
    return buffer_launch_gather_packed(b, d_plan, on, gn, batch, sq_threshold, clip_obs, o);
}

extern "C" int hp_buffer_sample_dev_fast(hp_buffer *b, hp_norm *on, hp_norm *gn, int64_t batch, double future_p, double sq_threshold,
                                         double clip_obs, uint64_t seed, uint64_t call, int32_t f32_rows, const hp_sample_dev_out *o) {
    HP_REQUIRE(b && on && gn && o, HP_ERR_INVALID, "hp_buffer_sample_dev_fast: null argument");
    HP_REQUIRE(on->ctx == b->ctx && gn->ctx == b->ctx, HP_ERR_INVALID, "hp_buffer_sample_dev_fast: handles of different contexts");
    HP_REQUIRE(on->size == b->obs_dim && gn->size == b->goal_dim, HP_ERR_INVALID,
               "hp_buffer_sample_dev_fast: normalizer sizes (%d, %d) do not match the buffer's observation / goal widths (%d, %d)", on->size,
               gn->size, b->obs_dim, b->goal_dim);
    HP_REQUIRE(batch > 0 && clip_obs > 0, HP_ERR_INVALID, "hp_buffer_sample_dev_fast: batch and clip_obs must be positive");
    HP_SERIALISE(b);
    HP_REQUIRE(!f32_rows || b->p_row, HP_ERR_STATE, "hp_buffer_sample_dev_fast: hp_buffer_enable_f32_rows first");
    HP_REQUIRE(b->current_size > 0, HP_ERR_EMPTY, "high <= 0");
    const FastDraw fd{seed, call, future_p};
    return f32_rows ? buffer_launch_gather_packed(b, nullptr, on, gn, batch, sq_threshold, clip_obs, o, &fd)
                    : buffer_launch_gather_fused(b, nullptr, on, gn, batch, sq_threshold, clip_obs, o, &fd);
}

extern "C" int hp_buffer_sample_dev_fast_us(hp_buffer *b, hp_norm *on, hp_norm *gn, int64_t batch, double future_p, double sq_threshold,
                                            double clip_obs, int32_t reps, int32_t f32_rows, double *us) {
    HP_REQUIRE(b && on && gn && us && batch > 0 && reps > 0, HP_ERR_INVALID, "hp_buffer_sample_dev_fast_us: bad argument");
    HP_SERIALISE(b);
    hipStream_t s = b->ctx->stream;
    const size_t ldx = (size_t)(b->obs_dim + b->goal_dim);
    if ((size_t)batch * (2 * ldx + b->act_dim + 1) * 4 > b->out.bytes) HP_CHECK_HIP(hipStreamSynchronize(s));
    HP_TRY(b->out.ensure((size_t)batch * (2 * ldx + b->act_dim + 1) * 4));
    hp_sample_dev_out o;
    memset(&o, 0, sizeof(o));
    o.x = b->out.as<float>();
    o.x_next = o.x + batch * ldx;
    o.actions = o.x_next + batch * ldx;
    o.r = o.actions + batch * b->act_dim;
    struct Events {
        hipEvent_t e[2] = {nullptr, nullptr};
        ~Events() { for (hipEvent_t x : e) if (x) (void)hipEventDestroy(x); }
    } ev;
    for (int i = 0; i < 2; ++i) HP_CHECK_HIP(hipEventCreate(&ev.e[i]));
    HP_TRY(hp_buffer_sample_dev_fast(b, on, gn, batch, future_p, sq_threshold, clip_obs, 1, 0, f32_rows, &o));
    HP_CHECK_HIP(hipEventRecord(ev.e[0], s));
    for (int i = 0; i < reps; ++i) HP_TRY(hp_buffer_sample_dev_fast(b, on, gn, batch, future_p, sq_threshold, clip_obs, 1, 1 + i, f32_rows, &o));
    HP_CHECK_HIP(hipEventRecord(ev.e[1], s));
    HP_CHECK_HIP(hipEventSynchronize(ev.e[1]));
    float ms = 0.f;
    HP_CHECK_HIP(hipEventElapsedTime(&ms, ev.e[0], ev.e[1]));
    *us = 1e3 * ms / reps;
    return HP_OK;
}

extern "C" int hp_buffer_sample_dev_us(hp_buffer *b, hp_rng *rng, hp_norm *on, hp_norm *gn, int64_t batch, double future_p,
                                       double sq_threshold, double clip_obs, int32_t reps, int32_t f32_rows, double *draw_us,
                                       double *gather_us) {
    hp_sample_dev_out o;
    memset(&o, 0, sizeof(o));
    HP_TRY(sample_dev_check(b, rng, on, gn, batch, clip_obs, &o, "hp_buffer_sample_dev_us"));
    HP_REQUIRE(draw_us && gather_us && reps > 0, HP_ERR_INVALID, "hp_buffer_sample_dev_us: bad argument");
    HP_SERIALISE(b);
    HP_REQUIRE(b->current_size > 0, HP_ERR_EMPTY, "high <= 0");
    HP_REQUIRE(!f32_rows || b->p_row, HP_ERR_STATE, "hp_buffer_sample_dev_us: hp_buffer_enable_f32_rows first");
    auto gather = [&](const PlanRec *plan, const hp_sample_dev_out *out) {
        return f32_rows ? buffer_launch_gather_packed(b, plan, on, gn, batch, sq_threshold, clip_obs, out)
                        : buffer_launch_gather_fused(b, plan, on, gn, batch, sq_threshold, clip_obs, out);
    };
    hipStream_t s = b->ctx->stream;
    const size_t ldx = (size_t)(b->obs_dim + b->goal_dim);
    if ((size_t)batch * sizeof(PlanRec) > b->plan.bytes || (size_t)batch * (2 * ldx + b->act_dim + 1) * 4 > b->out.bytes)
        HP_CHECK_HIP(hipStreamSynchronize(s));
    HP_TRY(b->plan.ensure(batch * sizeof(PlanRec)));
    HP_TRY(b->out.ensure((size_t)batch * (2 * ldx + b->act_dim + 1) * 4));
    PlanRec *d_plan = b->plan.as<PlanRec>();
    o.x = b->out.as<float>();
    o.x_next = o.x + batch * ldx;
    o.actions = o.x_next + batch * ldx;
    o.r = o.actions + batch * b->act_dim;
    struct Events {
        hipEvent_t e[3] = {nullptr, nullptr, nullptr};
        ~Events() { for (hipEvent_t x : e) if (x) (void)hipEventDestroy(x); }
    } ev;
    for (int i = 0; i < 3; ++i) HP_CHECK_HIP(hipEventCreate(&ev.e[i]));
    HP_TRY(rng_launch_plan_sample(rng, b->d_meta, b->T, batch, future_p, d_plan));
    HP_TRY(gather(d_plan, &o));
    HP_CHECK_HIP(hipEventRecord(ev.e[0], s));
    for (int i = 0; i < reps; ++i) HP_TRY(rng_launch_plan_sample(rng, b->d_meta, b->T, batch, future_p, d_plan));
    HP_CHECK_HIP(hipEventRecord(ev.e[1], s));
    for (int i = 0; i < reps; ++i) HP_TRY(gather(d_plan, &o));
    HP_CHECK_HIP(hipEventRecord(ev.e[2], s));
    HP_CHECK_HIP(hipEventSynchronize(ev.e[2]));
    float ms01 = 0.f, ms12 = 0.f;
    HP_CHECK_HIP(hipEventElapsedTime(&ms01, ev.e[0], ev.e[1]));
    HP_CHECK_HIP(hipEventElapsedTime(&ms12, ev.e[1], ev.e[2]));
    *draw_us = 1e3 * ms01 / reps;
    *gather_us = 1e3 * ms12 / reps;
    return HP_OK;
}

static int goal_reward_launch(hp_ctx *ctx, const double *ag, const double *g, int64_t n, int32_t goal_dim, double thr_sq,
                              int mode, float *out32, double *out64) {
    hipLaunchKernelGGL(k_goal_reward, dim3((unsigned)((n + 255) / 256)), dim3(256), 0, ctx->stream, ag, g, (long long)n,
                       (int)goal_dim, thr_sq, mode, out32, out64);
    HP_CHECK_HIP(hipGetLastError());
    return HP_OK;
}

static double squared_bound(double thr, bool strict) {
    if (!(thr >= 0.0)) return 0.0;
    double s = thr * thr;
    auto hit = [&](double v) { const double r = std::sqrt(v); return strict ? r > thr : r >= thr; };
    while (s > 0.0 && hit(s)) s = std::nextafter(s, -INFINITY);
    while (!hit(s)) s = std::nextafter(s, INFINITY);
    return s;
}

int hp_compute_reward_dev(hp_ctx *ctx, const double *ag_dev, const double *g_dev, int64_t n, int32_t goal_dim,
                          double distance_threshold, int32_t dense, float *sparse_out_dev, double *dense_out_dev) {
    HP_REQUIRE(ctx && ag_dev && g_dev, HP_ERR_INVALID, "hp_compute_reward_dev: null argument");
    CtxGuard guard(ctx);
    HP_REQUIRE(n >= 0 && goal_dim > 0, HP_ERR_INVALID, "hp_compute_reward_dev: bad shape");
    HP_REQUIRE(dense ? dense_out_dev != nullptr : sparse_out_dev != nullptr, HP_ERR_INVALID,
               "hp_compute_reward_dev: the output of the selected reward type is null");
    if (n == 0) return HP_OK;
    return goal_reward_launch(ctx, ag_dev, g_dev, n, goal_dim, dense ? 0.0 : squared_bound(distance_threshold, true),
                              dense ? 1 : 0, sparse_out_dev, dense_out_dev);
}

int hp_is_success_dev(hp_ctx *ctx, const double *ag_dev, const double *g_dev, int64_t n, int32_t goal_dim,
                      double distance_threshold, float *out_dev) {
    HP_REQUIRE(ctx && ag_dev && g_dev && out_dev, HP_ERR_INVALID, "hp_is_success_dev: null argument");
    CtxGuard guard(ctx);
    HP_REQUIRE(n >= 0 && goal_dim > 0, HP_ERR_INVALID, "hp_is_success_dev: bad shape");
    if (n == 0) return HP_OK;
    return goal_reward_launch(ctx, ag_dev, g_dev, n, goal_dim, squared_bound(distance_threshold, false), 2, out_dev,
                              nullptr);
}

static int goal_reward_host(hp_ctx *ctx, const double *ag, const double *g, int64_t n, int32_t goal_dim, double thr_sq,
                            int mode, void *out_host) {
    DevBuf &ws = ctx->reward_ws;
    const size_t nb = (size_t)n * goal_dim * 8, ob = (size_t)n * (mode == 1 ? 8 : 4);
    HP_TRY(ws.ensure(2 * nb + ob));
    char *d = ws.as<char>();
    hipStream_t s = ctx->stream;
    HP_CHECK_HIP(hipMemcpyAsync(d, ag, nb, hipMemcpyHostToDevice, s));
    HP_CHECK_HIP(hipMemcpyAsync(d + nb, g, nb, hipMemcpyHostToDevice, s));
    HP_TRY(goal_reward_launch(ctx, reinterpret_cast<double *>(d), reinterpret_cast<double *>(d + nb), n, goal_dim, thr_sq,
                              mode, reinterpret_cast<float *>(d + 2 * nb), reinterpret_cast<double *>(d + 2 * nb)));
    HP_CHECK_HIP(hipMemcpyAsync(out_host, d + 2 * nb, ob, hipMemcpyDeviceToHost, s));
    HP_CHECK_HIP(hipStreamSynchronize(s));
    return HP_OK;
}

int hp_compute_reward(hp_ctx *ctx, const double *ag_host, const double *g_host, int64_t n, int32_t goal_dim,
                      double distance_threshold, int32_t dense, float *sparse_out_host, double *dense_out_host) {
    HP_REQUIRE(ctx && ag_host && g_host, HP_ERR_INVALID, "hp_compute_reward: null argument");
    CtxGuard guard(ctx);
    HP_REQUIRE(n >= 0 && goal_dim > 0, HP_ERR_INVALID, "hp_compute_reward: bad shape");
    HP_REQUIRE(dense ? dense_out_host != nullptr : sparse_out_host != nullptr, HP_ERR_INVALID,
               "hp_compute_reward: the output of the selected reward type is null");
    if (n == 0) return HP_OK;
    return goal_reward_host(ctx, ag_host, g_host, n, goal_dim, dense ? 0.0 : squared_bound(distance_threshold, true),
                            dense ? 1 : 0, dense ? (void *)dense_out_host : (void *)sparse_out_host);
}

int hp_is_success(hp_ctx *ctx, const double *ag_host, const double *g_host, int64_t n, int32_t goal_dim,
                  double distance_threshold, float *out_host) {
    HP_REQUIRE(ctx && ag_host && g_host && out_host, HP_ERR_INVALID, "hp_is_success: null argument");
    CtxGuard guard(ctx);
    HP_REQUIRE(n >= 0 && goal_dim > 0, HP_ERR_INVALID, "hp_is_success: bad shape");
    if (n == 0) return HP_OK;
    return goal_reward_host(ctx, ag_host, g_host, n, goal_dim, squared_bound(distance_threshold, false), 2, out_host);
}

void hp_buffer_destroy(hp_buffer *b) {
    if (!b) return;
    if (b->d_obs) (void)hipFree(b->d_obs);
    if (b->d_ag) (void)hipFree(b->d_ag);
    if (b->d_g) (void)hipFree(b->d_g);
    if (b->d_act) (void)hipFree(b->d_act);
    if (b->d_meta) (void)hipFree(b->d_meta);
    if (b->d_slot_epoch) (void)hipFree(b->d_slot_epoch);
    if (b->d_epoch) (void)hipFree(b->d_epoch);
    b->dirty_counts.release();
    if (b->p_row) (void)hipFree(b->p_row);
    if (b->p_goal) (void)hipFree(b->p_goal);
    for (hipEvent_t ev : b->pin_events)
        if (ev) (void)hipEventDestroy(ev);
    b->st_obs.release();
    b->st_slots.release();
    b->pin.release();
    b->plan.release();
    b->out.release();
    delete b;
}

}
```

rl_arm_under_sparse_reward_amd/csrc/cycle_open.hip:

```cpp
#include "mt19937_device.h"
#include "norm_device.h"
#include "store_device.h"
#include "agent.h"

#define OPEN_THREADS NORM_THREADS
#define OPEN_PARTS 2
static_assert(MT_THREADS == 2 * NORM_MAX, "the draw and the normalizer columns use the same 512 threads");

struct OpenArgs {
    MtState *st;
    BufMeta *meta;
    long long size, inc;
    int T;
    long long *slots;
    PlanRec *norm_plan;
    PlanRec *plan;
    long long batch;
    int n_first;
    double future_p;
    const double *s_obs, *s_ag, *s_g, *s_act;
    double *obs, *ag, *g, *act;
    long long ep_obs, ep_ag, ep_g, ep_act;
    uint32_t *slot_epoch;
    const uint32_t *epoch;
    NormDev *onz, *gnz;
    int obs_dim, goal_dim;
    double clip_obs;
    int recompute;
    double o_eps_sq, g_eps_sq;
    int o_std_f32, g_std_f32;
    int chunk_rows;
    unsigned *sync;
    AgentDevState *dev;
    unsigned *fault, *fault_host;
};

__device__ __forceinline__ void open_publish(unsigned *flag) {
    asm volatile("s_waitcnt vmcnt(0)" ::: "memory");
    __syncthreads();
    if (threadIdx.x == 0) __hip_atomic_store(flag, 1u, __ATOMIC_RELAXED, __HIP_MEMORY_SCOPE_AGENT);
}

__device__ __forceinline__ bool open_wait(unsigned *flag, const OpenArgs &A) {
    __shared__ int s_open_ok;
    if (threadIdx.x == 0) {
        int spins = 0;
        while (__hip_atomic_load(flag, __ATOMIC_RELAXED, __HIP_MEMORY_SCOPE_AGENT) == 0u && ++spins < (1 << 22))
            __builtin_amdgcn_s_sleep(2);
        if (spins >= (1 << 22)) {
            atomicAdd(&A.dev->open_timeouts, 1u);
            handoff_fault(A.fault, A.fault_host, 3u);
        }
        s_open_ok = spins < (1 << 22) ? 1 : 0;
    }
    __syncthreads();
    return s_open_ok != 0;
}

__device__ __forceinline__ void open_leave(unsigned *sync) {
    const unsigned old = __hip_atomic_fetch_add(sync + 2, 1u, __ATOMIC_RELAXED, __HIP_MEMORY_SCOPE_AGENT);
    if (old + 1u == gridDim.x) {
        __hip_atomic_store(sync + 0, 0u, __ATOMIC_RELAXED, __HIP_MEMORY_SCOPE_AGENT);
        __hip_atomic_store(sync + 1, 0u, __ATOMIC_RELAXED, __HIP_MEMORY_SCOPE_AGENT);
        __hip_atomic_store(sync + 2, 0u, __ATOMIC_RELAXED, __HIP_MEMORY_SCOPE_AGENT);
    }
}

__global__ __launch_bounds__(OPEN_THREADS) void k_cycle_open(const OpenArgs A) {
    extern __shared__ __attribute__((aligned(16))) char open_lds[];
    const int role = blockIdx.x;
    if (role == 0) {
        if (threadIdx.x >= MT_THREADS) return;
        uint32_t(*ring)[MT_N] = reinterpret_cast<uint32_t(*)[MT_N]>(open_lds);
        int *ibuf = reinterpret_cast<int *>(open_lds + 4 * MT_N * sizeof(uint32_t));
        MtWg g;
        mt_load(g, A.st, ring, ibuf);
        const long long cur = A.meta->current_size;
        const long long now = (cur + A.inc < A.size) ? cur + A.inc : A.size;
        mt_draw_slots<true>(g, cur, A.size, A.inc, A.slots);
        open_publish(A.sync + 0);
        mt_her_draw<true>(g, A.inc, A.T, A.T, 1, A.future_p, A.norm_plan);
        open_publish(A.sync + 1);
        mt_her_draw(g, now, A.T, A.batch, A.n_first, A.future_p, A.plan);
        mt_store(g, A.st);
        if (threadIdx.x == 0) {
            A.meta->current_size = now;
            A.meta->n_transitions_stored += (long long)A.T * A.inc;
            open_leave(A.sync);
        }
    } else if (role == 1) {
        if (open_wait(A.sync + 1, A))
            norm_update_from_plan_body<true>(A.onz, A.gnz, A.norm_plan, (long long)A.T, A.s_obs, A.s_ag, A.s_g, A.T, A.obs_dim,
                                             A.goal_dim, A.clip_obs, A.recompute, A.o_eps_sq, A.o_std_f32, A.g_eps_sq, A.g_std_f32,
                                             A.chunk_rows, open_lds);
        if (threadIdx.x == 0) open_leave(A.sync);
    } else {
        const int w = role - 2;
        if (open_wait(A.sync + 0, A))
        store_scatter_share([&](long long j) { return __hip_atomic_load(A.slots + j, __ATOMIC_RELAXED, __HIP_MEMORY_SCOPE_AGENT); },
                            w / OPEN_PARTS, w % OPEN_PARTS, OPEN_PARTS, A.inc, A.s_obs, A.s_ag, A.s_g, A.s_act, A.obs, A.ag, A.g,
                            A.act, A.ep_obs, A.ep_ag, A.ep_g, A.ep_act, A.slot_epoch, A.epoch);
        if (threadIdx.x == 0) open_leave(A.sync);
    }
}

bool cycle_open_fits(const hp_agent *a, int64_t n_new) {
    return 2 + OPEN_PARTS * n_new <= (int64_t)a->ctx->cu_count;
}

int cycle_open_launch(hp_agent *a, hp_buffer *b, hp_norm *on, hp_norm *gn, hp_rng *rng, PlanRec *norm_plan, int n_first,
                      double future_p, bool recompute) {
    OpenArgs A;
    A.st = rng->d_state;
    A.meta = b->d_meta;
    A.size = b->size;
    A.inc = b->staged_n;
    A.T = b->T;
    A.slots = b->st_slots.as<long long>();
    A.norm_plan = norm_plan;
    A.plan = a->plan.as<PlanRec>();
    A.batch = a->B;
    A.n_first = n_first;
    A.future_p = future_p;
    A.s_obs = b->st_obs.as<double>();
    A.s_ag = b->st_ag;
    A.s_g = b->st_g;
    A.s_act = b->st_act;
    A.obs = b->d_obs;
    A.ag = b->d_ag;
    A.g = b->d_g;
    A.act = b->d_act;
    A.ep_obs = b->ep_obs();
    A.ep_ag = b->ep_ag();
    A.ep_g = b->ep_g();
    A.ep_act = b->ep_act();
    A.slot_epoch = b->d_slot_epoch;
    A.epoch = b->d_epoch;
    A.onz = on->d;
    A.gnz = gn->d;
    A.obs_dim = b->obs_dim;
    A.goal_dim = b->goal_dim;
    A.clip_obs = a->cfg.clip_obs;
    A.recompute = recompute ? 1 : 0;
    A.o_eps_sq = on->eps * on->eps;
    A.g_eps_sq = gn->eps * gn->eps;
    A.o_std_f32 = on->std_f32;
    A.g_std_f32 = gn->std_f32;
    size_t norm_bytes = 0;
    A.chunk_rows = norm_plan_chunk(b->obs_dim, b->goal_dim, b->T, &norm_bytes);
    A.sync = a->open_sync;
    A.dev = a->d_state;
    A.fault = a->k1_sync + SPLIT_FAULT;
    A.fault_host = a->fault_host_dev;
    const size_t mt_bytes = 4 * MT_N * sizeof(uint32_t) + MT_IBUF * sizeof(int);
    const size_t lds = norm_bytes > mt_bytes ? norm_bytes : mt_bytes;
    HP_KLOG("k_cycle_open");
    hipLaunchKernelGGL(k_cycle_open, dim3((unsigned)(2 + OPEN_PARTS * b->staged_n)), dim3(OPEN_THREADS), lds, a->ctx->stream, A);
    HP_CHECK_HIP(hipGetLastError());
    return buffer_launch_pack(b, b->staged_n);
}
```

rl_arm_under_sparse_reward_amd/csrc/internal.h:

```cpp
#pragma once
#include <hip/hip_runtime.h>

#include <cstdarg>
#include <cstdint>
#include <cstdio>
#include <cstring>
#include <mutex>
#include <string>
#include <vector>

#include "rlarm_hip.h"
#include "rlarm_hip_debug.h"

void hp_set_error(const char *fmt, ...);

extern thread_local std::vector<std::string> *hp_klog;
#define HP_KLOG(name) do { if (hp_klog) hp_klog->push_back(name); } while (0)

#define HP_CHECK_HIP(expr)                                                                   \
    do {                                                                                     \
        hipError_t _e = (expr);                                                              \
        if (_e != hipSuccess) {                                                              \
            hp_set_error("%s failed: %s (%s:%d)", #expr, hipGetErrorString(_e), __FILE__, __LINE__); \
            return HP_ERR_HIP;                                                               \
        }                                                                                    \
    } while (0)

#define HP_REQUIRE(cond, code, ...)   \
    do {                              \
        if (!(cond)) {                \
            hp_set_error(__VA_ARGS__); \
            return (code);            \
        }                             \
    } while (0)

#define HP_TRY(expr)              \
    do {                          \
        int _s = (expr);          \
        if (_s != HP_OK) return _s; \
    } while (0)

struct DevBuf {
    void *p = nullptr;
    size_t bytes = 0;
    int ensure(size_t need) {
        if (need <= bytes) return HP_OK;
        if (p) (void)hipFree(p);
        p = nullptr;
        bytes = 0;
        HP_CHECK_HIP(hipMalloc(&p, need));
        bytes = need;
        return HP_OK;
    }
    void release() {
        if (p) (void)hipFree(p);
        p = nullptr;
        bytes = 0;
    }
    template <class T> T *as() const { return reinterpret_cast<T *>(p); }
};

struct GraphExec {
    hipGraphExec_t h = nullptr;
    GraphExec() = default;
    GraphExec(GraphExec &&o) noexcept : h(o.h) { o.h = nullptr; }
    GraphExec &operator=(GraphExec &&o) noexcept { std::swap(h, o.h); return *this; }
    ~GraphExec() { if (h) (void)hipGraphExecDestroy(h); }
};
struct Captured {
    int st = HP_OK;
    hipError_t e = hipSuccess;
    GraphExec exec;
    int status() const {
        if (st != HP_OK) return st;
        HP_REQUIRE(e == hipSuccess, HP_ERR_HIP, "stream capture failed: %s", hipGetErrorString(e));
        return HP_OK;
    }
};
template <class F> Captured capture_graph(hipStream_t s, F &&enqueue, bool instantiate = true) {
    Captured c;
    c.e = hipStreamBeginCapture(s, hipStreamCaptureModeThreadLocal);
    if (c.e == hipSuccess) {
        c.st = enqueue();
        hipGraph_t g = nullptr;
        c.e = hipStreamEndCapture(s, &g);
        if (c.st == HP_OK && c.e == hipSuccess && instantiate) c.e = hipGraphInstantiate(&c.exec.h, g, nullptr, nullptr, 0);
        if (g) (void)hipGraphDestroy(g);
    }
    if (c.e != hipSuccess) {
        c.exec.h = nullptr;
        (void)hipGetLastError();
    }
    return c;
}

struct hp_ctx {
    int device = 0;
    hipStream_t stream = nullptr;
    hipStream_t own_stream = nullptr;
    hipEvent_t order_ev = nullptr;
    hipStream_t borrowed_from = nullptr, foreign = nullptr;
    bool own_dirty = true;
    hipEvent_t fence_ev[2] = {nullptr, nullptr};
    int cu_count = 0;
    char name[128] = {0};
    std::recursive_mutex mu;
    DevBuf reward_ws;
};
void ctx_join_foreign(hp_ctx *c);
struct CtxGuard {
    std::lock_guard<std::recursive_mutex> g;
    explicit CtxGuard(hp_ctx *c) : g(c->mu) {
        (void)hipSetDevice(c->device);
        if (!c->borrowed_from) {
            if (c->foreign) ctx_join_foreign(c);
            c->own_dirty = true;
        }
    }
};
#define HP_SERIALISE(handle) CtxGuard hp_serialise_guard_((handle)->ctx)

struct PinnedBuf {
    void *p = nullptr;
    size_t bytes = 0;
    hipEvent_t fence = nullptr;
    bool pending = false;
    int ensure(size_t need) {
        if (!fence) HP_CHECK_HIP(hipEventCreateWithFlags(&fence, hipEventDisableTiming));
        if (pending) {
            HP_CHECK_HIP(hipEventSynchronize(fence));
            pending = false;
        }
        if (need <= bytes) return HP_OK;
        if (p) (void)hipHostFree(p);
        p = nullptr;
        bytes = 0;
        HP_CHECK_HIP(hipHostMalloc(&p, need, hipHostMallocDefault));
        bytes = need;
        return HP_OK;
    }
    int mark(hipStream_t s) {
        HP_CHECK_HIP(hipEventRecord(fence, s));
        pending = true;
        return HP_OK;
    }
    void release() {
        if (pending && fence) (void)hipEventSynchronize(fence);
        if (p) (void)hipHostFree(p);
        if (fence) (void)hipEventDestroy(fence);
        p = nullptr;
        fence = nullptr;
        bytes = 0;
        pending = false;
    }
};

#define MT_N 624
struct MtState {
    uint32_t key[MT_N];
    int32_t pos;
    int32_t has_gauss;
    double gauss;
};
static_assert(sizeof(MtState) == MT_N * 4 + 16, "MtState: key | pos | has_gauss | gauss");

__host__ __device__ inline void mt_init_genrand(uint32_t seed, uint32_t *key) {
    for (uint32_t i = 0; i < MT_N; ++i) {
        key[i] = seed;
        seed = 1812433253u * (seed ^ (seed >> 30)) + i + 1u;
    }
}

struct hp_rng_streams {
    hp_ctx *ctx = nullptr;
    int64_t n = 1;
    MtState *d_state = nullptr;
};
int mt_states_get(hp_rng_streams *s, MtState *host, int64_t first, int64_t count);
int mt_states_put(hp_rng_streams *s, const MtState *host, int64_t first, int64_t count);
int mt_state_fill(MtState &h, const char *entry, int64_t stream, const uint32_t *key624, int32_t pos, int32_t has_gauss, double gauss);

struct hp_rng : hp_rng_streams {
    DevBuf scratch;
    int64_t par_min_batch = 0;
    int64_t par_debug_window = 0;
    struct ParCtl *d_par = nullptr;
    DevBuf par_raw, par_win, par_counts, par_table, par_poly;
    std::vector<uint64_t> par_polys;
    double par_table_ms = 0;
};
void rng_parallel_release(hp_rng *rng);

struct __attribute__((aligned(16))) PlanRec {
    int32_t e;
    int32_t t;
    int32_t fut;
    int32_t her;
};

struct BufMeta {
    int64_t current_size;
    int64_t n_transitions_stored;
};

struct hp_buffer {
    hp_ctx *ctx = nullptr;
    int64_t size = 0;
    int32_t T = 0, obs_dim = 0, goal_dim = 0, act_dim = 0;
    double *d_obs = nullptr, *d_ag = nullptr, *d_g = nullptr, *d_act = nullptr;
    BufMeta *d_meta = nullptr;
    uint32_t *d_slot_epoch = nullptr, *d_epoch = nullptr;
    uint32_t epoch = 1, min_since = 0;
    DevBuf dirty_counts;
    int64_t current_size = 0, n_transitions_stored = 0;
    DevBuf st_obs, st_slots;
    double *st_ag = nullptr, *st_g = nullptr, *st_act = nullptr;
    PinnedBuf pin;
    int64_t staged_n = 0;
    static constexpr int PIN_RING = 16;
    hipEvent_t pin_events[PIN_RING] = {nullptr};
    uint64_t pin_tickets = 0;
    float *p_row = nullptr;
    double *p_goal = nullptr;
    int32_t row_w = 0, goal_w = 0;
    DevBuf plan, out;
    uint64_t gen = 0;
    size_t ep_obs() const { return (size_t)(T + 1) * obs_dim; }
    size_t ep_ag() const { return (size_t)(T + 1) * goal_dim; }
    size_t ep_g() const { return (size_t)T * goal_dim; }
    size_t ep_act() const { return (size_t)T * act_dim; }
};
int buffer_launch_pack(hp_buffer *b, int64_t n_new);
int buffer_launch_pack_range(hp_buffer *b, int64_t first, int64_t n);

#define NORM_MAX 256
struct NormDev {
    float local_sum[NORM_MAX], local_sumsq[NORM_MAX], local_count[4];
    float total_sum[NORM_MAX], total_sumsq[NORM_MAX], total_count[4];
    float sync[2 * NORM_MAX + 4];
    float mean[NORM_MAX];
    double std[NORM_MAX];
};

struct hp_norm {
    hp_ctx *ctx = nullptr;
    int32_t size = 0;
    double eps = 1e-2, clip = 0;
    int32_t std_f32 = 0;
    NormDev *d = nullptr;
    DevBuf scratch, scratch2;
    PinnedBuf pin;
    bool in_recompute = false;
};

#ifdef __HIPCC__
__device__ __forceinline__ float hp_reward(double s, double sq_threshold) {
    if (sq_threshold < 0.0) return (float)(-__dsqrt_rn(s));
    return (s >= sq_threshold) ? -1.0f : -0.0f;
}
__device__ __forceinline__ double hp_reward64(double s, double sq_threshold) {
    if (sq_threshold < 0.0) return -__dsqrt_rn(s);
    return (s >= sq_threshold) ? -1.0 : -0.0;
}
#endif

struct hp_comm {
    hp_ctx *ctx = nullptr;
    void *nccl = nullptr;
    int rank = 0, world = 1;
};
int comm_allreduce_sum_f32(hp_comm *c, float *dev, size_t n);
int comm_allreduce_mean_f32(hp_comm *c, float *dev, size_t n);

int rng_launch_plan(hp_rng *rng, const BufMeta *d_meta, int64_t n_eps_fixed, int32_t T, int64_t batch,
                    int32_t n_batches, double future_p, PlanRec *d_plan, hipStream_t stream = nullptr);
int rng_launch_slots(hp_rng *rng, hp_buffer *buf, int64_t n_new, int64_t *d_slots);
int rng_launch_plan_sample(hp_rng *rng, const BufMeta *d_meta, int32_t T, int64_t batch, double future_p, PlanRec *d_plan);
int rng_launch_plan2(hp_rng *rng, int64_t n_first, int32_t T, int64_t batch_first, PlanRec *d_plan_first,
                     const BufMeta *d_meta, int64_t batch, int32_t n_batches, double future_p, PlanRec *d_plan);

int buffer_launch_gather_dict(hp_buffer *buf, const PlanRec *d_plan, int64_t batch, double sq_threshold,
                              double *d_out, float *d_r, double *d_r64);
int buffer_stage_and_store(hp_buffer *b, hp_rng *rng, const double *obs, const double *ag, const double *g,
                           const double *actions, int64_t n_new);
int buffer_stage_for_cycle(hp_buffer *b, const double *obs, const double *ag, const double *g, const double *actions,
                           int64_t n_new);
int buffer_stage_pinned(hp_buffer *b, hp_rng *rng, const double *block, int64_t n_new, uint64_t *ticket, bool store_now);
int buffer_stage_dev(hp_buffer *b, hp_rng *rng, const double *block_dev, int64_t n_new, bool store_now);

int agent_act_dev(hp_agent *a, hp_norm *on, hp_norm *gn, int32_t net, const double *obs_dev, const double *g_dev, int64_t rows,
                  double clip_obs, float *actions_dev);

int norm_launch_update_from_plan(hp_norm *o, hp_norm *g, hp_buffer *b, const PlanRec *d_plan, int64_t rows,
                                 double clip_obs, bool recompute);
int norm_launch_begin(hp_norm *nz);
int norm_launch_end(hp_norm *nz);
```

rl_arm_under_sparse_reward_amd/csrc/norm_device.h:

```cpp
#pragma once
#include "internal.h"

__device__ __forceinline__ double clipd(double v, double lo, double hi) {
    return fmin(fmax(v, lo), hi);
}

__device__ __forceinline__ void norm_recompute_column(NormDev *nz, int c, int size, float ls, float lss, float lc,
                                                      double eps_sq, int std_f32, float &cnt_out) {
    const float cnt = __fadd_rn(nz->total_count[0], lc);
    cnt_out = cnt;
    if (c < size) {
        nz->sync[c] = ls;
        nz->sync[size + c] = lss;
        nz->local_sum[c] = 0.f;
        nz->local_sumsq[c] = 0.f;
        const float ts = __fadd_rn(nz->total_sum[c], ls);
        const float tss = __fadd_rn(nz->total_sumsq[c], lss);
        nz->total_sum[c] = ts;
        nz->total_sumsq[c] = tss;
        const float m = (float)__ddiv_rn((double)ts, (double)cnt);
        nz->mean[c] = m;
        const float var = __fsub_rn((float)__ddiv_rn((double)tss, (double)cnt), __fmul_rn(m, m));
        if (std_f32) nz->std[c] = (double)(float)__dsqrt_rn((double)fmaxf((float)eps_sq, var));
        else nz->std[c] = __dsqrt_rn(fmax(eps_sq, (double)var));
    }
}

#define NORM_THREADS 1024
template <bool SC1_PLAN>
__device__ __forceinline__ void norm_update_from_plan_body(
    NormDev *onz, NormDev *gnz, const PlanRec *__restrict__ plan, long long rows, const double *__restrict__ s_obs,
    const double *__restrict__ s_ag, const double *__restrict__ s_g, int T, int obs_dim, int goal_dim, double clip_obs,
    int recompute, double o_eps_sq, int o_std_f32, double g_eps_sq, int g_std_f32, int chunk_rows, char *norm_lds) {
    PlanRec *sp = reinterpret_cast<PlanRec *>(norm_lds);
    double *sv = reinterpret_cast<double *>(norm_lds + (size_t)chunk_rows * sizeof(PlanRec));
    const int c = threadIdx.x;
    const bool goal = c >= NORM_MAX;
    const int j = goal ? c - NORM_MAX : c;
    NormDev *nz = goal ? gnz : onz;
    const int size = goal ? goal_dim : obs_dim;
    const bool act = c < 2 * NORM_MAX && j < size;
    const int W = obs_dim + goal_dim;
    double s = 0.0, ss = 0.0;
    for (long long r0 = 0; r0 < rows; r0 += chunk_rows) {
        const int n = (int)((rows - r0) < chunk_rows ? (rows - r0) : chunk_rows);
        for (int r = c; r < n; r += NORM_THREADS) {
            if (SC1_PLAN) {
                const unsigned long long *q = reinterpret_cast<const unsigned long long *>(plan + r0 + r);
                const unsigned long long lo = __hip_atomic_load(q, __ATOMIC_RELAXED, __HIP_MEMORY_SCOPE_AGENT);
                const unsigned long long hi = __hip_atomic_load(q + 1, __ATOMIC_RELAXED, __HIP_MEMORY_SCOPE_AGENT);
                PlanRec rec;
                rec.e = (int)(unsigned)lo; rec.t = (int)(unsigned)(lo >> 32); rec.fut = (int)(unsigned)hi; rec.her = (int)(unsigned)(hi >> 32);
                sp[r] = rec;
            } else {
                sp[r] = plan[r0 + r];
            }
        }
        __syncthreads();
        for (int idx = c; idx < n * W; idx += NORM_THREADS) {
            const int r = idx / W, col = idx - r * W;
            const PlanRec p = sp[r];
            const int k = col - obs_dim;
            const double *src = col < obs_dim ? s_obs + ((long long)p.e * (T + 1) + p.t) * obs_dim + col
                                              : (p.her ? s_ag + ((long long)p.e * (T + 1) + p.fut) * goal_dim + k
                                                       : s_g + ((long long)p.e * T + p.t) * goal_dim + k);
            sv[idx] = clipd(*src, -clip_obs, clip_obs);
        }
        __syncthreads();
        if (act) {
            const double *col = sv + (goal ? obs_dim + j : j);
            for (int r = 0; r < n; ++r) {
                const double v = col[(size_t)r * W];
                s = __dadd_rn(s, v);
                ss = __dadd_rn(ss, __dmul_rn(v, v));
            }
        }
        __syncthreads();
    }
    if (c >= 2 * NORM_MAX) return;
    float ls = 0.f, lss = 0.f;
    if (act) {
        ls = (float)__dadd_rn((double)nz->local_sum[j], s);
        lss = (float)__dadd_rn((double)nz->local_sumsq[j], ss);
    }
    const float lc = (float)((double)nz->local_count[0] + (double)rows);
    __syncthreads();
    if (!recompute) {
        if (act) {
            nz->local_sum[j] = ls;
            nz->local_sumsq[j] = lss;
        }
        if (j == 0) nz->local_count[0] = lc;
        return;
    }
    float cnt;
    norm_recompute_column(nz, j, size, ls, lss, lc, goal ? g_eps_sq : o_eps_sq, goal ? g_std_f32 : o_std_f32, cnt);
    __syncthreads();
    if (j == 0) {
        nz->sync[2 * size] = lc;
        nz->local_count[0] = 0.f;
        nz->total_count[0] = cnt;
    }
}

inline int norm_plan_chunk(int obs_dim, int goal_dim, long long rows, size_t *lds_bytes) {
    const int W = obs_dim + goal_dim;
    int chunk = (int)((48 * 1024) / (sizeof(PlanRec) + (size_t)W * 8));
    chunk = chunk > 256 ? 256 : chunk;
    chunk = rows < chunk ? (int)rows : chunk;
    *lds_bytes = (size_t)chunk * (sizeof(PlanRec) + (size_t)W * 8);
    return chunk;
}
```

rl_arm_under_sparse_reward_amd/csrc/store_device.h:

```cpp
#pragma once
#include "internal.h"

template <class SlotOf>
__device__ __forceinline__ void store_scatter_share(SlotOf slot_of, long long i, int part, int parts, long long n_new,
                                                    const double *s_obs, const double *s_ag, const double *s_g,
                                                    const double *s_act, double *obs, double *ag, double *g, double *act,
                                                    long long ep_obs, long long ep_ag, long long ep_g, long long ep_act,
                                                    uint32_t *slot_epoch, const uint32_t *epoch) {
    const long long slot = slot_of(i);
    if (threadIdx.x == 0) slot_epoch[slot] = *epoch;
    int dup = 0;
    for (long long j = i + 1 + threadIdx.x; j < n_new; j += blockDim.x) dup |= (slot_of(j) == slot);
    if (__syncthreads_or(dup)) return;
    const long long t0 = (long long)part * blockDim.x + threadIdx.x, step = (long long)parts * blockDim.x;
    for (long long k = t0; k < ep_obs; k += step) obs[slot * ep_obs + k] = s_obs[i * ep_obs + k];
    for (long long k = t0; k < ep_ag; k += step) ag[slot * ep_ag + k] = s_ag[i * ep_ag + k];
    for (long long k = t0; k < ep_g; k += step) g[slot * ep_g + k] = s_g[i * ep_g + k];
    for (long long k = t0; k < ep_act; k += step) act[slot * ep_act + k] = s_act[i * ep_act + k];
}
```

Measured before the change: 7.072 million transitions/s.

## Stream staged episodes from mapped pinned ring directly in cycle-open kernel

Adds a triple-buffered mapped, coherent pinned host ring for new episodes in the cycle-open path. The host memcpys episodes into a ring slot, and the cycle-open scatter workgroups read them over the bus, write the staging area and scatter into the replay buffer in one pass. This removes the separate host-to-device memcpy before the cycle graph. In exchange it adds an extra sync counter, atomic loads in the normalizer, graph cache entries per ring slot, and event fences that can block the host when a ring slot is reused.

```diff
diff --git a/include/rlarm_hip_debug.h b/include/rlarm_hip_debug.h
--- a/include/rlarm_hip_debug.h
+++ b/include/rlarm_hip_debug.h
@@ -36,6 +36,8 @@
 int hp_state_debug_dirty_scan(hp_buffer *buf, const uint32_t *stamps_host, int64_t current_size, uint32_t since, int64_t max_dirty,
                               int64_t *slots_out, int64_t *n_dirty, int32_t *overflow);
 
+int hp_buffer_debug_stage_info(hp_buffer *buf, uint64_t *gen, uint64_t *ring_bytes, int32_t *ring_block);
+
 int hp_rollout_debug_set_launch_cap(hp_rollout *ro, int64_t timesteps);
 
 int hp_ctx_calibrate(hp_ctx *ctx, double *out4);
diff --git a/rl_arm_under_sparse_reward_amd/_lib.py b/rl_arm_under_sparse_reward_amd/_lib.py
--- a/rl_arm_under_sparse_reward_amd/_lib.py
+++ b/rl_arm_under_sparse_reward_amd/_lib.py
@@ -73,7 +73,7 @@
 DEBUG_SYMBOLS = {"hp_ctx_launch_floor", "hp_ctx_event_pair_us", "hp_ctx_clock_mhz", "hp_ctx_calibrate", "hp_buffer_sample_device_us",
                  "hp_buffer_sample_dev_us", "hp_buffer_sample_dev_fast_us",
                  "hp_mt_jump_poly", "hp_rng_parallel_info", "hp_rng_debug_set_window", "hp_rng_debug_table_ms",
-                 "hp_state_debug_dirty_scan", "hp_rollout_debug_set_launch_cap",
+                 "hp_state_debug_dirty_scan", "hp_rollout_debug_set_launch_cap", "hp_buffer_debug_stage_info",
                  "hp_agent_set_adam", "hp_agent_debug_chain", "hp_agent_debug_timeline", "hp_agent_update_kernels"}
 
 PROTOTYPES = {
@@ -119,6 +119,7 @@
     "hp_buffer_store_done": (C.c_int, [C.c_void_p, C.c_uint64, C.c_int32, C.POINTER(C.c_int32)]),
     "hp_buffer_info": (C.c_int, [C.c_void_p, i64p, i64p, i64p, C.POINTER(C.c_int32)]),
     "hp_buffer_last_slots": (C.c_int, [C.c_void_p, i64p, C.c_int64]),
+    "hp_buffer_debug_stage_info": (C.c_int, [C.c_void_p, C.POINTER(C.c_uint64), C.POINTER(C.c_uint64), C.POINTER(C.c_int32)]),
     "hp_buffer_read": (C.c_int, [C.c_void_p, C.c_int32, C.c_int64, C.c_int64, f64p]),
     "hp_buffer_sample": (C.c_int, [C.c_void_p, C.c_void_p, C.c_int64, C.c_double, C.c_double, C.POINTER(SampleOut)]),
     "hp_buffer_sample_device_us": (C.c_int, [C.c_void_p, C.c_void_p, C.c_int64, C.c_double, C.c_double, C.c_int32, f64p,
diff --git a/rl_arm_under_sparse_reward_amd/csrc/agent.h b/rl_arm_under_sparse_reward_amd/csrc/agent.h
--- a/rl_arm_under_sparse_reward_amd/csrc/agent.h
+++ b/rl_arm_under_sparse_reward_amd/csrc/agent.h
@@ -127,9 +127,11 @@
     double future_p, sq_threshold;
     bool open;
     uint64_t gen;
+    int ring_slot;
     bool operator==(const SeqKey &o) const {
         return kind == o.kind && b == o.b && on == o.on && gn == o.gn && rng == o.rng && n == o.n && n_new == o.n_new &&
-               future_p == o.future_p && sq_threshold == o.sq_threshold && open == o.open && gen == o.gen;
+               future_p == o.future_p && sq_threshold == o.sq_threshold && open == o.open && gen == o.gen &&
+               ring_slot == o.ring_slot;
     }
 };
 struct GraphCache {
@@ -148,7 +150,7 @@
     }
     hipGraphExec_t put(const SeqKey &k, GraphExec &&x) {
         const auto same_kind = [&](const Entry &e) { return e.key.kind == k.kind; };
-        if (std::count_if(entries.begin(), entries.end(), same_kind) >= (k.kind == SeqKey::CYCLE ? 1 : 8))
+        if (std::count_if(entries.begin(), entries.end(), same_kind) >= (k.kind == SeqKey::CYCLE ? decltype(hp_buffer::ring)::SLOTS + 1 : 8))
             entries.erase(std::find_if(entries.begin(), entries.end(), same_kind));
         entries.push_back({k, std::move(x)});
         return entries.back().exec.h;
@@ -224,6 +226,7 @@
     unsigned *fault_host = nullptr;
     unsigned *fault_host_dev = nullptr;
     bool cycle_open = true;
+    bool cycle_open_copy = false;
     bool prof = false;
     hipEvent_t ev0 = nullptr, ev1 = nullptr;
     double prof_ms[PROF_N] = {0};
@@ -420,6 +423,7 @@
 int enqueue_adam(hp_agent *a, const GatherCtx *gc = nullptr, unsigned *reset_sync = nullptr);
 int enqueue_polyak(hp_agent *a);
 bool cycle_open_fits(const hp_agent *a, int64_t n_new);
+bool cycle_open_direct_fits(const hp_buffer *b, int64_t n_new);
 int cycle_open_launch(hp_agent *a, hp_buffer *b, hp_norm *on, hp_norm *gn, hp_rng *rng, PlanRec *norm_plan, int n_first,
                       double future_p, bool recompute);
 int enqueue_peer_adam(hp_agent *a, const GatherCtx *gc, unsigned *reset_sync);
diff --git a/rl_arm_under_sparse_reward_amd/csrc/agent.hip b/rl_arm_under_sparse_reward_amd/csrc/agent.hip
--- a/rl_arm_under_sparse_reward_amd/csrc/agent.hip
+++ b/rl_arm_under_sparse_reward_amd/csrc/agent.hip
@@ -261,6 +261,8 @@
         a->upd_graph_ok = tri("RLARM_UPDATE_GRAPH") != 0;
         a->keep_grads_dbg = tri("RLARM_KEEP_GRADS") == 1;
         a->cycle_open = tri("RLARM_CYCLE_OPEN") != 0;
+        const char *co = getenv("RLARM_CYCLE_OPEN");
+        a->cycle_open_copy = co && strcmp(co, "copy") == 0;
         a->split_mode = tri("RLARM_SPLIT");
         a->dw64 = a->slab && (tri("RLARM_DW64") >= 0 ? tri("RLARM_DW64") == 1 : a->Mp >= 1536);
         if (const char *ds = getenv("RLARM_DW64"))
@@ -436,7 +438,7 @@
     HP_TRY(peer_check_alive(a->peer, "hp_agent_sample_and_update"));
     HP_TRY(agent_check_fault(a, "hp_agent_sample_and_update"));
     HP_REQUIRE(b->current_size > 0, HP_ERR_EMPTY, "high <= 0");
-    return run_seq(a, {SeqKey::UPDATES, b, on, gn, rng, n_updates, 0, future_p, sq_threshold, false, b->gen});
+    return run_seq(a, {SeqKey::UPDATES, b, on, gn, rng, n_updates, 0, future_p, sq_threshold, false, b->gen, -1});
 }
 
 int hp_agent_forward_backward(hp_agent *a, hp_buffer *b, hp_norm *on, hp_norm *gn, hp_rng *rng, double future_p,
@@ -629,9 +631,11 @@
     HP_REQUIRE(obs && ag_host && g && actions, HP_ERR_INVALID, "hp_agent_train_cycle: null episode array");
     HP_TRY(train_cycle_checks(a, b, n_new, n_batches, "hp_agent_train_cycle"));
     const bool open = a->cycle_open && cycle_open_fits(a, n_new);
-    if (open) HP_TRY(buffer_stage_for_cycle(b, obs, ag_host, g, actions, n_new));
+    const bool direct = open && !a->cycle_open_copy && cycle_open_direct_fits(b, n_new);
+    if (open) HP_TRY(buffer_stage_for_cycle(b, obs, ag_host, g, actions, n_new, direct));
     else HP_TRY(buffer_stage_and_store(b, rng, obs, ag_host, g, actions, n_new));
-    return run_seq(a, {SeqKey::CYCLE, b, on, gn, rng, n_batches, n_new, future_p, sq_threshold, open, b->gen});
+    HP_TRY(run_seq(a, {SeqKey::CYCLE, b, on, gn, rng, n_batches, n_new, future_p, sq_threshold, open, b->gen, direct ? b->ring_cur : -1}));
+    return direct ? buffer_mark_cycle_block(b) : HP_OK;
 }
 
 int hp_agent_train_cycle_pinned(hp_agent *a, hp_buffer *b, hp_norm *on, hp_norm *gn, hp_rng *rng, const double *block,
@@ -642,7 +646,7 @@
     HP_TRY(train_cycle_checks(a, b, n_new, n_batches, "hp_agent_train_cycle_pinned"));
     const bool open = a->cycle_open && cycle_open_fits(a, n_new);
     HP_TRY(buffer_stage_pinned(b, rng, block, n_new, ticket, !open));
-    return run_seq(a, {SeqKey::CYCLE, b, on, gn, rng, n_batches, n_new, future_p, sq_threshold, open, b->gen});
+    return run_seq(a, {SeqKey::CYCLE, b, on, gn, rng, n_batches, n_new, future_p, sq_threshold, open, b->gen, -1});
 }
 
 int hp_agent_train_cycle_dev(hp_agent *a, hp_buffer *b, hp_norm *on, hp_norm *gn, hp_rng *rng, const double *block_dev,
@@ -653,7 +657,7 @@
     HP_TRY(train_cycle_checks(a, b, n_new, n_batches, "hp_agent_train_cycle_dev"));
     const bool open = a->cycle_open && cycle_open_fits(a, n_new);
     HP_TRY(buffer_stage_dev(b, rng, block_dev, n_new, !open));
-    return run_seq(a, {SeqKey::CYCLE, b, on, gn, rng, n_batches, n_new, future_p, sq_threshold, open, b->gen});
+    return run_seq(a, {SeqKey::CYCLE, b, on, gn, rng, n_batches, n_new, future_p, sq_threshold, open, b->gen, -1});
 }
 
 int hp_agent_update_form(hp_agent *a, int32_t n_updates, int32_t *form) {
diff --git a/rl_arm_under_sparse_reward_amd/csrc/buffer.hip b/rl_arm_under_sparse_reward_amd/csrc/buffer.hip
--- a/rl_arm_under_sparse_reward_amd/csrc/buffer.hip
+++ b/rl_arm_under_sparse_reward_amd/csrc/buffer.hip
@@ -495,6 +495,7 @@
     HP_CHECK_HIP(hipMemcpyAsync(dst, h, n0 + n1 + n2 + n3, hipMemcpyHostToDevice, s));
     HP_TRY(b->pin.mark(s));
     b->staged_n = n_new;
+    b->ring_cur = -1;
     return HP_OK;
 }
 
@@ -533,6 +534,7 @@
     HP_CHECK_HIP(hipEventRecord(ev, s));
     if (ticket) *ticket = t;
     b->staged_n = n_new;
+    b->ring_cur = -1;
     if (store_now) {
         HP_TRY(rng_launch_slots(rng, b, n_new, b->st_slots.as<int64_t>()));
         hipLaunchKernelGGL(k_store_scatter, dim3((unsigned)(n_new * STORE_PARTS)), dim3(256), 0, s, b->st_slots.as<long long>(),
@@ -558,6 +560,7 @@
     b->st_act = reinterpret_cast<double *>(dst + n0 + n1 + n2);
     HP_CHECK_HIP(hipMemcpyAsync(dst, block_dev, n0 + n1 + n2 + n3, hipMemcpyDeviceToDevice, s));
     b->staged_n = n_new;
+    b->ring_cur = -1;
     if (store_now) {
         HP_TRY(rng_launch_slots(rng, b, n_new, b->st_slots.as<int64_t>()));
         hipLaunchKernelGGL(k_store_scatter, dim3((unsigned)(n_new * STORE_PARTS)), dim3(256), 0, s, b->st_slots.as<long long>(),
@@ -571,10 +574,43 @@
     return HP_OK;
 }
 
+static int buffer_stage_ring(hp_buffer *b, const double *obs, const double *ag, const double *g, const double *actions,
+                             int64_t n_new) {
+    const size_t n0 = n_new * b->ep_obs() * 8, n1 = n_new * b->ep_ag() * 8, n2 = n_new * b->ep_g() * 8,
+                 n3 = n_new * b->ep_act() * 8;
+    HP_TRY(stage_ensure(b, b->st_obs, n0 + n1 + n2 + n3));
+    char *dst = b->st_obs.as<char>();
+    b->st_ag = reinterpret_cast<double *>(dst + n0);
+    b->st_g = reinterpret_cast<double *>(dst + n0 + n1);
+    b->st_act = reinterpret_cast<double *>(dst + n0 + n1 + n2);
+    HipStageApi api;
+    int idx = -1;
+    bool moved = false;
+    HP_TRY(b->ring.acquire(api, n0 + n1 + n2 + n3, &idx, &moved));
+    if (moved) ++b->gen;
+    char *h = static_cast<char *>(b->ring.slot[idx].host);
+    memcpy(h, obs, n0);
+    memcpy(h + n0, ag, n1);
+    memcpy(h + n0 + n1, g, n2);
+    memcpy(h + n0 + n1 + n2, actions, n3);
+    b->staged_n = n_new;
+    b->ring_cur = idx;
+    return HP_OK;
+}
+
+int buffer_mark_cycle_block(hp_buffer *b) {
+    if (b->ring_cur < 0) return HP_OK;
+    HipStageApi api;
+    const int st = b->ring.mark(api, b->ring_cur, b->ctx->stream);
+    if (st != HP_OK) (void)hipStreamSynchronize(b->ctx->stream);
+    return st;
+}
+
 int buffer_stage_for_cycle(hp_buffer *b, const double *obs, const double *ag, const double *g, const double *actions,
-                           int64_t n_new) {
+                           int64_t n_new, bool direct) {
     HP_TRY(stage_ensure(b, b->st_slots, n_new * 8));
-    HP_TRY(buffer_stage(b, obs, ag, g, actions, n_new));
+    if (direct) HP_TRY(buffer_stage_ring(b, obs, ag, g, actions, n_new));
+    else HP_TRY(buffer_stage(b, obs, ag, g, actions, n_new));
     b->current_size = (b->current_size + n_new < b->size) ? b->current_size + n_new : b->size;
     b->n_transitions_stored += (int64_t)b->T * n_new;
     return HP_OK;
@@ -695,6 +731,15 @@
     if (current_size) *current_size = b->current_size;
     if (n_transitions_stored) *n_transitions_stored = b->n_transitions_stored;
     if (T) *T = b->T;
+    return HP_OK;
+}
+
+int hp_buffer_debug_stage_info(hp_buffer *b, uint64_t *gen, uint64_t *ring_bytes, int32_t *ring_block) {
+    HP_REQUIRE(b, HP_ERR_INVALID, "hp_buffer_debug_stage_info: null handle");
+    HP_SERIALISE(b);
+    if (gen) *gen = b->gen;
+    if (ring_bytes) *ring_bytes = b->ring.bytes;
+    if (ring_block) *ring_block = b->ring_cur;
     return HP_OK;
 }
 
@@ -1136,6 +1181,10 @@
     b->st_obs.release();
     b->st_slots.release();
     b->pin.release();
+    {
+        HipStageApi api;
+        b->ring.release(api);
+    }
     b->plan.release();
     b->out.release();
     delete b;
diff --git a/rl_arm_under_sparse_reward_amd/csrc/cycle_open.hip b/rl_arm_under_sparse_reward_amd/csrc/cycle_open.hip
--- a/rl_arm_under_sparse_reward_amd/csrc/cycle_open.hip
+++ b/rl_arm_under_sparse_reward_amd/csrc/cycle_open.hip
@@ -31,6 +31,8 @@
     int o_std_f32, g_std_f32;
     int chunk_rows;
     unsigned *sync;
+    const double *pin;
+    StageBlock blk;
     AgentDevState *dev;
     unsigned *fault, *fault_host;
 };
@@ -41,11 +43,12 @@
     if (threadIdx.x == 0) __hip_atomic_store(flag, 1u, __ATOMIC_RELAXED, __HIP_MEMORY_SCOPE_AGENT);
 }
 
-__device__ __forceinline__ bool open_wait(unsigned *flag, const OpenArgs &A) {
+__device__ __forceinline__ bool open_wait(unsigned *flag, const OpenArgs &A, unsigned want = 1u) {
     __shared__ int s_open_ok;
+    __syncthreads();
     if (threadIdx.x == 0) {
         int spins = 0;
-        while (__hip_atomic_load(flag, __ATOMIC_RELAXED, __HIP_MEMORY_SCOPE_AGENT) == 0u && ++spins < (1 << 22))
+        while (__hip_atomic_load(flag, __ATOMIC_RELAXED, __HIP_MEMORY_SCOPE_AGENT) < want && ++spins < (1 << 22))
             __builtin_amdgcn_s_sleep(2);
         if (spins >= (1 << 22)) {
             atomicAdd(&A.dev->open_timeouts, 1u);
@@ -63,7 +66,31 @@
         __hip_atomic_store(sync + 0, 0u, __ATOMIC_RELAXED, __HIP_MEMORY_SCOPE_AGENT);
         __hip_atomic_store(sync + 1, 0u, __ATOMIC_RELAXED, __HIP_MEMORY_SCOPE_AGENT);
         __hip_atomic_store(sync + 2, 0u, __ATOMIC_RELAXED, __HIP_MEMORY_SCOPE_AGENT);
-    }
+        __hip_atomic_store(sync + 3, 0u, __ATOMIC_RELAXED, __HIP_MEMORY_SCOPE_AGENT);
+    }
+}
+
+__device__ __forceinline__ void open_scatter_direct(const OpenArgs &A, int w, int n_wg, char *lds) {
+    const unsigned gtid = (unsigned)w * OPEN_THREADS + threadIdx.x, nthreads = (unsigned)n_wg * OPEN_THREADS;
+    double v[STORE_DIRECT_CHUNKS][2];
+    stage_block_load(A.pin, A.blk.nd, gtid, nthreads, v);
+    stage_block_put(const_cast<double *>(A.s_obs), A.blk.nd, gtid, nthreads, v);
+    asm volatile("s_waitcnt vmcnt(0)" ::: "memory");
+    __syncthreads();
+    if (threadIdx.x == 0) __hip_atomic_fetch_add(A.sync + 3, 1u, __ATOMIC_RELAXED, __HIP_MEMORY_SCOPE_AGENT);
+    if (!open_wait(A.sync + 0, A)) return;
+    long long *raw = reinterpret_cast<long long *>(lds), *win = raw + A.inc;
+    for (long long e = threadIdx.x; e < A.inc; e += OPEN_THREADS)
+        raw[e] = __hip_atomic_load(A.slots + e, __ATOMIC_RELAXED, __HIP_MEMORY_SCOPE_AGENT);
+    __syncthreads();
+    for (long long e = threadIdx.x; e < A.inc; e += OPEN_THREADS) {
+        int dup = 0;
+        for (long long j = e + 1; j < A.inc; ++j) dup |= (raw[j] == raw[e]);
+        win[e] = dup ? -1ll : raw[e];
+    }
+    if (threadIdx.x == 0) A.slot_epoch[raw[w / OPEN_PARTS]] = *A.epoch;
+    __syncthreads();
+    stage_block_scatter(A.blk, win, gtid, nthreads, v, A.obs, A.ag, A.g, A.act);
 }
 
 __global__ __launch_bounds__(OPEN_THREADS) void k_cycle_open(const OpenArgs A) {
@@ -88,11 +115,20 @@
             A.meta->n_transitions_stored += (long long)A.T * A.inc;
             open_leave(A.sync);
         }
+    } else if (role == 1 && A.pin) {
+        if (open_wait(A.sync + 1, A) && open_wait(A.sync + 3, A, gridDim.x - 2u))
+            norm_update_from_plan_body<true, true>(A.onz, A.gnz, A.norm_plan, (long long)A.T, A.s_obs, A.s_ag, A.s_g, A.T, A.obs_dim,
+                                                   A.goal_dim, A.clip_obs, A.recompute, A.o_eps_sq, A.o_std_f32, A.g_eps_sq,
+                                                   A.g_std_f32, A.chunk_rows, open_lds);
+        if (threadIdx.x == 0) open_leave(A.sync);
     } else if (role == 1) {
         if (open_wait(A.sync + 1, A))
             norm_update_from_plan_body<true>(A.onz, A.gnz, A.norm_plan, (long long)A.T, A.s_obs, A.s_ag, A.s_g, A.T, A.obs_dim,
                                              A.goal_dim, A.clip_obs, A.recompute, A.o_eps_sq, A.o_std_f32, A.g_eps_sq, A.g_std_f32,
                                              A.chunk_rows, open_lds);
+        if (threadIdx.x == 0) open_leave(A.sync);
+    } else if (A.pin) {
+        open_scatter_direct(A, role - 2, (int)gridDim.x - 2, open_lds);
         if (threadIdx.x == 0) open_leave(A.sync);
     } else {
         const int w = role - 2;
@@ -106,6 +142,13 @@
 
 bool cycle_open_fits(const hp_agent *a, int64_t n_new) {
     return 2 + OPEN_PARTS * n_new <= (int64_t)a->ctx->cu_count;
+}
+
+bool cycle_open_direct_fits(const hp_buffer *b, int64_t n_new) {
+    const uint64_t nd = (uint64_t)n_new * (b->ep_obs() + b->ep_ag() + b->ep_g() + b->ep_act());
+    const uint64_t threads = (uint64_t)OPEN_PARTS * n_new * OPEN_THREADS;
+    return nd < (1ull << 31) && (nd + 1) / 2 <= STORE_DIRECT_CHUNKS * threads &&
+           (uint64_t)n_new * 2 * sizeof(long long) <= 4 * MT_N * sizeof(uint32_t);
 }
 
 int cycle_open_launch(hp_agent *a, hp_buffer *b, hp_norm *on, hp_norm *gn, hp_rng *rng, PlanRec *norm_plan, int n_first,
@@ -149,6 +192,15 @@
     size_t norm_bytes = 0;
     A.chunk_rows = norm_plan_chunk(b->obs_dim, b->goal_dim, b->T, &norm_bytes);
     A.sync = a->open_sync;
+    A.pin = b->ring_cur >= 0 ? static_cast<const double *>(b->ring.slot[b->ring_cur].dev) : nullptr;
+    A.blk.n_obs = (unsigned)(A.inc * A.ep_obs);
+    A.blk.n_ag = (unsigned)(A.inc * A.ep_ag);
+    A.blk.n_g = (unsigned)(A.inc * A.ep_g);
+    A.blk.ep_obs = (unsigned)A.ep_obs;
+    A.blk.ep_ag = (unsigned)A.ep_ag;
+    A.blk.ep_g = (unsigned)A.ep_g;
+    A.blk.ep_act = (unsigned)A.ep_act;
+    A.blk.nd = (unsigned)(A.inc * (A.ep_obs + A.ep_ag + A.ep_g + A.ep_act));
     A.dev = a->d_state;
     A.fault = a->k1_sync + SPLIT_FAULT;
     A.fault_host = a->fault_host_dev;
diff --git a/rl_arm_under_sparse_reward_amd/csrc/internal.h b/rl_arm_under_sparse_reward_amd/csrc/internal.h
--- a/rl_arm_under_sparse_reward_amd/csrc/internal.h
+++ b/rl_arm_under_sparse_reward_amd/csrc/internal.h
@@ -11,6 +11,7 @@
 
 #include "rlarm_hip.h"
 #include "rlarm_hip_debug.h"
+#include "stage_ring.h"
 
 void hp_set_error(const char *fmt, ...);
 
@@ -155,6 +156,31 @@
     }
 };
 
+struct HipStageApi {
+    using Event = hipEvent_t;
+    using Stream = hipStream_t;
+    int alloc(size_t bytes, void **host, void **dev) {
+        *host = *dev = nullptr;
+        HP_CHECK_HIP(hipHostMalloc(host, bytes, hipHostMallocMapped | hipHostMallocCoherent));
+        HP_CHECK_HIP(hipHostGetDevicePointer(dev, *host, 0));
+        return HP_OK;
+    }
+    void free_block(void *host) { (void)hipHostFree(host); }
+    int event_create(Event *e) {
+        HP_CHECK_HIP(hipEventCreateWithFlags(e, hipEventDisableTiming));
+        return HP_OK;
+    }
+    int event_sync(Event e) {
+        HP_CHECK_HIP(hipEventSynchronize(e));
+        return HP_OK;
+    }
+    int event_record(Event e, Stream s) {
+        HP_CHECK_HIP(hipEventRecord(e, s));
+        return HP_OK;
+    }
+    void event_destroy(Event e) { (void)hipEventDestroy(e); }
+};
+
 #define MT_N 624
 struct MtState {
     uint32_t key[MT_N];
@@ -216,6 +242,8 @@
     DevBuf st_obs, st_slots;
     double *st_ag = nullptr, *st_g = nullptr, *st_act = nullptr;
     PinnedBuf pin;
+    StageRing<HipStageApi> ring;
+    int ring_cur = -1;
     int64_t staged_n = 0;
     static constexpr int PIN_RING = 16;
     hipEvent_t pin_events[PIN_RING] = {nullptr};
@@ -284,7 +312,8 @@
 int buffer_stage_and_store(hp_buffer *b, hp_rng *rng, const double *obs, const double *ag, const double *g,
                            const double *actions, int64_t n_new);
 int buffer_stage_for_cycle(hp_buffer *b, const double *obs, const double *ag, const double *g, const double *actions,
-                           int64_t n_new);
+                           int64_t n_new, bool direct);
+int buffer_mark_cycle_block(hp_buffer *b);
 int buffer_stage_pinned(hp_buffer *b, hp_rng *rng, const double *block, int64_t n_new, uint64_t *ticket, bool store_now);
 int buffer_stage_dev(hp_buffer *b, hp_rng *rng, const double *block_dev, int64_t n_new, bool store_now);
 
diff --git a/rl_arm_under_sparse_reward_amd/csrc/norm_device.h b/rl_arm_under_sparse_reward_amd/csrc/norm_device.h
--- a/rl_arm_under_sparse_reward_amd/csrc/norm_device.h
+++ b/rl_arm_under_sparse_reward_amd/csrc/norm_device.h
@@ -27,7 +27,7 @@
 }
 
 #define NORM_THREADS 1024
-template <bool SC1_PLAN>
+template <bool SC1_PLAN, bool SC1_STAGE = false>
 __device__ __forceinline__ void norm_update_from_plan_body(
     NormDev *onz, NormDev *gnz, const PlanRec *__restrict__ plan, long long rows, const double *__restrict__ s_obs,
     const double *__restrict__ s_ag, const double *__restrict__ s_g, int T, int obs_dim, int goal_dim, double clip_obs,
@@ -64,7 +64,10 @@
             const double *src = col < obs_dim ? s_obs + ((long long)p.e * (T + 1) + p.t) * obs_dim + col
                                               : (p.her ? s_ag + ((long long)p.e * (T + 1) + p.fut) * goal_dim + k
                                                        : s_g + ((long long)p.e * T + p.t) * goal_dim + k);
-            sv[idx] = clipd(*src, -clip_obs, clip_obs);
+            const double x = SC1_STAGE ? __longlong_as_double(__hip_atomic_load(reinterpret_cast<const long long *>(src), __ATOMIC_RELAXED,
+                                                                                 __HIP_MEMORY_SCOPE_AGENT))
+                                       : *src;
+            sv[idx] = clipd(x, -clip_obs, clip_obs);
         }
         __syncthreads();
         if (act) {
diff --git a/rl_arm_under_sparse_reward_amd/csrc/stage_ring.h b/rl_arm_under_sparse_reward_amd/csrc/stage_ring.h
--- /dev/null
+++ b/rl_arm_under_sparse_reward_amd/csrc/stage_ring.h
@@ -0,0 +1,80 @@
+#pragma once
+#include <cstddef>
+
+template <class Api, int N = 3> struct StageRing {
+    static_assert(N >= 2, "one block being read by the device, one being filled by the host");
+    static constexpr int SLOTS = N;
+    struct Slot {
+        void *host = nullptr, *dev = nullptr;
+        typename Api::Event fence{};
+        bool has_fence = false, pending = false;
+    };
+    Slot slot[N];
+    size_t bytes = 0;
+    int next = 0;
+
+    int acquire(Api &api, size_t need, int *idx, bool *moved) {
+        *moved = false;
+        if (need > bytes) {
+            if (int st = drain(api)) return st;
+            free_blocks(api);
+            for (int i = 0; i < N; ++i)
+                if (int st = api.alloc(need, &slot[i].host, &slot[i].dev)) {
+                    free_blocks(api);
+                    return st;
+                }
+            bytes = need;
+            next = 0;
+            *moved = true;
+        }
+        Slot &s = slot[next];
+        if (s.pending) {
+            if (int st = api.event_sync(s.fence)) return st;
+            s.pending = false;
+        }
+        *idx = next;
+        next = (next + 1) % N;
+        return 0;
+    }
+
+    int mark(Api &api, int idx, typename Api::Stream stream) {
+        Slot &s = slot[idx];
+        if (!s.has_fence) {
+            if (int st = api.event_create(&s.fence)) return st;
+            s.has_fence = true;
+        }
+        if (int st = api.event_record(s.fence, stream)) return st;
+        s.pending = true;
+        return 0;
+    }
+
+    void release(Api &api) {
+        (void)drain(api);
+        free_blocks(api);
+        for (Slot &s : slot) {
+            if (s.has_fence) api.event_destroy(s.fence);
+            s.has_fence = false;
+            s.pending = false;
+        }
+        next = 0;
+    }
+
+private:
+    int drain(Api &api) {
+        int first = 0;
+        for (Slot &s : slot) {
+            if (!s.pending) continue;
+            const int st = api.event_sync(s.fence);
+            if (st && !first) first = st;
+            s.pending = false;
+        }
+        return first;
+    }
+    void free_blocks(Api &api) {
+        for (Slot &s : slot) {
+            if (s.host) api.free_block(s.host);
+            s.host = s.dev = nullptr;
+        }
+        bytes = 0;
+    }
+};
diff --git a/rl_arm_under_sparse_reward_amd/csrc/store_device.h b/rl_arm_under_sparse_reward_amd/csrc/store_device.h
--- a/rl_arm_under_sparse_reward_amd/csrc/store_device.h
+++ b/rl_arm_under_sparse_reward_amd/csrc/store_device.h
@@ -18,3 +18,62 @@
     for (long long k = t0; k < ep_g; k += step) g[slot * ep_g + k] = s_g[i * ep_g + k];
     for (long long k = t0; k < ep_act; k += step) act[slot * ep_act + k] = s_act[i * ep_act + k];
 }
+
+#define STORE_DIRECT_CHUNKS 4
+
+struct StageBlock {
+    unsigned n_obs, n_ag, n_g;
+    unsigned ep_obs, ep_ag, ep_g, ep_act;
+    unsigned nd;
+};
+
+__device__ __forceinline__ void stage_block_load(const double *__restrict__ blk, unsigned nd, unsigned gtid, unsigned nthreads,
+                                                 double (&v)[STORE_DIRECT_CHUNKS][2]) {
+#pragma unroll
+    for (int it = 0; it < STORE_DIRECT_CHUNKS; ++it) {
+        const unsigned d = 2u * (gtid + (unsigned)it * nthreads);
+        v[it][0] = v[it][1] = 0.0;
+        if (d + 1u < nd) {
+            const double2 x = *reinterpret_cast<const double2 *>(blk + d);
+            v[it][0] = x.x;
+            v[it][1] = x.y;
+        } else if (d < nd) {
+            v[it][0] = blk[d];
+        }
+    }
+}
+
+__device__ __forceinline__ void stage_block_put(double *stage, unsigned nd, unsigned gtid, unsigned nthreads,
+                                                const double (&v)[STORE_DIRECT_CHUNKS][2]) {
+#pragma unroll
+    for (int it = 0; it < STORE_DIRECT_CHUNKS; ++it) {
+        const unsigned d = 2u * (gtid + (unsigned)it * nthreads);
+#pragma unroll
+        for (int h = 0; h < 2; ++h)
+            if (d + h < nd)
+                __hip_atomic_store(reinterpret_cast<long long *>(stage) + d + h, __double_as_longlong(v[it][h]), __ATOMIC_RELAXED,
+                                   __HIP_MEMORY_SCOPE_AGENT);
+    }
+}
+
+__device__ __forceinline__ void stage_block_scatter(const StageBlock &L, const long long *win, unsigned gtid, unsigned nthreads,
+                                                    const double (&v)[STORE_DIRECT_CHUNKS][2], double *obs, double *ag, double *g,
+                                                    double *act) {
+#pragma unroll
+    for (int it = 0; it < STORE_DIRECT_CHUNKS; ++it) {
+#pragma unroll
+        for (int h = 0; h < 2; ++h) {
+            const unsigned d = 2u * (gtid + (unsigned)it * nthreads) + h;
+            if (d >= L.nd) continue;
+            unsigned r = d, len;
+            double *arr;
+            if (r < L.n_obs) { arr = obs; len = L.ep_obs; }
+            else if ((r -= L.n_obs) < L.n_ag) { arr = ag; len = L.ep_ag; }
+            else if ((r -= L.n_ag) < L.n_g) { arr = g; len = L.ep_g; }
+            else { r -= L.n_g; arr = act; len = L.ep_act; }
+            const unsigned e = r / len, k = r - e * len;
+            const long long slot = win[e];
+            if (slot >= 0) arr[slot * (long long)len + k] = v[it][h];
+        }
+    }
+}
```

Measured after the change: 7.170 million transitions/s (median of 6 runs). +1.4%, better.
